# smups/inflatox

Hardware: AMD Instinct MI355X
Metric: grid-points/sec on complete_analysis sweep; achieved HBM GB/s vs peak (higher is better)
Workload: dtype f64

## Files before the change

include/inflx_hip.h:

```cpp
#ifndef INFLX_HIP_H
#define INFLX_HIP_H

#include <stddef.h>
#include <stdint.h>

#ifdef __cplusplus
extern "C" {
#endif

typedef struct inflx_model inflx_model;

typedef enum inflx_status {
  INFLX_OK = 0,
  INFLX_ERR_IO = 1,
  INFLX_ERR_SYMBOL = 2,
  INFLX_ERR_VERSION = 3,
  INFLX_ERR_SHAPE = 4,
  INFLX_ERR_DEVICE = 5,
  INFLX_ERR_ARG = 6,
  INFLX_ERR_BASIS = 7,
  INFLX_ERR_GSL = 8
} inflx_status;

typedef enum inflx_sf_bits {
  INFLX_SF_EDOM = 1,
  INFLX_SF_EDECLINED = 2
} inflx_sf_bits;

typedef enum inflx_sf_policy_t {
  INFLX_SF_QUIET = 0,
  INFLX_SF_FAIL = 1
} inflx_sf_policy_t;

typedef enum inflx_op {
  INFLX_SWEEP_COMPLETE = 0,
  INFLX_SWEEP_CONSISTENCY = 1,
  INFLX_SWEEP_RAPIDTURN = 2,
  INFLX_SWEEP_EPSILON_V = 3,
  INFLX_SWEEP_RAW = 4,
  INFLX_SWEEP_HESSE = 6
} inflx_op;

typedef enum inflx_layout {
  INFLX_AOS = 0,
  INFLX_SOA = 1
} inflx_layout;

const char* inflx_last_error(void);

int inflx_device_count(int* count);

int inflx_open(const char* artefact_path, int device, inflx_model** out);
void inflx_close(inflx_model* model);

int inflx_attach(inflx_model* model, const char* group_object_path);
uint32_t inflx_groups(const inflx_model* model);

uint32_t inflx_n_fields(const inflx_model* model);
uint32_t inflx_n_parameters(const inflx_model* model);
const char* inflx_model_name(const inflx_model* model);
int inflx_device_of(const inflx_model* model);
int inflx_stage_info(const inflx_model* model, uint32_t* n_uniform, uint32_t* n_row, uint32_t* n_col, uint32_t* out_mask);

int inflx_complete_analysis(inflx_model* model, const double* p, size_t n_p, double* out, const double* start_stop,
                            size_t N0, size_t N1, int progress, size_t threads);
int inflx_consistency_only(inflx_model* model, const double* p, size_t n_p, double* out, const double* start_stop,
                           size_t N0, size_t N1, int progress, size_t threads);
int inflx_consistency_rapidturn_only(inflx_model* model, const double* p, size_t n_p, double* out,
                                     const double* start_stop, size_t N0, size_t N1, int progress,
                                     size_t threads);
int inflx_epsilon_v_only(inflx_model* model, const double* p, size_t n_p, double* out, const double* start_stop,
                         size_t N0, size_t N1, int progress, size_t threads);

int inflx_flag_quantum_dif(inflx_model* model, const double* p, size_t n_p, uint8_t* out, const double* start_stop,
                           size_t N0, size_t N1, int progress, double accuracy);

int inflx_sweep_on_trajectory(inflx_model* model, int op, const double* p, size_t n_p, const double* x, size_t n,
                              double* out, int progress, size_t threads);

int inflx_basis_on_points(inflx_model* model, const double* p, size_t n_p, const double* x, size_t n, double* out);
int inflx_validate_basis_at_random(inflx_model* model, uint64_t seed);
int inflx_validate_basis_on_domain(inflx_model* model, const uint32_t* num_points, size_t n_axes, const double* p,
                                   size_t n_p, const double* start_stop, double accuracy);

int inflx_ops_on_values(inflx_model* model, const double* values, size_t n, double* out, int ieee_only);

int inflx_sweep_host(inflx_model* model, int op, const double* p, size_t P, size_t n_p, double* out,
                     const double* start_stop, size_t N0, size_t N1, size_t row_begin, size_t row_count, int layout);

int inflx_sweep_host_planes(inflx_model* model, int op, const double* p, size_t P, size_t n_p, double* out,
                            const double* start_stop, size_t N0, size_t N1, size_t row_begin, size_t row_count,
                            size_t first_plane, size_t n_planes);

int inflx_sweep_device(inflx_model* model, int op, const double* p, size_t P, size_t n_p, void* d_out,
                       size_t d_out_bytes, const double* start_stop, size_t N0, size_t N1, size_t row_begin,
                       size_t row_count, int layout, void* stream);

typedef enum inflx_path {
  INFLX_PATH_TILE = 0,
  INFLX_PATH_ROW_STREAM = 1,
  INFLX_PATH_ROWS = 2,
  INFLX_PATH_COL_STREAM = 3
} inflx_path;
int inflx_sweep_plan(const inflx_model* model, int op, size_t P, size_t N1, size_t row_count, int layout, uint32_t plan[4]);

typedef enum inflx_sweep_flags {
  INFLX_SWEEP_DEFAULT = 0,
  INFLX_SWEEP_FORCE_TILE = 1
} inflx_sweep_flags;
int inflx_sweep_device_ex(inflx_model* model, int op, const double* p, size_t P, size_t n_p, void* d_out,
                          size_t d_out_bytes, const double* start_stop, size_t N0, size_t N1, size_t row_begin,
                          size_t row_count, int layout, void* stream, unsigned flags);
int inflx_sweep_plan_ex(const inflx_model* model, int op, size_t P, size_t N1, size_t row_count, int layout, unsigned flags,
                        uint32_t plan[4]);

int inflx_host_threads(unsigned devices_at_work, unsigned out[3]);

int inflx_sweep_device_timed(inflx_model* model, int op, const double* p, size_t P, size_t n_p, void* d_out,
                             size_t d_out_bytes, const double* start_stop, size_t N0, size_t N1, size_t row_begin,
                             size_t row_count, int layout, void* stream, int repeats, int dominant_only,
                             float* ms_per_launch);
typedef enum inflx_timing {
  INFLX_TIME_BACK_TO_BACK = 0,
  INFLX_TIME_DOMINANT_ONLY = 1,
  INFLX_TIME_IN_PIPELINE = 2,
  INFLX_TIME_SINGLE_CALL = 3
} inflx_timing;
int inflx_sweep_device_timed_ex(inflx_model* model, int op, const double* p, size_t P, size_t n_p, void* d_out,
                                size_t d_out_bytes, const double* start_stop, size_t N0, size_t N1, size_t row_begin,
                                size_t row_count, int layout, void* stream, int repeats, int mode, unsigned flags,
                                float* ms_per_launch);

typedef struct inflx_summary {
  double min[6];
  double max[6];
  uint64_t count[6];
} inflx_summary;

int inflx_sweep_device_stats(inflx_model* model, const double* p, size_t P, size_t n_p, void* d_out, size_t d_out_bytes,
                             const double* start_stop, size_t N0, size_t N1, size_t row_begin, size_t row_count,
                             void* stream, inflx_summary* summary);

int inflx_synchronize(inflx_model* model);

int inflx_sf_status(inflx_model* model, unsigned* bits, int clear);
int inflx_sf_policy(inflx_model* model, int policy);
int inflx_uses_gsl(const inflx_model* model);

typedef struct inflx_multi inflx_multi;
int inflx_shard_plan(size_t P, size_t N0, int world, int rank, size_t plan[5]);
int inflx_open_multi(const char* artefact_path, const int* devices, int n_dev, inflx_multi** out);
void inflx_close_multi(inflx_multi* multi);
int inflx_multi_device_count(const inflx_multi* multi);
inflx_model* inflx_multi_handle(const inflx_multi* multi, int index);
int inflx_sweep_host_multi(inflx_multi* multi, int op, const double* p, size_t P, size_t n_p, double* out,
                           const double* start_stop, size_t N0, size_t N1, int layout, int progress, size_t max_devices);
int inflx_complete_analysis_multi(inflx_multi* multi, const double* p, size_t n_p, double* out, const double* start_stop,
                                  size_t N0, size_t N1, int progress, size_t threads);
int inflx_sweep_stats_multi(inflx_multi* multi, const double* p, size_t P, size_t n_p, const double* start_stop, size_t N0,
                            size_t N1, size_t max_devices, inflx_summary* summary);
int inflx_sweep_device_multi(inflx_multi* multi, int op, const double* p, size_t P, size_t n_p, void* const* d_out,
                             const size_t* d_out_bytes, const double* start_stop, size_t N0, size_t N1, int layout,
                             void* const* streams);
int inflx_sweep_allgather_multi(inflx_multi* multi, int op, const double* p, size_t P, size_t n_p, void* const* d_full,
                                size_t d_full_bytes, const double* start_stop, size_t N0, size_t N1);
typedef enum inflx_gather {
  INFLX_GATHER_PEER_PUSH = 0,
  INFLX_GATHER_RCCL = 1
} inflx_gather;
int inflx_sweep_allgather_multi_ex(inflx_multi* multi, int op, const double* p, size_t P, size_t n_p, void* const* d_full,
                                   size_t d_full_bytes, const double* start_stop, size_t N0, size_t N1, int gather);

typedef enum inflx_eom_method {
  INFLX_EOM_RK4 = 0,
  INFLX_EOM_RKF = 1
} inflx_eom_method;
typedef enum inflx_eom_flags {
  INFLX_EOM_STOP_AT_END = 1,
  INFLX_EOM_FINAL_ONLY = 2,
  INFLX_EOM_SAMPLE_T = 4,
  INFLX_EOM_HOST_SCATTER = 8
} inflx_eom_flags;
typedef enum inflx_eom_status {
  INFLX_EOM_COMPLETE = 0,
  INFLX_EOM_ENDED = 1,
  INFLX_EOM_NONFINITE = 2,
  INFLX_EOM_REJECTED = 3,
  INFLX_EOM_UNDERFLOW = 4,
  INFLX_EOM_TARGET = 5
} inflx_eom_status;
int inflx_solve_eom(inflx_model* model, const double* p, size_t P, size_t n_p, const double* init, size_t B, size_t rows, size_t substeps,
                    int method, double max_err, double dt, unsigned flags, double* states, double* t, double* efolds, int8_t* status,
                    int64_t* last_row);

int inflx_solve_eom_device(inflx_model* model, const double* p, size_t P, size_t n_p, const double* init, size_t B, size_t rows,
                           size_t substeps, int method, double max_err, double dt, unsigned flags, double* d_states, size_t d_states_bytes,
                           double* d_t, size_t d_t_bytes, double* efolds, int8_t* status, int64_t* last_row, void* stream);

int inflx_solve_eom_to_efolds(inflx_model* model, const double* p, size_t P, size_t n_p, const double* init, size_t B, const double* target,
                              size_t max_steps, int method, double max_err, double dt, unsigned flags, double* states, double* t,
                              double* eps_h, double* efolds, int8_t* status);

int inflx_solve_eom_sampled(inflx_model* model, const double* p, size_t P, size_t n_p, const double* init, size_t B, const double* samples,
                            size_t S, size_t max_steps, int method, double max_err, double dt, unsigned flags, double* out, double* efolds,
                            int8_t* status, uint32_t* n_stored);

int inflx_kinematics(inflx_model* model, const double* p, size_t P, size_t n_p, const double* states, size_t n, size_t ld, size_t traj_len,
                     double* out);

int inflx_kinematics_device(inflx_model* model, const double* p, size_t P, size_t n_p, const void* d_states, size_t d_states_bytes, size_t n,
                            size_t ld, size_t traj_len, void* d_out, size_t d_out_bytes, void* stream);

int inflx_masses(inflx_model* model, const double* p, size_t P, size_t n_p, const double* states, size_t n, size_t ld, size_t traj_len, double* out);

int inflx_masses_device(inflx_model* model, const double* p, size_t P, size_t n_p, const void* d_states, size_t d_states_bytes, size_t n, size_t ld,
                        size_t traj_len, void* d_out, size_t d_out_bytes, void* stream);

#ifdef __cplusplus
}
#endif
#endif
```

inflatox_amd/_native.py:

```python

from __future__ import annotations

import ctypes as C
import os
import subprocess

import numpy as np

_PKG = os.path.dirname(os.path.abspath(__file__))
_REPO = os.path.dirname(_PKG)
LIB_PATH = os.path.join(_PKG, "libinflx_hip.so")

OK, ERR_IO, ERR_SYMBOL, ERR_VERSION, ERR_SHAPE, ERR_DEVICE, ERR_ARG, ERR_BASIS, ERR_GSL = range(9)
SF_EDOM, SF_EDECLINED = 1, 2
SF_QUIET, SF_FAIL = 0, 1

OP_COMPLETE, OP_CONSISTENCY, OP_RAPIDTURN, OP_EPSILON_V, OP_RAW = range(5)
OP_HESSE = 6
OP_QDIF = 5
OP_GROUP = {OP_COMPLETE: "core", OP_CONSISTENCY: "consistency", OP_RAPIDTURN: "rapidturn", OP_EPSILON_V: "epsilon_v", OP_RAW: "raw", OP_QDIF: "qdif", OP_HESSE: "hesse"}
OP_WIDTH = {OP_COMPLETE: 6, OP_CONSISTENCY: 1, OP_RAPIDTURN: 1, OP_EPSILON_V: 1, OP_RAW: 5, OP_HESSE: 4}
LAYOUT_AOS, LAYOUT_SOA = 0, 1
SWEEP_DEFAULT, SWEEP_FORCE_TILE = 0, 1
TIME_BACK_TO_BACK, TIME_DOMINANT_ONLY, TIME_IN_PIPELINE, TIME_SINGLE_CALL = range(4)
EOM_RK4, EOM_RKF = 0, 1
EOM_STOP_AT_END, EOM_FINAL_ONLY, EOM_SAMPLE_T, EOM_HOST_SCATTER = 1, 2, 4, 8
GATHER_PEER_PUSH, GATHER_RCCL = 0, 1

_DP = C.POINTER(C.c_double)
_SIZE = C.c_size_t

SIGNATURES = {
    "inflx_last_error": (C.c_char_p, []),
    "inflx_device_count": (C.c_int, [C.POINTER(C.c_int)]),
    "inflx_open": (C.c_int, [C.c_char_p, C.c_int, C.POINTER(C.c_void_p)]),
    "inflx_close": (None, [C.c_void_p]),
    "inflx_attach": (C.c_int, [C.c_void_p, C.c_char_p]),
    "inflx_groups": (C.c_uint32, [C.c_void_p]),
    "inflx_n_fields": (C.c_uint32, [C.c_void_p]),
    "inflx_n_parameters": (C.c_uint32, [C.c_void_p]),
    "inflx_model_name": (C.c_char_p, [C.c_void_p]),
    "inflx_device_of": (C.c_int, [C.c_void_p]),
    "inflx_stage_info": (C.c_int, [C.c_void_p] + [C.POINTER(C.c_uint32)] * 4),
    "inflx_complete_analysis": (C.c_int, [C.c_void_p, _DP, _SIZE, _DP, _DP, _SIZE, _SIZE, C.c_int, _SIZE]),
    "inflx_consistency_only": (C.c_int, [C.c_void_p, _DP, _SIZE, _DP, _DP, _SIZE, _SIZE, C.c_int, _SIZE]),
    "inflx_consistency_rapidturn_only": (C.c_int, [C.c_void_p, _DP, _SIZE, _DP, _DP, _SIZE, _SIZE, C.c_int, _SIZE]),
    "inflx_epsilon_v_only": (C.c_int, [C.c_void_p, _DP, _SIZE, _DP, _DP, _SIZE, _SIZE, C.c_int, _SIZE]),
    "inflx_flag_quantum_dif": (C.c_int, [C.c_void_p, _DP, _SIZE, C.POINTER(C.c_uint8), _DP, _SIZE, _SIZE, C.c_int, C.c_double]),
    "inflx_sweep_on_trajectory": (C.c_int, [C.c_void_p, C.c_int, _DP, _SIZE, _DP, _SIZE, _DP, C.c_int, _SIZE]),
    "inflx_sweep_host": (C.c_int, [C.c_void_p, C.c_int, _DP, _SIZE, _SIZE, _DP, _DP, _SIZE, _SIZE, _SIZE, _SIZE, C.c_int]),
    "inflx_sweep_host_planes": (C.c_int, [C.c_void_p, C.c_int, _DP, _SIZE, _SIZE, _DP, _DP, _SIZE, _SIZE, _SIZE, _SIZE, _SIZE, _SIZE]),
    "inflx_sweep_device": (
        C.c_int,
        [C.c_void_p, C.c_int, _DP, _SIZE, _SIZE, C.c_void_p, _SIZE, _DP, _SIZE, _SIZE, _SIZE, _SIZE, C.c_int, C.c_void_p],
    ),
    "inflx_sweep_device_timed": (
        C.c_int,
        [C.c_void_p, C.c_int, _DP, _SIZE, _SIZE, C.c_void_p, _SIZE, _DP, _SIZE, _SIZE, _SIZE, _SIZE, C.c_int, C.c_void_p, C.c_int, C.c_int, C.POINTER(C.c_float)],
    ),
    "inflx_sweep_device_ex": (
        C.c_int,
        [C.c_void_p, C.c_int, _DP, _SIZE, _SIZE, C.c_void_p, _SIZE, _DP, _SIZE, _SIZE, _SIZE, _SIZE, C.c_int, C.c_void_p, C.c_uint],
    ),
    "inflx_sweep_device_timed_ex": (
        C.c_int,
        [C.c_void_p, C.c_int, _DP, _SIZE, _SIZE, C.c_void_p, _SIZE, _DP, _SIZE, _SIZE, _SIZE, _SIZE, C.c_int, C.c_void_p, C.c_int, C.c_int, C.c_uint, C.POINTER(C.c_float)],
    ),
    "inflx_sweep_plan_ex": (C.c_int, [C.c_void_p, C.c_int, _SIZE, _SIZE, _SIZE, C.c_int, C.c_uint, C.POINTER(C.c_uint32)]),
    "inflx_host_threads": (C.c_int, [C.c_uint, C.POINTER(C.c_uint)]),
    "inflx_sweep_device_stats": (
        C.c_int,
        [C.c_void_p, _DP, _SIZE, _SIZE, C.c_void_p, _SIZE, _DP, _SIZE, _SIZE, _SIZE, _SIZE, C.c_void_p, C.c_void_p],
    ),
    "inflx_synchronize": (C.c_int, [C.c_void_p]),
    "inflx_sf_status": (C.c_int, [C.c_void_p, C.POINTER(C.c_uint), C.c_int]),
    "inflx_sf_policy": (C.c_int, [C.c_void_p, C.c_int]),
    "inflx_uses_gsl": (C.c_int, [C.c_void_p]),
    "inflx_sweep_plan": (C.c_int, [C.c_void_p, C.c_int, _SIZE, _SIZE, _SIZE, C.c_int, C.POINTER(C.c_uint32)]),
    "inflx_basis_on_points": (C.c_int, [C.c_void_p, _DP, _SIZE, _DP, _SIZE, _DP]),
    "inflx_ops_on_values": (C.c_int, [C.c_void_p, _DP, _SIZE, _DP, C.c_int]),
    "inflx_validate_basis_at_random": (C.c_int, [C.c_void_p, C.c_uint64]),
    "inflx_validate_basis_on_domain": (C.c_int, [C.c_void_p, C.POINTER(C.c_uint32), _SIZE, _DP, _SIZE, _DP, C.c_double]),
    "inflx_shard_plan": (C.c_int, [_SIZE, _SIZE, C.c_int, C.c_int, C.POINTER(_SIZE)]),
    "inflx_open_multi": (C.c_int, [C.c_char_p, C.POINTER(C.c_int), C.c_int, C.POINTER(C.c_void_p)]),
    "inflx_close_multi": (None, [C.c_void_p]),
    "inflx_multi_device_count": (C.c_int, [C.c_void_p]),
    "inflx_multi_handle": (C.c_void_p, [C.c_void_p, C.c_int]),
    "inflx_sweep_host_multi": (C.c_int, [C.c_void_p, C.c_int, _DP, _SIZE, _SIZE, _DP, _DP, _SIZE, _SIZE, C.c_int, C.c_int, _SIZE]),
    "inflx_complete_analysis_multi": (C.c_int, [C.c_void_p, _DP, _SIZE, _DP, _DP, _SIZE, _SIZE, C.c_int, _SIZE]),
    "inflx_sweep_stats_multi": (C.c_int, [C.c_void_p, _DP, _SIZE, _SIZE, _DP, _SIZE, _SIZE, _SIZE, C.c_void_p]),
    "inflx_sweep_device_multi": (C.c_int, [C.c_void_p, C.c_int, _DP, _SIZE, _SIZE, C.POINTER(C.c_void_p), C.POINTER(_SIZE), _DP, _SIZE, _SIZE, C.c_int, C.POINTER(C.c_void_p)]),
    "inflx_sweep_allgather_multi": (C.c_int, [C.c_void_p, C.c_int, _DP, _SIZE, _SIZE, C.POINTER(C.c_void_p), _SIZE, _DP, _SIZE, _SIZE]),
    "inflx_sweep_allgather_multi_ex": (C.c_int, [C.c_void_p, C.c_int, _DP, _SIZE, _SIZE, C.POINTER(C.c_void_p), _SIZE, _DP, _SIZE, _SIZE, C.c_int]),
    "inflx_solve_eom": (
        C.c_int,
        [C.c_void_p, _DP, _SIZE, _SIZE, _DP, _SIZE, _SIZE, _SIZE, C.c_int, C.c_double, C.c_double, C.c_uint, _DP, _DP, _DP, C.POINTER(C.c_int8), C.POINTER(C.c_int64)],
    ),
    "inflx_solve_eom_device": (
        C.c_int,
        [C.c_void_p, _DP, _SIZE, _SIZE, _DP, _SIZE, _SIZE, _SIZE, C.c_int, C.c_double, C.c_double, C.c_uint, C.c_void_p, _SIZE, C.c_void_p, _SIZE, _DP, C.POINTER(C.c_int8),
         C.POINTER(C.c_int64), C.c_void_p],
    ),
    "inflx_solve_eom_to_efolds": (
        C.c_int,
        [C.c_void_p, _DP, _SIZE, _SIZE, _DP, _SIZE, _DP, _SIZE, C.c_int, C.c_double, C.c_double, C.c_uint, _DP, _DP, _DP, _DP, C.POINTER(C.c_int8)],
    ),
    "inflx_solve_eom_sampled": (
        C.c_int,
        [C.c_void_p, _DP, _SIZE, _SIZE, _DP, _SIZE, _DP, _SIZE, _SIZE, C.c_int, C.c_double, C.c_double, C.c_uint, _DP, _DP, C.POINTER(C.c_int8), C.POINTER(C.c_uint32)],
    ),
    "inflx_kinematics": (C.c_int, [C.c_void_p, _DP, _SIZE, _SIZE, _DP, _SIZE, _SIZE, _SIZE, _DP]),
    "inflx_kinematics_device": (C.c_int, [C.c_void_p, _DP, _SIZE, _SIZE, C.c_void_p, _SIZE, _SIZE, _SIZE, _SIZE, C.c_void_p, _SIZE, C.c_void_p]),
    "inflx_masses": (C.c_int, [C.c_void_p, _DP, _SIZE, _SIZE, _DP, _SIZE, _SIZE, _SIZE, _DP]),
    "inflx_masses_device": (C.c_int, [C.c_void_p, _DP, _SIZE, _SIZE, C.c_void_p, _SIZE, _SIZE, _SIZE, _SIZE, C.c_void_p, _SIZE, C.c_void_p]),
}


class Summary(C.Structure):

    _fields_ = [("min", C.c_double * 6), ("max", C.c_double * 6), ("count", C.c_uint64 * 6)]

_lib = None


def build_library(force: bool = False) -> str:
    src = os.path.join(_PKG, "csrc", "inflx_hip.cpp")
    deps = [src, os.path.join(_PKG, "csrc", "inflx_kernel_abi.h"), os.path.join(_PKG, "csrc", "inflx_background_abi.h"), os.path.join(_PKG, "csrc", "inflx_background_rows.h"), os.path.join(_PKG, "csrc", "inflx_kinematics_abi.h"), os.path.join(_PKG, "csrc", "inflx_masses_abi.h"), os.path.join(_REPO, "include", "inflx_hip.h")]
    stale = force or not os.path.exists(LIB_PATH) or any(os.path.getmtime(d) > os.path.getmtime(LIB_PATH) for d in deps)
    if stale:
        from .compiler import hipcc_path

        cmd = [
            hipcc_path(),
            "-O2",
            "-fPIC",
            "-shared",
            "-std=c++17",
            "-Wall",
            "-Wextra",
            f"-I{os.path.join(_REPO, 'include')}",
            f"-I{os.path.join(_PKG, 'csrc')}",
            src,
            "-o",
            LIB_PATH + ".tmp",
        ]
        subprocess.run(cmd, check=True)
        os.replace(LIB_PATH + ".tmp", LIB_PATH)
    return LIB_PATH


def _preload_hip_runtime():
    import importlib.util

    try:
        spec = importlib.util.find_spec("torch")
    except (ImportError, ValueError):
        spec = None
    if spec is not None and spec.origin:
        cand = os.path.join(os.path.dirname(spec.origin), "lib", "libamdhip64.so")
        if os.path.exists(cand):
            C.CDLL(cand, mode=C.RTLD_GLOBAL)


def load_library():
    global _lib
    if _lib is None:
        if not os.path.exists(LIB_PATH):
            raise ImportError(
                f"{LIB_PATH} is missing: build it with `python -c 'import __graft_entry__ as g; g.build()'` "
                "(the sweep has no CPU fallback)"
            )
        _preload_hip_runtime()
        lib = C.CDLL(LIB_PATH)
        for name, (res, args) in SIGNATURES.items():
            fn = getattr(lib, name)
            fn.restype = res
            fn.argtypes = args
        _lib = lib
    return _lib


class InflatoxShapeError(Exception):
    """Counterpart of LibInflxRsErr::Shape, which PyO3 raises as a plain Exception (err.rs:71)."""


class InflatoxBasisError(Exception):
    """Counterpart of LibInflxRsErr::BasisNorm / BasisOth (err.rs:36-37), plain Exceptions in PyO3 too."""


class InflatoxSpecialFunctionError(ArithmeticError):
    """A special function of the model was called outside its domain somewhere in the call (``INFLX_ERR_GSL``).  The reference's
    GSL error handler prints the reason and panics at that point (src/err.rs:86-103): the call does not return there either.  Here
    the result was complete when the error was raised -- NaN at the offending points -- and ``sf_errors="nan"`` returns it."""


def _raise(rc: int):
    msg = load_library().inflx_last_error().decode("utf-8", "replace")
    if rc == ERR_GSL:
        raise InflatoxSpecialFunctionError(msg)
    if rc == ERR_IO:
        raise IOError(msg)
    if rc in (ERR_SYMBOL, ERR_VERSION, ERR_DEVICE):
        raise SystemError(msg)
    if rc == ERR_SHAPE:
        raise InflatoxShapeError(msg)
    if rc == ERR_BASIS:
        raise InflatoxBasisError(msg)
    raise ValueError(msg)


def _check(rc: int):
    if rc != OK:
        _raise(rc)


def _sf_policy(mode: str) -> int:
    try:
        return {"raise": SF_FAIL, "nan": SF_QUIET}[mode]
    except (KeyError, TypeError):
        raise ValueError(f'sf_errors must be "raise" or "nan" (got {mode!r})') from None


def _f64(a, name: str) -> np.ndarray:
    try:
        return np.ascontiguousarray(a, dtype=np.float64)
    except (TypeError, ValueError) as exc:
        raise ValueError(f"{name} must be convertible to a float64 array") from exc


def _ptr(a: np.ndarray):
    return a.ctypes.data_as(_DP)


def device_count() -> int:
    n = C.c_int(0)
    rc = load_library().inflx_device_count(C.byref(n))
    return n.value if rc == OK else 0


def _ensure_group(lib, handles, art, group: str) -> None:
    from .compiler import KERNEL_GROUPS

    bit = KERNEL_GROUPS[group]
    pending = [h for h in handles if not (int(lib.inflx_groups(h)) & bit)]
    if not pending or art is None:
        return
    path = art.ensure_group(group)
    if path is None:
        return
    for h in pending:
        _check(lib.inflx_attach(h, os.fsencode(path)))


class InflatoxDevLib:

    def __init__(self, artefact_path: str, device: int = 0):
        lib = load_library()
        handle = C.c_void_p()
        _check(lib.inflx_open(os.fsencode(artefact_path), int(device), C.byref(handle)))
        self._h = handle
        self._lib = lib
        self.path = artefact_path
        from .compiler import artefact_for_path

        self._artefact = artefact_for_path(artefact_path)
        self.device = int(device)
        self.n_fields = int(lib.inflx_n_fields(handle))
        self.n_parameters = int(lib.inflx_n_parameters(handle))
        self.name = lib.inflx_model_name(handle).decode("utf-8", "replace")
        vals = [C.c_uint32(0) for _ in range(4)]
        _check(lib.inflx_stage_info(handle, *[C.byref(v) for v in vals]))
        self.stage_info = dict(zip(("n_uniform", "n_row", "n_col", "out_mask"), (v.value for v in vals)))

    def close(self):
        if getattr(self, "_h", None):
            self._lib.inflx_close(self._h)
            self._h = None

    def __del__(self):
        try:
            self.close()
        except Exception:
            pass

    def _need(self, group: str) -> None:
        _ensure_group(self._lib, [self._h], self._artefact, group)

    @property
    def uses_gsl(self) -> bool:
        return bool(self._lib.inflx_uses_gsl(self._h))

    def sf_status(self, clear: bool = True) -> int:
        bits = C.c_uint(0)
        _check(self._lib.inflx_sf_status(self._h, C.byref(bits), int(bool(clear))))
        return int(bits.value)

    def set_sf_errors(self, mode: str) -> None:
        _check(self._lib.inflx_sf_policy(self._h, _sf_policy(mode)))

    @property
    def groups(self) -> int:
        return int(self._lib.inflx_groups(self._h))

    def _grid(self, fn, p, out, start_stop, progress, threads, last_axis):
        p = _f64(p, "p").reshape(-1)
        ss = _f64(start_stop, "start_stop")
        if ss.shape != (2, 2):
            raise InflatoxShapeError(f"start_stop array should have 2 rows and as many columns as there are fields (got {ss.shape})")
        if out.dtype != np.float64 or not out.flags.c_contiguous or not out.flags.writeable:
            raise ValueError("output array must be a writeable C-contiguous float64 array")
        if last_axis is not None and (out.ndim != 3 or out.shape[2] != last_axis):
            raise InflatoxShapeError(f"Output array should be 3D. Last axis must have lenght {last_axis} (got {out.shape})")
        if last_axis is None and out.ndim != 2:
            raise InflatoxShapeError(f"Output array should be 2D (got {out.shape})")
        _check(fn(self._h, _ptr(p), p.size, _ptr(out), _ptr(ss), out.shape[0], out.shape[1], int(bool(progress)), int(threads)))

    def complete_analysis(self, p, out, start_stop, progress=False, threads=0):
        self._grid(self._lib.inflx_complete_analysis, p, out, start_stop, progress, threads, 6)

    def consistency_only(self, p, out, start_stop, progress=False, threads=0):
        self._need("consistency")
        self._grid(self._lib.inflx_consistency_only, p, out, start_stop, progress, threads, None)

    def consistency_rapidturn_only(self, p, out, start_stop, progress=False, threads=0):
        self._need("rapidturn")
        self._grid(self._lib.inflx_consistency_rapidturn_only, p, out, start_stop, progress, threads, None)

    def epsilon_v_only(self, p, out, start_stop, progress=False, threads=0):
        self._need("epsilon_v")
        self._grid(self._lib.inflx_epsilon_v_only, p, out, start_stop, progress, threads, None)

    def flag_quantum_dif(self, p, out, start_stop, progress=False, accuracy=1e-3):
        p = _f64(p, "p").reshape(-1)
        ss = _f64(start_stop, "start_stop")
        if ss.shape != (2, 2):
            raise InflatoxShapeError(f"start_stop array should have 2 rows and as many columns as there are fields (got {ss.shape})")
        if out.dtype != np.bool_ or out.ndim != 2 or not out.flags.c_contiguous or not out.flags.writeable:
            raise ValueError("output array must be a writeable C-contiguous 2-D bool array")
        self._need("qdif")
        _check(
            self._lib.inflx_flag_quantum_dif(
                self._h, _ptr(p), p.size, out.view(np.uint8).ctypes.data_as(C.POINTER(C.c_uint8)), _ptr(ss), out.shape[0], out.shape[1], int(bool(progress)), float(accuracy)
            )
        )

    def sweep_on_trajectory(self, op, p, x, progress=False, threads=0) -> np.ndarray:
        p = _f64(p, "p").reshape(-1)
        x = _f64(x, "x")
        if x.ndim != 2 or x.shape[1] != 2:
            raise InflatoxShapeError(f"trajectory array should have shape (n,2) (got {x.shape})")
        k = OP_WIDTH[op]
        self._need(OP_GROUP[op])
        from ._result_pool import result_array

        shape = (x.shape[0], k) if k > 1 else (x.shape[0],)
        out = result_array(shape) if x.shape[0] * k * 8 >= (1 << 20) else np.zeros(shape)
        _check(self._lib.inflx_sweep_on_trajectory(self._h, op, _ptr(p), p.size, _ptr(x), x.shape[0], _ptr(out), int(bool(progress)), int(threads)))
        return out

    def basis_on_points(self, p, x) -> np.ndarray:
        p = _f64(p, "p").reshape(-1)
        x = _f64(x, "x")
        if x.ndim != 2 or x.shape[1] != 2:
            raise InflatoxShapeError(f"point array should have shape (n,2) (got {x.shape})")
        out = np.zeros((x.shape[0], 7))
        _check(self._lib.inflx_basis_on_points(self._h, _ptr(p), p.size, _ptr(x), x.shape[0], _ptr(out)))
        return out

    def ops_on_values(self, values, ieee_only: bool = False) -> np.ndarray:
        values = _f64(values, "values")
        if values.ndim != 2 or values.shape[1] != 5:
            raise InflatoxShapeError(f"values array should have shape (n,5) (got {values.shape})")
        out = np.zeros((values.shape[0], 9))
        self._need("values")
        _check(self._lib.inflx_ops_on_values(self._h, _ptr(values), values.shape[0], _ptr(out), int(bool(ieee_only))))
        return out

    def validate_basis_at_random(self, seed: int = 0) -> None:
        _check(self._lib.inflx_validate_basis_at_random(self._h, int(seed)))

    def validate_basis_on_domain(self, num_points, p, start_stop, accuracy) -> None:
        n = np.ascontiguousarray(num_points, dtype=np.uint32).reshape(-1)
        p = _f64(p, "p").reshape(-1)
        ss = _f64(start_stop, "start_stop")
        if ss.ndim != 2 or ss.shape[1] != 2 or ss.shape[0] != n.size:
            raise InflatoxShapeError(f"start_stop array should have 2 rows and as many columns as there are fields (got {ss.shape})")
        _check(
            self._lib.inflx_validate_basis_on_domain(
                self._h, n.ctypes.data_as(C.POINTER(C.c_uint32)), n.size, _ptr(p), p.size, _ptr(ss), float(accuracy)
            )
        )

    def solve_eom(self, p, init, rows: int, substeps: int, method: int, max_err: float, dt: float, flags: int):
        init = _f64(init, "init")
        p = _f64(p, "p")
        B = init.shape[0]
        P = 1 if p.ndim <= 1 else p.shape[0]
        p = p.reshape(-1)
        final_only = bool(flags & EOM_FINAL_ONLY)
        states = np.empty((B, 6) if final_only else (B, rows, 6))
        t = np.empty((B,) if final_only else (B, rows))
        efolds = np.empty(B)
        status = np.empty(B, dtype=np.int8)
        last_row = np.empty(B, dtype=np.int64)
        _check(
            self._lib.inflx_solve_eom(
                self._h, _ptr(p), P, self.n_parameters, _ptr(init), B, int(rows), int(substeps), int(method), float(max_err), float(dt), int(flags),
                _ptr(states), _ptr(t), _ptr(efolds), status.ctypes.data_as(C.POINTER(C.c_int8)), last_row.ctypes.data_as(C.POINTER(C.c_int64)),
            )
        )
        return states, t, efolds, status, last_row

    def solve_eom_device(self, p, init, rows: int, substeps: int, method: int, max_err: float, dt: float, flags: int, d_states_ptr: int, d_states_bytes: int,
                         d_t_ptr: int, d_t_bytes: int, stream: int = 0):
        init = _f64(init, "init")
        p = _f64(p, "p")
        B = init.shape[0]
        P = 1 if p.ndim <= 1 else p.shape[0]
        p = p.reshape(-1)
        efolds = np.empty(B)
        status = np.empty(B, dtype=np.int8)
        last_row = np.empty(B, dtype=np.int64)
        _check(
            self._lib.inflx_solve_eom_device(
                self._h, _ptr(p), P, self.n_parameters, _ptr(init), B, int(rows), int(substeps), int(method), float(max_err), float(dt), int(flags),
                C.c_void_p(d_states_ptr), int(d_states_bytes), C.c_void_p(d_t_ptr), int(d_t_bytes), _ptr(efolds), status.ctypes.data_as(C.POINTER(C.c_int8)),
                last_row.ctypes.data_as(C.POINTER(C.c_int64)), C.c_void_p(stream),
            )
        )
        return efolds, status, last_row

    def solve_eom_to_efolds(self, p, init, target, max_steps: int, method: int, max_err: float, dt: float, flags: int):
        init = _f64(init, "init")
        p = _f64(p, "p")
        target = _f64(target, "target")
        B = init.shape[0]
        if target.shape != (B,):
            raise InflatoxShapeError(f"target must have shape ({B},) (got {target.shape})")
        P = 1 if p.ndim <= 1 else p.shape[0]
        p = p.reshape(-1)
        states = np.empty((B, 6))
        t, eps_h, efolds = np.empty(B), np.empty(B), np.empty(B)
        status = np.empty(B, dtype=np.int8)
        _check(
            self._lib.inflx_solve_eom_to_efolds(
                self._h, _ptr(p), P, self.n_parameters, _ptr(init), B, _ptr(target), int(max_steps), int(method), float(max_err), float(dt), int(flags),
                _ptr(states), _ptr(t), _ptr(eps_h), _ptr(efolds), status.ctypes.data_as(C.POINTER(C.c_int8)),
            )
        )
        return states, t, eps_h, efolds, status

    def solve_eom_sampled(self, p, init, samples, max_steps: int, method: int, max_err: float, dt: float, flags: int):
        init = _f64(init, "init")
        p = _f64(p, "p")
        samples = _f64(samples, "samples")
        if samples.ndim != 1:
            raise InflatoxShapeError(f"samples must be one-dimensional (got shape {samples.shape})")
        B, S = init.shape[0], samples.size
        P = 1 if p.ndim <= 1 else p.shape[0]
        p = p.reshape(-1)
        out = np.empty((S, 8, B))
        efolds = np.empty(B)
        status = np.empty(B, dtype=np.int8)
        n_stored = np.empty(B, dtype=np.uint32)
        _check(
            self._lib.inflx_solve_eom_sampled(
                self._h, _ptr(p), P, self.n_parameters, _ptr(init), B, _ptr(samples), S, int(max_steps), int(method), float(max_err), float(dt), int(flags),
                _ptr(out), _ptr(efolds), status.ctypes.data_as(C.POINTER(C.c_int8)), n_stored.ctypes.data_as(C.POINTER(C.c_uint32)),
            )
        )
        return out, efolds, status, n_stored

    def kinematics(self, p, states: np.ndarray, n: int, ld: int, traj_len: int = 1) -> np.ndarray:
        p = _f64(p, "p")
        P = 1 if p.ndim <= 1 else p.shape[0]
        p = p.reshape(-1)
        out = np.empty((6, n))
        _check(self._lib.inflx_kinematics(self._h, _ptr(p), P, self.n_parameters, _ptr(states), int(n), int(ld), int(traj_len), _ptr(out)))
        return out

    def kinematics_device(self, p, d_states_ptr: int, d_states_bytes: int, n: int, ld: int, traj_len: int, d_out_ptr: int, d_out_bytes: int, stream: int = 0) -> None:
        p = _f64(p, "p")
        P = 1 if p.ndim <= 1 else p.shape[0]
        p = p.reshape(-1)
        _check(
            self._lib.inflx_kinematics_device(
                self._h, _ptr(p), P, self.n_parameters, C.c_void_p(d_states_ptr), int(d_states_bytes), int(n), int(ld), int(traj_len), C.c_void_p(d_out_ptr),
                int(d_out_bytes), C.c_void_p(stream),
            )
        )

    def masses(self, p, states: np.ndarray, n: int, ld: int, traj_len: int = 1) -> np.ndarray:
        p = _f64(p, "p")
        P = 1 if p.ndim <= 1 else p.shape[0]
        p = p.reshape(-1)
        out = np.empty((8, n))
        _check(self._lib.inflx_masses(self._h, _ptr(p), P, self.n_parameters, _ptr(states), int(n), int(ld), int(traj_len), _ptr(out)))
        return out

    def masses_device(self, p, d_states_ptr: int, d_states_bytes: int, n: int, ld: int, traj_len: int, d_out_ptr: int, d_out_bytes: int, stream: int = 0) -> None:
        p = _f64(p, "p")
        P = 1 if p.ndim <= 1 else p.shape[0]
        p = p.reshape(-1)
        _check(
            self._lib.inflx_masses_device(
                self._h, _ptr(p), P, self.n_parameters, C.c_void_p(d_states_ptr), int(d_states_bytes), int(n), int(ld), int(traj_len), C.c_void_p(d_out_ptr),
                int(d_out_bytes), C.c_void_p(stream),
            )
        )

    def sweep_host(self, op, p, start_stop, N0, N1, row_begin=0, row_count=None, layout=LAYOUT_AOS) -> np.ndarray:
        p = _f64(p, "p")
        single = p.ndim == 1
        p2 = p.reshape(1, -1) if single else p
        ss = _f64(start_stop, "start_stop").reshape(-1)
        row_count = N0 - row_begin if row_count is None else row_count
        P, k = p2.shape[0], OP_WIDTH[op]
        if k == 1:
            shape = (P, row_count, N1)
        elif layout == LAYOUT_AOS:
            shape = (P, row_count, N1, k)
        else:
            shape = (P, k, row_count, N1)
        from ._result_pool import result_array

        out = result_array(shape)
        self._need(OP_GROUP[op])
        _check(self._lib.inflx_sweep_host(self._h, op, _ptr(p2), P, p2.shape[1], _ptr(out), _ptr(ss), N0, N1, row_begin, row_count, layout))
        return out[0] if single else out

    def sweep_host_planes(self, op, p, start_stop, N0, N1, first_plane, n_planes, row_begin=0, row_count=None) -> np.ndarray:
        p = _f64(p, "p")
        single = p.ndim == 1
        p2 = p.reshape(1, -1) if single else p
        ss = _f64(start_stop, "start_stop").reshape(-1)
        row_count = N0 - row_begin if row_count is None else row_count
        from ._result_pool import result_array

        out = result_array((p2.shape[0], n_planes, row_count, N1))
        self._need(OP_GROUP[op])
        _check(self._lib.inflx_sweep_host_planes(self._h, op, _ptr(p2), p2.shape[0], p2.shape[1], _ptr(out), _ptr(ss), N0, N1, row_begin, row_count, first_plane, n_planes))
        return out[0] if single else out

    def sweep_device(self, op, p, d_out_ptr: int, d_out_bytes: int, start_stop, N0, N1, row_begin=0, row_count=None, layout=LAYOUT_AOS, stream: int = 0, force_tile: bool = False):
        p2 = _f64(p, "p")
        p2 = p2.reshape(1, -1) if p2.ndim == 1 else p2
        ss = _f64(start_stop, "start_stop").reshape(-1)
        row_count = N0 - row_begin if row_count is None else row_count
        self._need(OP_GROUP[op])
        _check(
            self._lib.inflx_sweep_device_ex(
                self._h, op, _ptr(p2), p2.shape[0], p2.shape[1], C.c_void_p(d_out_ptr), d_out_bytes, _ptr(ss), N0, N1, row_begin, row_count, layout, C.c_void_p(stream),
                SWEEP_FORCE_TILE if force_tile else SWEEP_DEFAULT,
            )
        )

    def sweep_device_timed(self, op, p, d_out_ptr, d_out_bytes, start_stop, N0, N1, row_begin=0, row_count=None, layout=LAYOUT_AOS, stream: int = 0, repeats: int = 10, dominant_only: bool = False, in_pipeline: bool = False, single_call: bool = False, force_tile: bool = False) -> float:
        p2 = _f64(p, "p")
        p2 = p2.reshape(1, -1) if p2.ndim == 1 else p2
        ss = _f64(start_stop, "start_stop").reshape(-1)
        row_count = N0 - row_begin if row_count is None else row_count
        mode = TIME_SINGLE_CALL if single_call else (TIME_IN_PIPELINE if in_pipeline else (TIME_DOMINANT_ONLY if dominant_only else TIME_BACK_TO_BACK))
        ms = C.c_float(0.0)
        self._need(OP_GROUP[op])
        _check(
            self._lib.inflx_sweep_device_timed_ex(
                self._h, op, _ptr(p2), p2.shape[0], p2.shape[1], C.c_void_p(d_out_ptr), d_out_bytes, _ptr(ss), N0, N1, row_begin, row_count, layout, C.c_void_p(stream), repeats, mode,
                SWEEP_FORCE_TILE if force_tile else SWEEP_DEFAULT, C.byref(ms)
            )
        )
        return float(ms.value)

    def sweep_stats(self, p, start_stop, N0, N1, row_begin=0, row_count=None, d_out_ptr: int = 0, d_out_bytes: int = 0, stream: int = 0) -> dict:
        p2 = _f64(p, "p")
        p2 = p2.reshape(1, -1) if p2.ndim == 1 else p2
        ss = _f64(start_stop, "start_stop").reshape(-1)
        row_count = N0 - row_begin if row_count is None else row_count
        out = Summary()
        self._need("stats")
        _check(
            self._lib.inflx_sweep_device_stats(
                self._h, _ptr(p2), p2.shape[0], p2.shape[1], C.c_void_p(d_out_ptr), d_out_bytes, _ptr(ss), N0, N1, row_begin, row_count, C.c_void_p(stream), C.byref(out)
            )
        )
        return {"min": np.array(out.min[:]), "max": np.array(out.max[:]), "count": np.array(out.count[:], dtype=np.uint64)}

    def sweep_plan(self, op, P, N1, row_count, layout=LAYOUT_AOS, force_tile: bool = False) -> dict:
        plan = (C.c_uint32 * 4)()
        _check(self._lib.inflx_sweep_plan_ex(self._h, op, P, N1, row_count, layout, SWEEP_FORCE_TILE if force_tile else SWEEP_DEFAULT, plan))
        path = ("tile", "row_stream", "rows", "col_stream")[plan[0]]
        out = {"path": path, "batch_rows": int(plan[1]), "batches": int(plan[2]), "replicas": int(plan[3])}
        if path == "tile":
            out["tile_rows"] = out.pop("replicas")
        out["host_threads"] = host_threads()
# ... 133 lines not shown
```

inflatox_amd/compiler.py:

```python

from __future__ import annotations

import hashlib
import os
import re
import shutil
import subprocess
import sys
import tempfile
import weakref

import numpy as np
import sympy
from sympy.printing.c import C99CodePrinter

from .staging import HIPInflatoxPrinter, emit_eom_header, emit_kinematics_header, emit_masses_header, emit_stage_header
from .symbolic import InflationModel
from .version import __abi_version__, __version__

_CSRC = os.path.join(os.path.dirname(os.path.abspath(__file__)), "csrc")

KERNEL_GROUPS = {"core": 1, "stats": 2, "values": 4, "consistency": 8, "rapidturn": 16, "epsilon_v": 32, "raw": 64, "qdif": 128, "hesse": 256}
ALL_GROUPS = 511
GROUP_OF_OP = {0: "core", 1: "consistency", 2: "rapidturn", 3: "epsilon_v", 4: "raw", 5: "qdif", 6: "hesse"}

_ARTEFACTS: "weakref.WeakValueDictionary[str, CompilationArtifact]" = weakref.WeakValueDictionary()


def artefact_for_path(path: str):
    return _ARTEFACTS.get(os.path.abspath(path))

_REFERENCE_CONSTANTS = {
    "M_E": "2.71828182846",
    "M_LOG2E": "1.44269504089",
    "M_LOG10E": "0.4342944819",
    "M_LN2": "0.69314718056",
    "M_LN10": "2.30258509299",
    "M_PI": "3.14159265359",
    "M_PI_2": "1.57079632679",
    "M_PI_4": "0.78539816339",
    "M_1_PI": "0.31830988618",
    "M_2_PI": "0.63661977236",
    "M_2_SQRTPI": "1.1283791671",
    "M_SQRT2": "1.41421356237",
    "M_SQRT1_2": "0.70710678118",
}
_EXACT_CONSTANTS = {
    "M_E": "2.7182818284590452354",
    "M_LOG2E": "1.4426950408889634074",
    "M_LOG10E": "0.43429448190325182765",
    "M_LN2": "0.69314718055994530942",
    "M_LN10": "2.30258509299404568402",
    "M_PI": "3.14159265358979323846",
    "M_PI_2": "1.57079632679489661923",
    "M_PI_4": "0.78539816339744830962",
    "M_1_PI": "0.31830988618379067154",
    "M_2_PI": "0.63661977236758134308",
    "M_2_SQRTPI": "1.12837916709551257390",
    "M_SQRT2": "1.41421356237309504880",
    "M_SQRT1_2": "0.70710678118654752440",
}


class CInflatoxPrinter(C99CodePrinter):

    def __init__(self, coordinate_symbols, coordinate_derivative_symbols, settings=None):
        super().__init__(settings)
        plain = super()._print_Symbol
        self.coord_dict = {plain(s): f"x[{i}]" for i, s in enumerate(coordinate_symbols)}
        self.dotcoord_dict = {plain(s): f"xdot[{i}]" for i, s in enumerate(coordinate_derivative_symbols)}
        self.param_dict = {}

    def _print_Symbol(self, expr):
        if expr.is_number:
            return expr.evalf(self._settings["precision"])
        known = self.get_symbol(expr)
        return known if known is not None else self.register_parameter(expr)

    def register_parameter(self, symbol):
        slot = f"args[{len(self.param_dict)}]"
        self.param_dict[super()._print_Symbol(symbol)] = slot
        return slot

    def get_symbol(self, symbol):
        name = super()._print_Symbol(symbol)
        if name.startswith("cse"):
            return name
        for table in (self.coord_dict, self.dotcoord_dict, self.param_dict):
            if name in table:
                return table[name]
        return None


class GSLInflatoxPrinter(CInflatoxPrinter):

    HYPERH = "gsl_sf_hyperg"
    BESSELH = "gsl_sf_bessel"
    _FAMILIES = {
        "besselj": ("J", ("0", "1"), "Jn", "Jnu"),
        "bessely": ("Y", ("0", "1"), "Yn", "Ynu"),
        "besseli": ("I", ("0", "1"), "In", "Inu"),
        "besselk": ("K", ("0", "1"), "Kn", "Knu"),
        "jn": ("j", ("0", "1", "2"), "jl", None),
        "yn": ("y", ("0", "1", "2"), "yl", None),
    }
    _HYPER = {(2, 0): "2F0", (2, 1): "2F1", (1, 1): "1F1", (0, 1): "0F1"}

    def __init__(self, coordinate_symbols, coordinate_derivative_symbols, settings=None):
        super().__init__(coordinate_symbols, coordinate_derivative_symbols, settings)
        self.required_headers = []

    def update_preamble(self, header):
        if header not in self.required_headers:
            self.required_headers.append(header)

    def _bessel(self, expr):
        letter, own, integer_name, real_name = self._FAMILIES[expr.func.__name__]
        self.update_preamble(self.BESSELH)
        arg = expr.args[1]
        nu, x = expr.args[0], (self._print_Symbol(arg) if arg.is_Symbol else self._print(arg))
        if nu.is_integer:
            n = int(float(self._print_Symbol(nu)))
            if str(n) in own:
                return f"gsl_sf_bessel_{letter}{n}({x})"
            return f"gsl_sf_bessel_{integer_name}({n}, {x})"
        if real_name is None:
            raise KeyError("No non-integer impl found.")
        return f"gsl_sf_bessel_{real_name}({self._print_Symbol(nu) if (nu.is_Symbol or nu.is_number) else self._print(nu)}, {x})"

    _print_besselj = _print_bessely = _print_besseli = _print_besselk = _print_jn = _print_yn = _bessel

    def _print_hyper(self, expr):
        self.update_preamble(self.HYPERH)
        ap, bq, x = expr.args[0], expr.args[1], self.doprint(expr.args[2])
        kind = self._HYPER.get((len(ap), len(bq)))
        if kind is None:
            raise Exception("Cannot compute hypergeometric functions other than 2F0, 2F1, 1F1 and 0F1")
        return f"gsl_sf_hyperg_{kind}(" + ", ".join([self.doprint(a) for a in list(ap) + list(bq)] + [x]) + ")"




class CompilationArtifact:

    symbol_printer = C99CodePrinter()

    def __init__(self, symbol_dictionary, shared_object_path, n_fields, n_parameters, auto_cleanup=True, stage_info=None, header_path=None):
        self.symbol_dictionary = symbol_dictionary
        self.shared_object_path = shared_object_path
        self.n_fields = n_fields
        self.n_parameters = n_parameters
        self.auto_cleanup = auto_cleanup
        self.stage_info = stage_info or {}
        self.header_path = header_path
        self._recipe = None
        self.kernel_groups = ALL_GROUPS
        self._build = None
        self._group_paths = {}
        self._eom_recipe = None
        self._companion_paths = {}
        _ARTEFACTS[os.path.abspath(shared_object_path)] = self

    def ensure_group(self, group: str) -> str | None:
        bit = KERNEL_GROUPS[group]
        if self.kernel_groups & bit:
            return None
        path = self._group_paths.get(group)
        if path is None or not os.path.exists(path):
            if self._build is None:
                raise ValueError(f"this artefact does not know how it was compiled: kernel group {group!r} cannot be built (not made by Compiler.compile)")
            header_text, options, tag = self._build
            cached, log, code = _build_code_object(header_text, options, tag, bit)
            if code != 0:
                print(log.decode("utf-8", "replace"))
                raise Exception(f"hipcc compiler error while building kernel group {group!r} (see previous output)")
            path = self.shared_object_path + "." + group
            tmp = path + f".{os.getpid()}.tmp"
            shutil.copyfile(cached, tmp)
            os.replace(tmp, path)
            self._group_paths[group] = path
        return path

    def _trajectory_header_text(self, emitter) -> str:
        if self._eom_recipe is None:
            raise ValueError("this artefact does not know how it was compiled (not made by Compiler.compile)")
        model, params, use_cse, max_cses = self._eom_recipe
        cse = cse_vector = None
        if use_cse:
            def symbols():
                for k in range(max_cses + 1):
                    yield sympy.symbols(f"cse{k}")
                raise Exception("Maximum number of common subexpressions reached!")

            def cse(expr):
                return sympy.cse(expr, symbols=symbols(), order="none", list=False)

            def cse_vector(vector):
                return sympy.cse(list(vector), symbols=symbols(), list=True)

        return emitter(model, params, cse=cse, cse_vector=cse_vector)

    def eom_header_text(self) -> str:
        return self._trajectory_header_text(emit_eom_header)

    def kinematics_header_text(self) -> str:
        return self._trajectory_header_text(emit_kinematics_header)

    def masses_header_text(self) -> str:
        return self._trajectory_header_text(emit_masses_header)

    def _ensure_companion(self, what: str, sources: tuple, object_name: str, headers) -> str:
        path = self._companion_paths.get(what)
        if path is None or not os.path.exists(path):
            if self._build is None or self._eom_recipe is None:
                raise ValueError(f"this artefact does not know how it was compiled: its {what} object cannot be built (not made by Compiler.compile)")
            header_text, options, tag = self._build
            cached, log, code = _build_companion_object(header_text, options, tag, sources, object_name, headers())
            if code != 0:
                print(log.decode("utf-8", "replace"))
                raise Exception(f"hipcc compiler error while building the {what} object (see previous output)")
            path = self.shared_object_path + "." + what
            tmp = path + f".{os.getpid()}.tmp"
            shutil.copyfile(cached, tmp)
            os.replace(tmp, path)
            self._companion_paths[what] = path
        return path

    def ensure_background(self) -> str:
        return self._ensure_companion("background", _BACKGROUND_SOURCES, "bg{key}.hsaco", lambda: [("INFLX_EOM_HEADER", "eom{key}.h", self.eom_header_text())])

    def ensure_kinematics(self) -> str:
        return self._ensure_companion(
            "kinematics", _KINEMATICS_SOURCES, "kin{key}.hsaco",
            lambda: [("INFLX_EOM_HEADER", "kin{key}.eom.h", self.eom_header_text()), ("INFLX_KIN_HEADER", "kin{key}.h", self.kinematics_header_text())],
        )

    def ensure_masses(self) -> str:
        return self._ensure_companion(
            "masses", _MASSES_SOURCES, "mass{key}.hsaco",
            lambda: [("INFLX_EOM_HEADER", "mass{key}.eom.h", self.eom_header_text()), ("INFLX_KIN_HEADER", "mass{key}.kin.h", self.kinematics_header_text()),
                     ("INFLX_MASS_HEADER", "mass{key}.h", self.masses_header_text())],
        )

    def ensure_all_groups(self) -> list[str]:
        return [p for p in (self.ensure_group(g) for g in KERNEL_GROUPS) if p]

    def profile_guided(self, args, extent, silent: bool = True) -> "CompilationArtifact":
        if self._recipe is None:
            raise ValueError("this artefact does not know how it was compiled (not made by Compiler.compile)")
        model, kwargs = self._recipe
        kwargs = dict(kwargs, regroup="auto", sample=(args, extent), silent=silent, tan_shortcut=None)
        return Compiler(model, **kwargs).compile()

    def __del__(self):
        if getattr(self, "auto_cleanup", False):
            for path in [self.shared_object_path, *getattr(self, "_group_paths", {}).values(), *getattr(self, "_companion_paths", {}).values()]:
                if path is None:
                    continue
                try:
                    os.remove(path)
                except OSError:
                    pass

    def lookup_symbol(self, symbol):
        name = self.symbol_printer._print_Symbol(symbol)
        if not isinstance(name, str):
            return None
        return self.symbol_dictionary[name]

    def print_sym_lookup_table(self):
        print("[Symbol Dictionary]")
        for old, new in self.symbol_dictionary.items():
            print(f"{old} -> {new}")


_COMMENT = re.compile(r'"(?:\\.|[^"\\])*"|(?<![0-9A-Za-z_])\'(?:\\.|[^\'\\])*\'|//[^\n]*|/\*.*?\*/', re.S)


def _code_only(source: str) -> str:
    text = _COMMENT.sub(lambda m: m.group(0) if m.group(0)[0] in "\"'" else " ", source)
    return "\n".join(ln.rstrip() for ln in text.splitlines() if ln.strip())


def _tile_kernel_scratch_bytes(code_object: str) -> int:
    tool = os.path.join(os.path.dirname(os.path.realpath(hipcc_path())), "..", "lib", "llvm", "bin", "llvm-readelf")
    if not os.path.exists(tool):
        tool = "/opt/rocm/lib/llvm/bin/llvm-readelf"
    try:
        notes = subprocess.run([tool, "--notes", code_object], capture_output=True, text=True, timeout=60).stdout
    except (OSError, subprocess.SubprocessError):
        return 1 << 30
    for block in notes.split("- .agpr_count:"):
        if re.search(r"\.name:\s+inflx_sweep_tile_complete\s", block):
            m = re.search(r"\.private_segment_fixed_size:\s+(\d+)", block)
            if m:
                return int(m.group(1))
    return 1 << 30


def _cache_dir() -> str:
    d = os.environ.get("INFLATOX_AMD_CACHE") or os.path.join(os.path.dirname(os.path.abspath(__file__)), "_jit_cache")
    os.makedirs(d, exist_ok=True)
    return d


def hipcc_path() -> str:
    cand = os.environ.get("HIPCC") or shutil.which("hipcc") or "/opt/rocm/bin/hipcc"
    if not os.path.exists(cand):
        raise FileNotFoundError("hipcc not found: the HIP back-end needs ROCm's hipcc to build the model code object")
    return cand


def _build_code_object(header_text: str, options: list[str], tag: str, groups: int):
    cache = _cache_dir()
    kernel_src = os.path.join(_CSRC, "inflx_sweep_kernels.hip")
    header_path = os.path.join(cache, f"{tag}.h")
    cached = os.path.join(cache, f"{tag}.hsaco" if groups == KERNEL_GROUPS["core"] else f"{tag}.g{groups}.hsaco")
    log, code = b"", 0
    if not os.path.exists(cached):
        if not os.path.exists(header_path):
            tmp_hdr = header_path + f".{os.getpid()}.tmp"
            with open(tmp_hdr, "w") as fh:
                fh.write(header_text)
            os.replace(tmp_hdr, header_path)
        tmp_out = cached + f".{os.getpid()}.tmp"
        cmd = [hipcc_path(), *options, f"-DINFLX_KERNEL_GROUPS={groups}u", f'-DINFLX_MODEL_TAG="{tag}"', f"-I{_CSRC}", f'-DINFLX_MODEL_HEADER="{header_path}"', kernel_src, "-o", tmp_out]
        proc = subprocess.run(cmd, stdout=subprocess.PIPE, stderr=subprocess.STDOUT)
        log, code = proc.stdout, proc.returncode
        if code == 0:
            os.replace(tmp_out, cached)
    return cached, log, code


_BACKGROUND_SOURCES = ("inflx_background_kernels.hip", "inflx_background.h", "inflx_background_abi.h", "inflx_background_rows.h")
_KINEMATICS_SOURCES = ("inflx_kinematics_kernels.hip", "inflx_kinematics.h", "inflx_kinematics_abi.h")
_MASSES_SOURCES = ("inflx_masses_kernels.hip", "inflx_masses.h", "inflx_masses_abi.h")


def _build_companion_object(header_text: str, options: list[str], tag: str, sources: tuple, object_name: str, headers: list):
    cache = _cache_dir()
    h = hashlib.sha256()
    for _macro, _name, text in headers:
        h.update(text.encode())
    for f in sources:
        with open(os.path.join(_CSRC, f), "r", encoding="utf-8") as fh:
            h.update(_code_only(fh.read()).encode())
    key = h.hexdigest()[:12]
    files = [("INFLX_MODEL_HEADER", os.path.join(cache, f"{tag}.h"), header_text)]
    files += [(macro, os.path.join(cache, f"{tag}." + name.format(key=key)), text) for macro, name, text in headers]
    cached = os.path.join(cache, f"{tag}." + object_name.format(key=key))
    log, code = b"", 0
    if not os.path.exists(cached):
        for _macro, path, text in files:
            if not os.path.exists(path):
                tmp = path + f".{os.getpid()}.tmp"
                with open(tmp, "w") as fh:
                    fh.write(text)
                os.replace(tmp, path)
        tmp_out = cached + f".{os.getpid()}.tmp"
        cmd = [hipcc_path(), *options, f'-DINFLX_MODEL_TAG="{tag}"', f"-I{_CSRC}", *[f'-D{macro}="{path}"' for macro, path, _text in files],
               os.path.join(_CSRC, sources[0]), "-o", tmp_out]
        proc = subprocess.run(cmd, stdout=subprocess.PIPE, stderr=subprocess.STDOUT)
        log, code = proc.stdout, proc.returncode
        if code == 0:
            os.replace(tmp_out, cached)
    return cached, log, code


class Compiler:

    HOIST_MIN_GAIN = 100
    INLINE_MIN_QUOTIENTS = 6
    DEFAULT_TAN_SHORTCUT = 0
    TUNED_TAN_SHORTCUT = 16

    @staticmethod
    def quick_point_gain(info) -> int:
        hoisted, pure = info.get("hoisted_quotients", 0), info.get("pure_quotients", 0)
        shared, groups = info.get("shared_quotients", 0), info.get("shared_reciprocals", 0)
        return 8 * pure + 7 * (hoisted - pure) + 7 * shared - 6 * groups

    MAX_SCRATCH_FOR_THREE_WAVES = 128
    c_prefix = "inflx_auto_"
    lib_prefix = "libinflx_auto_"

    default_hipcc_flags = [
        "--offload-arch=gfx950",
        "--genco",
        "--no-gpu-bundle-output",
        "-O3",
        "-std=c++17",
        "-fno-fast-math",
        "-ffp-contract=on",
        "-fno-gpu-rdc",
        "-Wall",
        "-Werror",
        "-Wno-unused-but-set-variable",
        "-Wno-unused-variable",
        "-Wno-error=pass-failed",
    ]

    def __init__(
        self,
        model: InflationModel,
        output_path: str | None = None,
        cleanup: bool = True,
        silent: bool = False,
        link_gsl: bool = False,
        cse: bool = False,
        max_cses: int = 1000,
        compiler_flags: list[str] | None = None,
        staged: bool = True,
        exact_constants: bool = False,
        regroup: bool | None = None,
        hoist_reciprocals: bool | None = None,
        tan_shortcut: float | None = None,
        share_reciprocals: bool = False,
        sample=None,
        quick_sqrt: bool | None = None,
        kernel_groups="core",
        contraction: str = "expression",
    ):
        self._init_kwargs = dict(output_path=None, cleanup=cleanup, silent=silent, link_gsl=link_gsl, cse=cse, max_cses=max_cses, compiler_flags=compiler_flags,
                                 staged=staged, exact_constants=exact_constants, hoist_reciprocals=hoist_reciprocals, share_reciprocals=share_reciprocals, quick_sqrt=quick_sqrt,
                                 kernel_groups=kernel_groups, contraction=contraction)
        self.gsl = bool(link_gsl)
        if contraction not in ("statement", "expression"):
            raise ValueError('contraction must be "statement" or "expression"')
        self.contraction = contraction
        if isinstance(kernel_groups, str):
            if kernel_groups not in ("core", "all"):
                raise ValueError('kernel_groups must be "core", "all" or an iterable of group names')
            self.kernel_groups = ALL_GROUPS if kernel_groups == "all" else KERNEL_GROUPS["core"]
        else:
            unknown = [g for g in kernel_groups if g not in KERNEL_GROUPS]
            if unknown:
                raise ValueError(f"kernel_groups: unknown group(s) {unknown}; choose from {sorted(KERNEL_GROUPS)}")
            self.kernel_groups = KERNEL_GROUPS["core"]
            for g in kernel_groups:
                self.kernel_groups |= KERNEL_GROUPS[g]
        if model.dim != 2:
            raise Exception("the HIP sweep back-end supports two-field models only")
        self.symbolic_out = model
        self.output_path = output_path
        self.cleanup = cleanup
        self.silent = silent
        self.cse = cse
        self.max_cses = max_cses
        self.staged = staged
        if regroup is None:
            regroup = False
        self.sample = None
        if isinstance(regroup, str) and regroup == "auto":
            if sample is None:
                raise ValueError('regroup="auto" needs sample=(args, (x0_start, x0_stop, x1_start, x1_stop)): the parameter values and the field range the decision is measured on')
            args_, extent_ = sample
            self.sample = (np.ascontiguousarray(args_, dtype=np.float64).reshape(-1), tuple(float(v) for v in extent_))
            if len(self.sample[1]) != 4:
                raise ValueError("sample extent must be (x0_start, x0_stop, x1_start, x1_stop)")
            self.regroup = "auto"
        elif isinstance(regroup, (bool, int)):
            self.regroup = bool(regroup)
        else:
            names = {"V": 0, "v00": 1, "v10": 2, "v11": 3, "g": 4, "v": 5}
            unknown = [n for n in regroup if n not in names]
            if unknown:
                raise ValueError(f"regroup: unknown model value(s) {unknown}; choose from {sorted(names)}")
            self.regroup = frozenset(names[n] for n in regroup)
        self.hoist_reciprocals = hoist_reciprocals
        self.share_reciprocals = bool(share_reciprocals)
        self.quick_sqrt = quick_sqrt
        if tan_shortcut is None:
            tan_shortcut = self.TUNED_TAN_SHORTCUT if self.regroup == "auto" else self.DEFAULT_TAN_SHORTCUT
        if tan_shortcut < 0 or tan_shortcut != int(tan_shortcut) or tan_shortcut >= 2**17:
            raise ValueError("tan_shortcut must be a whole number in [0, 2^17): the largest |v10/v00| for which tan(atan(t)) is taken as t")
        self.tan_shortcut = int(tan_shortcut)
        self.constants = dict(_EXACT_CONSTANTS if exact_constants else _REFERENCE_CONSTANTS)
        self.hipcc_opts = list(compiler_flags) if compiler_flags is not None else list(self.default_hipcc_flags)
        self.symbol_dict = None
        self.stage_info = None

    def _cse_symbols(self):
        k = 0
        while k <= self.max_cses:
            yield sympy.symbols(f"cse{k}")
            k += 1
        raise Exception("Maximum number of common subexpressions reached!")

    def _register(self, printer, expr_or_list):
        is_list = isinstance(expr_or_list, (list, tuple))
        if self.cse:
            if is_list:
                repl, red = sympy.cse(list(expr_or_list), symbols=self._cse_symbols(), list=True)
            else:
                repl, red = sympy.cse(expr_or_list, symbols=self._cse_symbols(), order="none", list=False)
                red = [red]
            for s, d in repl:
                printer.doprint(s)
                printer.doprint(d)
            for r in red:
                printer.doprint(r)
        else:
            for e in expr_or_list if is_list else [expr_or_list]:
                printer.doprint(e)

    def _number_parameters(self):
        m = self.symbolic_out
        pr = (GSLInflatoxPrinter if self.gsl else CInflatoxPrinter)(m.coordinates, m.coordinate_tangents)
        plain = C99CodePrinter()._print_Symbol
        coords = set(m.coordinates) | set(m.coordinate_tangents)

        def pending(exprs):
            want = set()
            for e in exprs:
                want |= {s for s in sympy.sympify(e).free_symbols if s not in coords}
            return {s for s in want if plain(s) not in pr.param_dict}

        dim = m.dim
        flat_metric = [sympy.sympify(m.metric[i][j]) for i in range(dim) for j in range(dim)]
        hesse = [m.hesse_cmp[a][b] for a in range(dim) for b in range(dim)]
        later = hesse + [c for vec in m.basis for c in vec] + [m.gradient_square] + list(m.eom_fields or []) + [m.eom_h, m.eom_hdot]
        later = [e for e in later if e is not None]
        self._register(pr, sympy.sympify(m.potential))
        self._register(pr, flat_metric)
        if pending(later):
            for a in range(dim):
                for b in range(dim):
                    self._register(pr, sympy.sympify(m.hesse_cmp[a][b]))
            for vec in m.basis:
                self._register(pr, [sympy.sympify(c) for c in vec])
            self._register(pr, sympy.sympify(m.gradient_square))
            for e in list(m.eom_fields or []) + [m.eom_h, m.eom_hdot]:
                if e is not None:
                    self._register(pr, sympy.sympify(e))
        symbol_dict = dict(pr.coord_dict)
        symbol_dict.update(pr.param_dict)
        return symbol_dict, dict(pr.param_dict)

    def _generate_hip_header(self) -> str:
        self.symbol_dict, params = self._number_parameters()
        self._param_slots = params
        if not self.silent and self.cse:
            print("Converting sympy to HIP using common subexpression elimination...")
        cse = cse_vector = None
        if self.cse:
            def cse(expr):
                return sympy.cse(expr, symbols=self._cse_symbols(), order="none", list=False)

            def cse_vector(vector):
                return sympy.cse(list(vector), symbols=self._cse_symbols(), list=True)

        if isinstance(self.regroup, str):
            from . import _instrument

            def header_for(regroup):
                saved, saved_info = self.regroup, self.stage_info
                self.regroup = regroup
                try:
                    return self._generate_hip_header()
                finally:
                    self.regroup, self.stage_info = saved, saved_info

            log = None if self.silent else (lambda msg: print("[regroup=auto] " + msg))
            key = hashlib.sha256()
            key.update(header_for(False).encode())
            key.update(header_for(frozenset(range(5))).encode())
            key.update(self.sample[0].tobytes() + np.asarray(self.sample[1], dtype=np.float64).tobytes())
            key.update(repr((_instrument.RTOL, _instrument.C_ERR, _instrument.COPIES)).encode())
            with open(_instrument.__file__, "rb") as fh:
                key.update(fh.read())
            decision_path = os.path.join(_cache_dir(), f"{key.hexdigest()[:20]}.regroup")
            if os.path.exists(decision_path):
                chosen = [int(t) for t in open(decision_path).read().split()]
                if log:
                    log("cached decision: " + ", ".join(_instrument.NAMES[k] for k in chosen))
            else:
                chosen = sorted(_instrument.choose_regroup(header_for, self.sample[0], self.sample[1], log=log))
                if _instrument.host_compiler() is not None:
                    tmp = decision_path + f".{os.getpid()}.tmp"
                    with open(tmp, "w") as fh:
                        fh.write(" ".join(str(k) for k in chosen) + "\n")
                    os.replace(tmp, decision_path)
            self.regroup = frozenset(chosen)
            self.regrouped_values = tuple(_instrument.NAMES[k] for k in sorted(chosen))
            self.symbol_dict, params = self._number_parameters()

        def emit(hoist):
            return emit_stage_header(
                self.symbolic_out,
                params,
                self.constants,
                self.symbolic_out.model_name,
                __version__,
                __abi_version__,
                staged=self.staged,
                cse=cse,
                cse_vector=cse_vector,
                regroup=self.regroup,
                hoist_reciprocals=hoist,
                share_point_reciprocals=self.share_reciprocals,
                quick_sqrt=(hoist is True or hoist == 1) if self.quick_sqrt is None else bool(self.quick_sqrt),
                contract_products=self.contraction == "expression",
            )

        if self.hoist_reciprocals is None:
            text, info = emit(self.staged)
            self._inline_fallback = None
            if self.quick_point_gain(info) < self.HOIST_MIN_GAIN:
                text, info = emit(False)
                if self.staged:
                    itext, iinfo = emit("inline")
                    if iinfo.get("inline_quotients", 0) >= self.INLINE_MIN_QUOTIENTS and self._inline_verdict(itext) != "no":
                        self._inline_fallback = (text, info)
                        text, info = itext, iinfo
        else:
            text, info = emit(self.hoist_reciprocals)
        value_names = ("V", "v00", "v10", "v11", "g")
        info["regrouped"] = (list(value_names) if self.regroup else []) if isinstance(self.regroup, bool) else [value_names[k] for k in sorted(self.regroup) if k < 5]
        self.stage_info = info
        return text

    def _inline_verdict_path(self, inline_header: str) -> str:
        return os.path.join(_cache_dir(), hashlib.sha256(("inline-verdict:" + " ".join(self.hipcc_opts) + inline_header).encode()).hexdigest()[:20] + ".inline")

    def _inline_verdict(self, inline_header: str):
        path = self._inline_verdict_path(inline_header)
        return open(path).read().strip() if os.path.exists(path) else None

    def _hipcc_compile(self, header_text: str):
        kernel_src = os.path.join(_CSRC, "inflx_sweep_kernels.hip")
        deps = [kernel_src] + [os.path.join(_CSRC, f) for f in ("inflx_ops.h", "inflx_device_math.h", "inflx_kernel_abi.h")]
        if "inflx_sf_" in header_text:
            deps += [os.path.join(_CSRC, f) for f in ("inflx_sf.h", "inflx_sf_tables.h")]
        h = hashlib.sha256()
        h.update(header_text.encode())
        for d in deps:
            with open(d, "r", encoding="utf-8") as fh:
                h.update(_code_only(fh.read()).encode())
        opts = list(self.hipcc_opts)
        if self.gsl:
            opts.append("-DINFLX_USE_GSL=1")
        info = self.stage_info or {}
        n_row = (max(1, info.get("nr", 1)) + 1) & ~1
        n_uniform = max(1, info.get("nu", 1))
        fixed_lds = 4 * 64 * 6 * 8 + 34 * 8 + (n_uniform * 8 if n_uniform > 8 else 0)
        if not any(o.startswith("-DINFLX_TILE_ROWS") for o in opts):
            rows = 32
            while rows > 1 and rows * n_row * 8 + fixed_lds > 64 * 1024:
                rows //= 2
            if rows != 32:
                opts.append(f"-DINFLX_TILE_ROWS={rows}")
        if self.tan_shortcut and not any(o.startswith("-DINFLX_TAN_SHORTCUT_MAX") for o in opts):
            opts.append(f"-DINFLX_TAN_SHORTCUT_MAX={self.tan_shortcut}")
        cache = _cache_dir()

        def build(options):
            hh = h.copy()
            hh.update(" ".join(options).encode())
            tag = hh.hexdigest()[:20]
            cached, log, code = _build_code_object(header_text, options, tag, self.kernel_groups)
            return cached, os.path.join(cache, f"{tag}.h"), log, code, list(options), tag

        if any(o.startswith("-DINFLX_MIN_WAVES") for o in opts):
            return build(opts)
        three = opts + ["-DINFLX_MIN_WAVES=3"]
        hh = h.copy()
        hh.update(" ".join(three).encode())
        verdict_path = os.path.join(cache, f"{hh.hexdigest()[:20]}.waves")
        verdict = open(verdict_path).read().strip() if os.path.exists(verdict_path) else None
        if verdict != "2":
            result = build(three)
            if result[3] == 0 and verdict is None:
                verdict = "3" if _tile_kernel_scratch_bytes(result[0]) <= self.MAX_SCRATCH_FOR_THREE_WAVES else "2"
                tmp = verdict_path + f".{os.getpid()}.tmp"
                with open(tmp, "w") as fh:
                    fh.write(verdict + "\n")
                os.replace(tmp, verdict_path)
            if verdict == "3" or result[3] != 0:
                return result
        return build(opts + ["-DINFLX_MIN_WAVES=2"])

    def compile(self) -> CompilationArtifact:
        if not self.silent:
            print("Compiling model...")
        header = self._generate_hip_header()
        cached, header_path, log, code, options, tag = self._hipcc_compile(header)
        fallback = getattr(self, "_inline_fallback", None)
        if code == 0 and fallback is not None and self._inline_verdict(header) is None:
            fits = "-DINFLX_MIN_WAVES=3" in options
            tmp = self._inline_verdict_path(header) + f".{os.getpid()}.tmp"
            with open(tmp, "w") as fh:
                fh.write(("yes" if fits else "no") + "\n")
            os.replace(tmp, self._inline_verdict_path(header))
            if not fits:
                header, self.stage_info = fallback
                self._inline_fallback = None
                cached, header_path, log, code, options, tag = self._hipcc_compile(header)
        if code != 0:
            print(log.decode("utf-8", "replace"))
            print(f'Problematic source file located at: "{header_path}"')
            raise Exception("hipcc compiler error (see previous output)")
        if not self.silent and log:
            print(log.decode("utf-8", "replace"), end="")
        if self.output_path is not None and not self.cleanup:
            with open(self.output_path, "w") as fh:
                fh.write(header)
        fd, out_path = tempfile.mkstemp(prefix=self.lib_prefix, suffix=".hsaco")
        os.close(fd)
        shutil.copyfile(cached, out_path)
        art = CompilationArtifact(
            self.symbol_dict,
            out_path,
            self.symbolic_out.dim,
            len(self.symbol_dict) - self.symbolic_out.dim,
            auto_cleanup=self.cleanup,
            stage_info=self.stage_info,
            header_path=header_path,
        )
        art._recipe = (self.symbolic_out, dict(self._init_kwargs))
        art.kernel_groups = self.kernel_groups
        art._build = (header, options, tag)
        art._eom_recipe = (self.symbolic_out, dict(self._param_slots), self.cse, self.max_cses)
        return art
```

inflatox_amd/csrc/inflx_hip.cpp:

```cpp
#include "inflx_hip.h"

#include <dlfcn.h>
#include <hip/hip_runtime.h>

#include <algorithm>
#include <atomic>
#include <cerrno>
#include <chrono>
#include <cmath>
#include <cstdarg>
#include <cstdio>
#include <cstdlib>
#include <condition_variable>
#include <cstring>
#include <mutex>
#include <future>
#include <random>
#include <string>
#include <thread>
#include <vector>

#include <sched.h>
#include <sys/mman.h>
#if defined(__x86_64__)
#include <emmintrin.h>
#endif
#include <unistd.h>

#include "inflx_background_abi.h"
#include "inflx_background_rows.h"
#include "inflx_kernel_abi.h"
#include "inflx_kinematics_abi.h"
#include "inflx_masses_abi.h"

namespace {

thread_local std::string g_last_error;

int fail(int code, const char* fmt, ...) {
  char buf[1024];
  va_list ap;
  va_start(ap, fmt);
  vsnprintf(buf, sizeof buf, fmt, ap);
  va_end(ap);
  g_last_error = buf;
  return code;
}

#define HIP_TRY(expr)                                                                              \
  do {                                                                                             \
    hipError_t e_ = (expr);                                                                        \
    if (e_ != hipSuccess) return fail(INFLX_ERR_DEVICE, "%s failed: %s", #expr, hipGetErrorString(e_)); \
  } while (0)

constexpr uint16_t kAbiMajor = 5, kAbiMinor = 0;
const char* const kOpNames[INFLX_OP_COUNT] = {"complete", "consistency", "rapidturn", "epsilon_v", "raw", "qdif", "hesse"};
constexpr int kOpWidth[INFLX_OP_COUNT] = {6, 1, 1, 1, 5, 1, 4};
constexpr size_t kOpBytes[INFLX_OP_COUNT] = {48, 8, 8, 8, 40, 1, 32};

size_t chunk_bytes_limit() {
  static const size_t v = [] {
    const char* e = getenv("INFLX_CHUNK_MB");
    const long mb = e ? atol(e) : 0;
    return (size_t)(mb > 0 ? mb : 32) << 20;
  }();
  return v;
}
size_t whole_result_limit() {
  static const size_t v = [] {
    const char* e = getenv("INFLX_WHOLE_RESULT_MB");
    const long mb = e ? atol(e) : -1;
    return (size_t)(mb >= 0 ? mb : 65536) << 20;
  }();
  return v;
}
unsigned quota_from(const std::string& quota_file, const std::string& period_file) {
  FILE* fh = fopen(quota_file.c_str(), "r");
  if (!fh) return 0;
  char a[64] = {0}, b[64] = {0};
  const int got = fscanf(fh, "%63s %63s", a, b);
  fclose(fh);
  if (got < 1 || strcmp(a, "max") == 0) return 0;
  double quota = atof(a), period = got >= 2 ? atof(b) : 0.0;
  if (!period_file.empty()) {
    FILE* ph = fopen(period_file.c_str(), "r");
    if (!ph) return 0;
    if (fscanf(ph, "%63s", b) == 1) period = atof(b);
    fclose(ph);
  }
  if (quota <= 0.0 || period <= 0.0) return 0;
  return (unsigned)std::max(1.0, std::floor(quota / period + 0.5));
}

std::string own_cgroup(const char* want) {
  FILE* fh = fopen("/proc/self/cgroup", "r");
  if (!fh) return "";
  char line[1024];
  std::string found;
  while (fgets(line, sizeof line, fh)) {
    char* c1 = strchr(line, ':');
    char* c2 = c1 ? strchr(c1 + 1, ':') : nullptr;
    if (!c2) continue;
    std::string ctrl(c1 + 1, c2), path(c2 + 1);
    while (!path.empty() && (path.back() == '\n' || path.back() == '\r')) path.pop_back();
    const bool match = *want ? (("," + ctrl + ",").find(std::string(",") + want + ",") != std::string::npos) : ctrl.empty();
    if (match) { found = path; break; }
  }
  fclose(fh);
  return found;
}

unsigned min_quota_upwards(const std::string& mount, std::string leaf, bool v2) {
  unsigned best = 0;
  for (;;) {
    const std::string dir = mount + (leaf == "/" ? "" : leaf);
    const unsigned q = v2 ? quota_from(dir + "/cpu.max", "") : quota_from(dir + "/cpu.cfs_quota_us", dir + "/cpu.cfs_period_us");
    if (q && (!best || q < best)) best = q;
    if (leaf.empty() || leaf == "/") break;
    const size_t cut = leaf.find_last_of('/');
    leaf = cut == 0 || cut == std::string::npos ? "/" : leaf.substr(0, cut);
  }
  return best;
}

unsigned detect_cpu_budget() {
  unsigned n = std::max(1u, std::thread::hardware_concurrency());
  cpu_set_t set;
  CPU_ZERO(&set);
  if (sched_getaffinity(0, sizeof set, &set) == 0) n = std::max(1, CPU_COUNT(&set));
  unsigned quota = min_quota_upwards("/sys/fs/cgroup", own_cgroup(""), true);
  if (!quota) quota = min_quota_upwards("/sys/fs/cgroup", "/", true);
  for (const char* mount : {"/sys/fs/cgroup/cpu", "/sys/fs/cgroup/cpu,cpuacct"}) {
    unsigned q = min_quota_upwards(mount, own_cgroup("cpu"), false);
    if (!q) q = min_quota_upwards(mount, "/", false);
    if (q && (!quota || q < quota)) quota = q;
  }
  return quota ? std::min(n, quota) : n;
}

unsigned host_cpu_budget() {
  static const unsigned v = [] {
    const char* e = getenv("INFLX_HOST_THREADS");
    const long n = e ? atol(e) : 0;
    return n > 0 ? (unsigned)n : detect_cpu_budget();
  }();
  return v;
}

thread_local unsigned tl_sharers = 1;

struct HelperPlan {
  unsigned prefault, fill;
};
HelperPlan helper_plan(unsigned cpus, unsigned sharers) {
  cpus = std::max(1u, cpus);
  sharers = std::max(1u, sharers);
  const unsigned share = std::max(1u, cpus / sharers);
  HelperPlan h;
  h.prefault = std::max(1u, std::min(8u, (share + 1) / 2));
  h.fill = std::min(64u, sharers == 1 ? 2 * share : share);
  return h;
}

unsigned prefault_threads() {
  static const long forced = [] {
    const char* e = getenv("INFLX_PREFAULT_THREADS");
    return e ? atol(e) : 0L;
  }();
  return forced > 0 ? (unsigned)forced : helper_plan(host_cpu_budget(), tl_sharers).prefault;
}

unsigned host_fill_threads() {
  static const long forced = [] {
    const char* e = getenv("INFLX_HOST_FILL_THREADS");
    return e ? atol(e) : 0L;
  }();
  return forced > 0 ? (unsigned)forced : helper_plan(host_cpu_budget(), tl_sharers).fill;
}

#if defined(__x86_64__)
constexpr bool kTouchIsAtomic = true;
#else
constexpr bool kTouchIsAtomic = false;
#endif
void touch_range(char* begin, size_t bytes) {
  const size_t page = (size_t)sysconf(_SC_PAGESIZE);
  char* lo = reinterpret_cast<char*>((reinterpret_cast<uintptr_t>(begin) + page - 1) / page * page);
  char* hi = reinterpret_cast<char*>(reinterpret_cast<uintptr_t>(begin + bytes) / page * page);
#if defined(__x86_64__)
  for (char* q = lo; q < hi; q += page) asm volatile("lock orb $0, %0" : "+m"(*q) : : "cc");
#else
  if (hi > lo && madvise(lo, (size_t)(hi - lo), MADV_POPULATE_WRITE) != 0)
    for (volatile char* q = lo; q < hi; q += page) *q = *q;
#endif
}

void advise_huge_pages(char* begin, size_t bytes) {
#ifdef MADV_HUGEPAGE
  const size_t page = (size_t)sysconf(_SC_PAGESIZE);
  char* lo = reinterpret_cast<char*>((reinterpret_cast<uintptr_t>(begin) + page - 1) / page * page);
  char* hi = reinterpret_cast<char*>(reinterpret_cast<uintptr_t>(begin + bytes) / page * page);
  if (hi > lo) (void)madvise(lo, (size_t)(hi - lo), MADV_HUGEPAGE);
#else
  (void)begin, (void)bytes;
#endif
}

void prefault_range(char* begin, size_t bytes) {
  const size_t page = (size_t)sysconf(_SC_PAGESIZE);
  char* lo = reinterpret_cast<char*>((reinterpret_cast<uintptr_t>(begin) + page - 1) / page * page);
  char* hi = reinterpret_cast<char*>(reinterpret_cast<uintptr_t>(begin + bytes) / page * page);
  if (hi <= lo) return;
#ifdef MADV_HUGEPAGE
  (void)madvise(lo, (size_t)(hi - lo), MADV_HUGEPAGE);
#endif
  const unsigned nthreads = (unsigned)std::min<size_t>(prefault_threads(), (size_t)(hi - lo) / (size_t(8) << 20) + 1);
  static const bool use_populate = [] {
    const char* e = getenv("INFLX_PREFAULT_MODE");
    return e && strcmp(e, "populate") == 0;
  }();
  auto work = [](char* a, char* b) {
#ifdef MADV_POPULATE_WRITE
    if (use_populate && madvise(a, (size_t)(b - a), MADV_POPULATE_WRITE) == 0) return;
#endif
    touch_range(a, (size_t)(b - a));
  };
  std::vector<std::thread> pool;
  const size_t pages = (size_t)(hi - lo) / page;
  for (unsigned t = 0; t < nthreads; ++t) {
    char* a = lo + pages * t / nthreads * page;
    char* b = lo + pages * (t + 1) / nthreads * page;
    bool spawned = false;
    if (t + 1 < nthreads) {
      try {
        pool.emplace_back(work, a, b);
        spawned = true;
      } catch (...) {
      }
    }
    if (!spawned) work(a, b);
  }
  for (auto& th : pool) th.join();
}

struct TableRing {
  double* buf[2] = {nullptr, nullptr};
  size_t cap[2] = {0, 0};
  hipEvent_t ready[2] = {nullptr, nullptr};
  hipEvent_t free[2] = {nullptr, nullptr};
  bool used[2] = {false, false};
  unsigned turn = 0;

  bool create() {
    for (int b = 0; b < 2; ++b)
      if (hipEventCreateWithFlags(&ready[b], hipEventDisableTiming | hipEventDisableSystemFence) != hipSuccess ||
          hipEventCreateWithFlags(&free[b], hipEventDisableTiming | hipEventDisableSystemFence) != hipSuccess)
        return false;
    return true;
  }
  void destroy() {
    for (int b = 0; b < 2; ++b) {
      if (ready[b]) (void)hipEventDestroy(ready[b]);
      if (free[b]) (void)hipEventDestroy(free[b]);
      if (buf[b]) (void)hipFree(buf[b]);
    }
  }
  bool idle() const {
    for (int b = 0; b < 2; ++b)
      if (used[b] && hipEventQuery(free[b]) != hipSuccess) return false;
    return true;
  }
  int grow(int b, size_t doubles) {
    if (buf[b]) HIP_TRY(hipFree(buf[b]));
    buf[b] = nullptr;
    cap[b] = 0;
    HIP_TRY(hipMalloc(reinterpret_cast<void**>(&buf[b]), doubles * sizeof(double)));
    cap[b] = doubles;
    return INFLX_OK;
  }
};
}

#define INFLX_SERIALISE(m) \
  std::unique_lock<std::recursive_mutex> inflx_call_lock_; \
  if (m) inflx_call_lock_ = std::unique_lock<std::recursive_mutex>((m)->mu)

struct inflx_model {
  std::recursive_mutex mu;
  int device = 0;
  hipModule_t module = nullptr;
  hipStream_t stream = nullptr;
  hipStream_t copy_stream = nullptr;
  hipFunction_t tile[INFLX_OP_COUNT] = {};
  hipFunction_t rows[INFLX_OP_COUNT] = {};
  hipFunction_t traj[INFLX_OP_COUNT] = {};
  hipFunction_t basis_points = nullptr;
  hipFunction_t ops_on_values = nullptr;
  hipFunction_t rowvals[INFLX_OP_COUNT] = {};
  hipFunction_t rowstream6 = nullptr;
  hipFunction_t rowstream_planes = nullptr;
  hipFunction_t colvals[INFLX_OP_COUNT] = {};
  hipFunction_t colstream = nullptr;
  hipFunction_t colvals_stats = nullptr;
  hipFunction_t stage_tables = nullptr;
  TableRing stage_ring;
  hipFunction_t tile_stats = nullptr, tile_stats_nostore = nullptr, rowvals_stats = nullptr;
  double* d_stats = nullptr;
  TableRing row_ring;
  hipStream_t side = nullptr;
  std::vector<std::pair<hipEvent_t, hipEvent_t>>* probe = nullptr;
  size_t probe_used = 0;
  bool probe_overflow = false;
  InflxKernelInfo info = {};
  uint32_t groups = 0;
  std::vector<hipModule_t> attached;
  std::string tag;
  std::vector<hipDeviceptr_t> sf_words;
  int sf_policy = INFLX_SF_QUIET;
  hipEvent_t sf_done = nullptr;
  bool sf_pending = false;
  char use_gsl = 0;
  uint16_t version[3] = {};
  uint32_t dim = 0, n_par = 0;
  std::string name, path;
  struct ParamSlot {
    double* host = nullptr;
    double* dev = nullptr;
    size_t cap = 0, count = 0;
    hipStream_t stream = nullptr;
    hipEvent_t last_use = nullptr;
    hipStream_t last_reader = nullptr;
    bool in_flight = false;
  };
  static constexpr int kParamSlots = 4;
  ParamSlot pslot[kParamSlots];
  int pcur = 0;
  void* d_chunk[2] = {nullptr, nullptr};
  size_t d_chunk_cap[2] = {0, 0};
  void* d_whole = nullptr;
  size_t d_whole_cap = 0;
  hipEvent_t chunk_done[2] = {nullptr, nullptr};
  hipEvent_t copy_done[2] = {nullptr, nullptr};
  hipEvent_t t0 = nullptr, t1 = nullptr;
  hipModule_t bg_module = nullptr;
  hipFunction_t bg_init = nullptr;
  hipFunction_t bg_advance[2][2] = {};
  hipFunction_t bg_target[2] = {};
  hipFunction_t bg_sampled[2] = {};
  hipFunction_t bg_rows_transpose = nullptr;
  hipModule_t kin_module = nullptr;
  hipFunction_t kin_states = nullptr;
  hipModule_t mass_module = nullptr;
  hipFunction_t mass_states = nullptr;
};

namespace {

template <typename T>
int read_global(inflx_model* m, const char* sym, T* dst, size_t bytes, bool exact) {
  hipDeviceptr_t dptr = nullptr;
  size_t size = 0;
  if (hipModuleGetGlobal(&dptr, &size, m->module, sym) != hipSuccess)
    return fail(INFLX_ERR_SYMBOL, "artefact %s lacks symbol %s", m->path.c_str(), sym);
  if (exact ? size != bytes : size > bytes)
    return fail(INFLX_ERR_SYMBOL, "symbol %s in %s has %zu bytes, expected %s%zu", sym, m->path.c_str(), size,
                exact ? "" : "<= ", bytes);
  HIP_TRY(hipMemcpy(dst, dptr, size, hipMemcpyDeviceToHost));
  return INFLX_OK;
}

int acquire_params(inflx_model* m, const double* p, size_t count, hipStream_t s, const double** d_params) {
  inflx_model::ParamSlot& cur = m->pslot[m->pcur];
  if (cur.dev && cur.count == count && cur.stream == s && memcmp(cur.host, p, count * sizeof(double)) == 0) {
    *d_params = cur.dev;
    return INFLX_OK;
  }
  const int next = (m->pcur + 1) % inflx_model::kParamSlots;
  inflx_model::ParamSlot& slot = m->pslot[next];
  if (slot.in_flight) {
    HIP_TRY(hipEventSynchronize(slot.last_use));
    slot.in_flight = false;
  }
  if (!slot.last_use) HIP_TRY(hipEventCreateWithFlags(&slot.last_use, hipEventDisableTiming));
  if (count > slot.cap) {
    if (slot.dev) HIP_TRY(hipFree(slot.dev));
    if (slot.host) HIP_TRY(hipHostFree(slot.host));
    slot.dev = slot.host = nullptr;
    slot.cap = slot.count = 0;
    const size_t cap = std::max<size_t>(count, 64);
    HIP_TRY(hipHostMalloc(reinterpret_cast<void**>(&slot.host), cap * sizeof(double), hipHostMallocDefault));
    HIP_TRY(hipMalloc(reinterpret_cast<void**>(&slot.dev), cap * sizeof(double)));
    slot.cap = cap;
  }
  memcpy(slot.host, p, count * sizeof(double));
  HIP_TRY(hipMemcpyAsync(slot.dev, slot.host, count * sizeof(double), hipMemcpyHostToDevice, s));
  slot.count = count;
  slot.stream = s;
  m->pcur = next;
  *d_params = slot.dev;
  return INFLX_OK;
}

int release_params(inflx_model* m, hipStream_t reader) {
  inflx_model::ParamSlot& cur = m->pslot[m->pcur];
  if (!cur.last_use) return INFLX_OK;
  if (cur.in_flight && cur.last_reader != reader) HIP_TRY(hipStreamWaitEvent(reader, cur.last_use, 0));
  HIP_TRY(hipEventRecord(cur.last_use, reader));
  cur.last_reader = reader;
  cur.in_flight = true;
  return INFLX_OK;
}

int release_params_after(inflx_model* m, hipStream_t reader, int rc) {
  if (rc == INFLX_OK) return release_params(m, reader);
  const std::string first = g_last_error;
  (void)release_params(m, reader);
  g_last_error = first;
  return rc;
}

void note_sf_word(inflx_model* m, hipModule_t module) {
  if (!m->use_gsl) return;
  hipDeviceptr_t dptr = nullptr;
  size_t size = 0;
  if (hipModuleGetGlobal(&dptr, &size, module, "INFLX_SF_STATUS") == hipSuccess && size == sizeof(unsigned))
    m->sf_words.push_back(dptr);
  else
    (void)hipGetLastError();
}

int sf_collect(inflx_model* m, bool clear, unsigned* bits) {
  *bits = 0;
  if (m->sf_words.empty()) return INFLX_OK;
  HIP_TRY(hipSetDevice(m->device));
  HIP_TRY(hipStreamSynchronize(m->side));
  HIP_TRY(hipStreamSynchronize(m->stream));
  if (m->sf_pending) {
    HIP_TRY(hipEventSynchronize(m->sf_done));
    m->sf_pending = false;
  }
  for (hipDeviceptr_t w : m->sf_words) {
    unsigned v = 0;
    HIP_TRY(hipMemcpy(&v, w, sizeof v, hipMemcpyDeviceToHost));
    *bits |= v;
    if (v && clear) {
      const unsigned zero = 0;
      HIP_TRY(hipMemcpy(w, &zero, sizeof zero, hipMemcpyHostToDevice));
    }
  }
  return INFLX_OK;
}

int sf_error(const inflx_model* m, unsigned bits) {
  const bool dom = (bits & INFLX_SF_EDOM) != 0;
  return fail(INFLX_ERR_GSL, "a GSL exception ocurred (ERRCODE %s): model \"%s\" called a special function %s at one or more points of this call. "
              "Those points hold NaN and the result is complete otherwise; the reference's GSL error handler panics here instead of returning. "
              "inflx_sf_policy(handle, INFLX_SF_QUIET) / GeneralisedAL(..., sf_errors=\"nan\") returns the result with its NaNs.",
              dom ? "0X1" : "0X11", m->name.c_str(),
              dom ? "outside its domain (input domain error)" : "where this implementation could not deliver 1e-13 and declined (loss of accuracy)");
}

int sf_verdict(inflx_model* m) {
  if (m->sf_words.empty() || m->sf_policy != INFLX_SF_FAIL) return INFLX_OK;
  unsigned bits = 0;
  const int rc = sf_collect(m, true, &bits);
  if (rc) return rc;
  return bits ? sf_error(m, bits) : INFLX_OK;
}

const char* const kGroupNames[9] = {"core", "stats", "values", "consistency", "rapidturn", "epsilon_v", "raw", "qdif", "hesse"};
uint32_t group_of_op(int op) { return INFLX_GROUP_OF_OP(op); }

int resolve_group_kernels(inflx_model* m, hipModule_t module, uint32_t mask, const char* path) {
  auto get = [&](hipFunction_t* slot, const std::string& name) -> int {
    if (hipModuleGetFunction(slot, module, name.c_str()) != hipSuccess) {
      *slot = nullptr;
      return fail(INFLX_ERR_SYMBOL, "artefact %s lacks kernel %s", path, name.c_str());
    }
    return INFLX_OK;
  };
  int rc;
  for (int op = 0; op < INFLX_OP_COUNT; ++op) {
    if (!(mask & group_of_op(op))) continue;
    const std::string nm = kOpNames[op];
    if ((rc = get(&m->tile[op], "inflx_sweep_tile_" + nm)) || (rc = get(&m->rows[op], "inflx_sweep_rows_" + nm)) || (rc = get(&m->traj[op], "inflx_sweep_traj_" + nm)) ||
        (rc = get(&m->rowvals[op], "inflx_sweep_rowvals_" + nm)) || (rc = get(&m->colvals[op], "inflx_sweep_colvals_" + nm)))
      return rc;
  }
  if (mask & INFLX_GROUP_CORE) {
    if ((rc = get(&m->rowstream6, "inflx_sweep_rowstream6")) || (rc = get(&m->rowstream_planes, "inflx_sweep_rowstream_planes")) || (rc = get(&m->colstream, "inflx_sweep_colstream")) ||
        (rc = get(&m->stage_tables, "inflx_stage_tables")) || (rc = get(&m->basis_points, "inflx_basis_points")))
      return rc;
  }
  if (mask & INFLX_GROUP_STATS) {
    if ((rc = get(&m->tile_stats, "inflx_sweep_tile_complete_stats")) || (rc = get(&m->tile_stats_nostore, "inflx_sweep_tile_complete_stats_nostore")) ||
        (rc = get(&m->rowvals_stats, "inflx_sweep_rowvals_complete_stats")) || (rc = get(&m->colvals_stats, "inflx_sweep_colvals_complete_stats")))
      return rc;
  }
  if (mask & INFLX_GROUP_VALUES) {
    if ((rc = get(&m->ops_on_values, "inflx_ops_on_values"))) return rc;
  }
  return INFLX_OK;
}

template <typename T>
int read_global_of(hipModule_t module, const char* path, const char* sym, T* dst, size_t bytes, bool exact) {
  hipDeviceptr_t dptr = nullptr;
  size_t size = 0;
  if (hipModuleGetGlobal(&dptr, &size, module, sym) != hipSuccess) return fail(INFLX_ERR_SYMBOL, "artefact %s lacks symbol %s", path, sym);
  if (exact ? size != bytes : size > bytes) return fail(INFLX_ERR_SYMBOL, "symbol %s in %s has %zu bytes, expected %s%zu", sym, path, size, exact ? "" : "<= ", bytes);
  HIP_TRY(hipMemcpy(dst, dptr, size, hipMemcpyDeviceToHost));
  return INFLX_OK;
}

int attach_object(inflx_model* m, const char* path) {
  hipModule_t module = nullptr;
  hipError_t e = hipModuleLoad(&module, path);
  if (e != hipSuccess) return fail(INFLX_ERR_IO, "could not load %s as a gfx950 code object: %s", path, hipGetErrorString(e));
  auto bail = [&](int code) {
    const std::string first = g_last_error;
    (void)hipModuleUnload(module);
    g_last_error = first;
    return code;
  };
  uint16_t version[3] = {};
  InflxKernelInfo info = {};
  uint32_t groups = 0;
  char tag[128] = {0};
  int rc;
  if ((rc = read_global_of(module, path, "VERSION", version, sizeof version, true)) || (rc = read_global_of(module, path, "INFLX_KERNEL_INFO", &info, sizeof info, true)) ||
      (rc = read_global_of(module, path, "INFLX_GROUPS", &groups, sizeof groups, true)) || (rc = read_global_of(module, path, "MODEL_TAG", tag, sizeof tag - 1, false)))
    return bail(rc);
  if (version[0] != m->version[0] || version[1] != m->version[1] || memcmp(&info, &m->info, sizeof info) != 0 || m->tag != tag)
    return bail(fail(INFLX_ERR_VERSION, "%s does not belong to artefact %s: built from another model, with other options or for another kernel ABI (tag \"%s\", expected \"%s\")",
                     path, m->path.c_str(), tag, m->tag.c_str()));
  const uint32_t fresh = groups & ~m->groups;
  if ((rc = resolve_group_kernels(m, module, fresh, path))) return bail(rc);
  m->attached.push_back(module);
  m->groups |= fresh;
  note_sf_word(m, module);
  return INFLX_OK;
}

int need_groups(inflx_model* m, uint32_t mask) {
  uint32_t missing = mask & ~m->groups & INFLX_GROUP_ALL;
  for (int b = 0; missing && b < 9; ++b) {
    const uint32_t bit = 1u << b;
    if (!(missing & bit)) continue;
    const std::string side = m->path + "." + kGroupNames[b];
    FILE* fh = fopen(side.c_str(), "rb");
    if (!fh)
      return fail(INFLX_ERR_SYMBOL, "the kernels of group \"%s\" are not part of %s and no %s exists: build that group (inflatox_amd does on first use; "
                  "Compiler(kernel_groups=\"all\") builds a complete artefact) and pass it to inflx_attach", kGroupNames[b], m->path.c_str(), side.c_str());
    fclose(fh);
    HIP_TRY(hipSetDevice(m->device));
    const int rc = attach_object(m, side.c_str());
    if (rc) return rc;
    missing = mask & ~m->groups & INFLX_GROUP_ALL;
  }
  return INFLX_OK;
}

int validate(inflx_model* m, int op, const double* p, size_t P, size_t n_p, bool kernels = true) {
  if (!m) return fail(INFLX_ERR_ARG, "model handle is NULL");
  if (op < 0 || op >= INFLX_OP_COUNT) return fail(INFLX_ERR_ARG, "unknown sweep operation %d", op);
  if (m->dim != 2)
    return fail(INFLX_ERR_SHAPE, "the Anguelova & Lazaroiu consistency condition requires a 2-field model (model has %u fields)",
                m->dim);
  if (n_p != m->n_par)
    return fail(INFLX_ERR_SHAPE, "model \"%s\" has %u paramters (got %zu)", m->name.c_str(), m->n_par, n_p);
  if (!p && n_p) return fail(INFLX_ERR_ARG, "parameter array is NULL");
  if (P == 0) return fail(INFLX_ERR_SHAPE, "parameter array has no rows");
  if (kernels && (m->groups & group_of_op(op)) == 0) {
    INFLX_SERIALISE(m);
    return need_groups(m, group_of_op(op));
  }
  return INFLX_OK;
}

struct SweepPlan {
  int path = INFLX_PATH_TILE;
  size_t batch = 0;
  size_t cpr = 0;
  size_t replicas = 0;
  size_t rows_per_launch = 0;
  bool one_stream = false;

  hipStream_t upload_stream(const inflx_model* m, hipStream_t s) const {
    return path == INFLX_PATH_ROWS || one_stream ? s : m->side;
  }
  hipStream_t reader_stream(const inflx_model* m, hipStream_t s) const {
    return path == INFLX_PATH_ROW_STREAM || path == INFLX_PATH_COL_STREAM ? upload_stream(m, s) : s;
  }
};

SweepPlan plan_sweep(const InflxKernelInfo& info, int op, int layout, size_t P, size_t N1, size_t row_count, unsigned flags, bool alone) {
  SweepPlan pl;
  const size_t K = kOpWidth[op];
  const bool aos6 = K == 6 && layout == INFLX_AOS;
  const bool planes = layout == INFLX_SOA || K == 1;
  const bool may_broadcast = op != INFLX_OP_QDIF && !(flags & INFLX_SWEEP_FORCE_TILE);
  const bool row_only = may_broadcast && (info.out_mask & 2u) == 0, col_only = may_broadcast && (info.out_mask & 3u) == 2u;
  if (row_only && (aos6 || (planes && N1 % 2 == 0))) {
    pl.path = INFLX_PATH_ROW_STREAM;
    const size_t units_row = aos6 ? 3 * N1 : N1 / 2;
    pl.cpr = (units_row + info.row_chunk_units - 1) / info.row_chunk_units;
    pl.replicas = 32;
    while (pl.replicas > 1 && pl.replicas > pl.cpr) pl.replicas /= 2;
    const size_t line_bytes = row_count * pl.replicas * 64;
    pl.batch = std::max<size_t>(1, std::min<size_t>(P, (size_t(64) << 20) / std::max<size_t>(line_bytes, 1)));
    pl.batch = std::min<size_t>(pl.batch, 65535 / (aos6 ? 1 : K));
    pl.one_stream = alone && P <= pl.batch;
  } else if (col_only && (planes ? N1 : K * N1) % 2 == 0) {
    pl.path = INFLX_PATH_COL_STREAM;
    pl.batch = std::max<size_t>(1, std::min<size_t>(P, (size_t(64) << 20) / std::max<size_t>(K * N1 * 8, 1)));
    pl.batch = std::min<size_t>(pl.batch, 65535 / (planes ? K : 1));
    pl.one_stream = alone && P <= pl.batch;
  } else if (row_only) {
    pl.path = INFLX_PATH_ROWS;
  } else {
    pl.path = INFLX_PATH_TILE;
    const size_t nu = std::max<size_t>(info.n_uniform, 1), nc = std::max<size_t>(info.n_col, 1);
    const size_t nr = (std::max<size_t>(info.n_row, 1) + 1) & ~size_t(1);
    pl.rows_per_launch = size_t(65535) * info.tile_rows;
    const size_t per_p = nu + std::min(pl.rows_per_launch, row_count) * nr + nc * N1;
    pl.batch = std::max<size_t>(1, std::min<size_t>(P, (size_t(1) << 27) / std::max<size_t>(per_p, 1)));
    pl.one_stream = alone && P <= pl.batch && row_count <= pl.rows_per_launch;
  }
  return pl;
}

bool handle_idle(inflx_model* m) {
  const bool idle = m->row_ring.idle() && m->stage_ring.idle();
  (void)hipGetLastError();
  return idle;
}

hipError_t probe_begin(inflx_model* m, hipStream_t s) {
  if (!m->probe) return hipSuccess;
  if (m->probe_used >= m->probe->size()) {
    m->probe_overflow = true;
    return hipSuccess;
  }
  return hipEventRecord((*m->probe)[m->probe_used].first, s);
}
hipError_t probe_end(inflx_model* m, hipStream_t s) {
  if (!m->probe || m->probe_used >= m->probe->size()) return hipSuccess;
  return hipEventRecord((*m->probe)[m->probe_used++].second, s);
}


struct BroadcastPath {
  hipFunction_t eval;
  unsigned eval_gx, eval_block;
  hipFunction_t store;
  size_t cpr;
  size_t z_per_p;
  size_t table_doubles;
};

int launch_broadcast(inflx_model* m, const SweepPlan& plan, const BroadcastPath& path, int op, InflxSweepArgs a, const double* d_params, size_t P,
                     double* d_out, hipStream_t s, bool stores_only) {
  void* params[] = {&a};
  TableRing& ring = m->row_ring;
  const hipStream_t ev = plan.upload_stream(m, s);
  const size_t batch = plan.batch, row_count = a.row_count;
  if (path.cpr > 0x7fffffffULL) return fail(INFLX_ERR_SHAPE, "grid rows too long for one launch");
  if (stores_only && batch < P)
    return fail(INFLX_ERR_ARG, "dominant_only timing needs the parameter rows to fit one table batch (%zu rows here, got %zu)", batch, P);
  const bool store = d_out != nullptr;
  for (size_t p0 = 0; p0 < P; p0 += batch) {
    const size_t pb = std::min(batch, P - p0);
    const int b = (int)((ring.turn + (stores_only ? 1 : 0)) & 1);
    if (store && pb * path.table_doubles > ring.cap[b]) {
      HIP_TRY(hipDeviceSynchronize());
      const int rc = ring.grow(b, pb * path.table_doubles);
      if (rc) return rc;
    }
    a.params = d_params + p0 * m->n_par;
    a.out = store ? d_out + p0 * row_count * a.N1 * kOpWidth[op] : nullptr;
    a.P = (uint32_t)pb;
    a.row_table = store ? ring.buf[b] : nullptr;
    if (!stores_only) {
      if (ring.used[b]) HIP_TRY(hipStreamWaitEvent(ev, ring.free[b], 0));
      HIP_TRY(hipModuleLaunchKernel(path.eval, path.eval_gx, (unsigned)pb, 1, path.eval_block, 1, 1, 0, ev, params, nullptr));
      if (ev != s) HIP_TRY(hipEventRecord(ring.ready[b], ev));
      ring.turn++;
    }
    if (store) {
      if (ev != s) HIP_TRY(hipStreamWaitEvent(s, ring.ready[b], 0));
      for (size_t r0 = 0; r0 < row_count; r0 += 65535) {
        a.stream_row0 = (uint32_t)r0;
        const size_t nr = std::min<size_t>(65535, row_count - r0);
        HIP_TRY(probe_begin(m, s));
        HIP_TRY(hipModuleLaunchKernel(path.store, (unsigned)path.cpr, (unsigned)nr, (unsigned)(pb * path.z_per_p), m->info.tile_cols, 1, 1, 0, s, params, nullptr));
        HIP_TRY(probe_end(m, s));
      }
      HIP_TRY(hipEventRecord(ring.free[b], s));
      ring.used[b] = true;
    }
  }
  return INFLX_OK;
}

int launch_rows_fallback(inflx_model* m, int op, InflxSweepArgs a, size_t P, size_t N1, size_t row_count, hipStream_t s) {
  void* params[] = {&a};
  const size_t rpb = m->info.rows_per_block;
  const size_t groups = (row_count + rpb - 1) / rpb;
  size_t chunks = 1;
  const size_t want = 4096;
  if (groups * P < want) {
    const size_t units = N1 / 64;
    chunks = std::min<size_t>(std::max<size_t>(units, 1), (want + groups * P - 1) / (groups * P));
  }
  if (groups * chunks > 0x7fffffffULL) return fail(INFLX_ERR_SHAPE, "grid too large for one launch");
  a.col_chunks = (uint32_t)chunks;
  HIP_TRY(hipModuleLaunchKernel(m->rows[op], (unsigned)(groups * chunks), (unsigned)P, 1, m->info.tile_cols, 1, 1, 0, s, params,
                                nullptr));
  return INFLX_OK;
}

constexpr size_t kLaunchWorkgroups = 1024;

size_t tile_height(size_t full, size_t segments) {
  return std::min(full, std::max<size_t>({size_t(1), std::min(full / 2, segments / kLaunchWorkgroups), segments / (4 * kLaunchWorkgroups)}));
}

int launch_tiles(inflx_model* m, const SweepPlan& plan, int op, InflxSweepArgs a, const double* d_params, size_t P, double* d_out, size_t N1,
                 size_t row_count, hipStream_t s, double* d_stats) {
  void* params[] = {&a};
  TableRing& ring = m->stage_ring;
  const size_t gx = (N1 + m->info.tile_cols - 1) / m->info.tile_cols;
  if (gx > 0x7fffffffULL) return fail(INFLX_ERR_SHAPE, "grid rows too long for one launch (%zu column tiles)", gx);
  if (row_count > 0xffffffffULL) return fail(INFLX_ERR_SHAPE, "at most 2^32 grid rows per call (got %zu)", row_count);
  hipFunction_t f = d_stats ? (d_out ? m->tile_stats : m->tile_stats_nostore) : m->tile[op];
  const size_t nu = std::max<size_t>(m->info.n_uniform, 1), nc = std::max<size_t>(m->info.n_col, 1);
  const size_t nr = (std::max<size_t>(m->info.n_row, 1) + 1) & ~size_t(1);
  const size_t rows_per_launch = plan.rows_per_launch, pbatch = plan.batch;
  const hipStream_t tables = plan.upload_stream(m, s);
  for (size_t p0 = 0; p0 < P; p0 += pbatch) {
    const size_t pb = std::min(pbatch, P - p0);
    a.params = d_params + p0 * m->n_par;
    a.out = d_out ? reinterpret_cast<double*>(reinterpret_cast<char*>(d_out) + p0 * row_count * N1 * kOpBytes[op]) : nullptr;
    a.P = (uint32_t)pb;
    for (size_t r0 = 0; r0 < row_count; r0 += rows_per_launch) {
      const size_t slab = std::min(rows_per_launch, row_count - r0);
      const size_t need = pb * (nu + slab * nr + nc * N1);
      const int b = (int)(ring.turn & 1);
      if (need > ring.cap[b]) {
        if (ring.used[b]) HIP_TRY(hipEventSynchronize(ring.free[b]));
        const int rc = ring.grow(b, need);
        if (rc) return rc;
      }
      a.row_table = ring.buf[b];
      a.stream_row0 = (uint32_t)r0;
      a.stream_units = slab;
      if (ring.used[b]) HIP_TRY(hipStreamWaitEvent(tables, ring.free[b], 0));
      const size_t tx = (slab + m->info.tile_cols - 1) / m->info.tile_cols + (N1 + m->info.tile_cols - 1) / m->info.tile_cols;
      HIP_TRY(hipModuleLaunchKernel(m->stage_tables, (unsigned)tx, (unsigned)pb, 1, m->info.tile_cols, 1, 1, 0, tables, params, nullptr));
      ring.turn++;
      if (tables != s) {
        HIP_TRY(hipEventRecord(ring.ready[b], tables));
        HIP_TRY(hipStreamWaitEvent(s, ring.ready[b], 0));
      }
      const size_t th = tile_height(m->info.tile_rows, gx * slab * pb);
      a.tile_rows = (uint32_t)th;
      const size_t gy = (slab + th - 1) / th;
      HIP_TRY(probe_begin(m, s));
      HIP_TRY(hipModuleLaunchKernel(f, (unsigned)gx, (unsigned)gy, (unsigned)pb, m->info.tile_cols, 1, 1, 0, s, params, nullptr));
      HIP_TRY(probe_end(m, s));
      HIP_TRY(hipEventRecord(ring.free[b], s));
      ring.used[b] = true;
    }
  }
  return INFLX_OK;
}

int launch_grid(inflx_model* m, const SweepPlan& plan, int op, const double* d_params, size_t P, double* d_out, const double* ss, size_t N0,
                size_t N1, size_t row_begin, size_t row_count, int layout, hipStream_t s, bool stores_only = false, double accuracy = 0.0,
                double* d_stats = nullptr) {
  if (row_count == 0 || N1 == 0) return INFLX_OK;
  if (P > 65535) {
    for (size_t p0 = 0; p0 < P; p0 += 65535) {
      const size_t pb = std::min<size_t>(65535, P - p0);
      double* sub = d_out ? reinterpret_cast<double*>(reinterpret_cast<char*>(d_out) + p0 * row_count * N1 * kOpBytes[op]) : nullptr;
      const int rc = launch_grid(m, plan, op, d_params + p0 * m->n_par, pb, sub, ss, N0, N1, row_begin, row_count, layout, s, stores_only, accuracy, d_stats);
      if (rc) return rc;
    }
    return INFLX_OK;
  }
  InflxSweepArgs a;
  memset(&a, 0, sizeof a);
  a.out = d_out;
  a.params = d_params;
  a.x0a = ss[0];
  a.dx0 = (ss[1] - ss[0]) / (double)N0;
  a.x1a = ss[2];
  a.dx1 = (ss[3] - ss[2]) / (double)N1;
  a.N1 = N1;
  a.row_begin = row_begin;
  a.row_count = row_count;
  a.P = (uint32_t)P;
  a.layout = (uint32_t)layout;
  a.col_chunks = 1;
  a.accuracy = accuracy;
  a.stats = d_stats;
  const size_t K = kOpWidth[op];
  switch (plan.path) {
    case INFLX_PATH_ROW_STREAM: {
      const bool aos6 = K == 6 && layout == INFLX_AOS;
      a.table_replicas = (uint32_t)plan.replicas;
      a.stream_planes = (uint32_t)K;
      const BroadcastPath path = {d_stats ? m->rowvals_stats : m->rowvals[op], (unsigned)((row_count + 63) / 64), 64,
                                  aos6 ? m->rowstream6 : m->rowstream_planes, plan.cpr, aos6 ? 1 : K, row_count * plan.replicas * 8};
      return launch_broadcast(m, plan, path, op, a, d_params, P, d_out, s, stores_only);
    }
    case INFLX_PATH_COL_STREAM: {
      const bool planes = layout == INFLX_SOA || K == 1;
      a.stream_units = (planes ? N1 : K * N1) / 2;
      const size_t tc = m->info.tile_cols;
      const BroadcastPath path = {d_stats ? m->colvals_stats : m->colvals[op], (unsigned)((N1 + tc - 1) / tc), (unsigned)tc,
                                  m->colstream, (a.stream_units + tc - 1) / tc, planes ? K : 1, K * N1};
      return launch_broadcast(m, plan, path, op, a, d_params, P, d_out, s, stores_only);
    }
    case INFLX_PATH_ROWS:
      return launch_rows_fallback(m, op, a, P, N1, row_count, s);
    default:
      return launch_tiles(m, plan, op, a, d_params, P, d_out, N1, row_count, s, d_stats);
  }
}

int ensure_chunk(inflx_model* m, int which, size_t bytes) {
  if (bytes <= m->d_chunk_cap[which]) return INFLX_OK;
  if (m->d_chunk[which]) HIP_TRY(hipFree(m->d_chunk[which]));
  m->d_chunk[which] = nullptr;
  m->d_chunk_cap[which] = 0;
  HIP_TRY(hipMalloc(&m->d_chunk[which], bytes));
  m->d_chunk_cap[which] = bytes;
  return INFLX_OK;
}

void say(const char* fmt, ...) {
  va_list ap;
  va_start(ap, fmt);
  fputs("[Inflatox Info] ", stderr);
  vfprintf(stderr, fmt, ap);
  fputc('\n', stderr);
  fflush(stderr);
  va_end(ap);
}

void warn(const char* fmt, ...) {
  va_list ap;
  va_start(ap, fmt);
  fputs("[Inflatox Warning] ", stderr);
  vfprintf(stderr, fmt, ap);
  fputc('\n', stderr);
  fflush(stderr);
  va_end(ap);
}

std::string num_text(double v, int digits = -1) {
  if (std::isnan(v)) return "NaN";
  if (std::isinf(v)) return v > 0 ? "inf" : "-inf";
  char buf[64];
  if (digits >= 0) snprintf(buf, sizeof buf, "%.*f", digits, v); else snprintf(buf, sizeof buf, "%.17g", v);
  return buf;
}

std::string list_text(const double* v, size_t n) {
  std::string s = "[";
  for (size_t k = 0; k < n; ++k) s += (k ? ", " : "") + num_text(v[k], 3);
  return s + "]";
}

double unit_random(uint64_t& state) {
  uint64_t z = (state += 0x9E3779B97F4A7C15ull);
  z = (z ^ (z >> 30)) * 0xBF58476D1CE4E5B9ull;
  z = (z ^ (z >> 27)) * 0x94D049BB133111EBull;
  z ^= z >> 31;
  return (double)(z >> 11) * 0x1.0p-53;
}

int check_basis(const double* basis, const double* x, size_t n, double accuracy, size_t* failed) {
  for (size_t k = 0; k < n; ++k) {
    const double* b = basis + 7 * k;
    const std::string point = list_text(x + 2 * k, 2);
    bool encountered_nan = false;
    const int pair[3][2] = {{0, 0}, {0, 1}, {1, 1}};
    for (int q = 0; q < 3; ++q) {
      const int i = pair[q][0], j = pair[q][1];
      const double ip = b[q];
      const std::string vi = list_text(b + 3 + 2 * i, 2), vj = list_text(b + 3 + 2 * j, 2);
      if (i == j) {
        if (!std::isnormal(ip)) {
          warn("Norm of basisvector %d is %s at field-space point %s. v%d=%s\nAre we outside the model's domain?", i,
               num_text(ip).c_str(), point.c_str(), i, vi.c_str());
          encountered_nan = true;
        } else if (std::fabs(ip - 1.) >= accuracy) {
          return fail(INFLX_ERR_BASIS, "Expected basis vector %d to be normalised everywhere in the models domain. Instead, "
                      "found norm %s at %s.", i, num_text(ip).c_str(), point.c_str());
        }
      } else {
        if (!std::isnormal(ip) && ip != 0.0) {
          warn("w%d•w%d = %s at field-space point %s.\nv%d=%s\nv%d=%s\nAre we outside the model's domain?", i, j,
               num_text(ip).c_str(), point.c_str(), i, vi.c_str(), j, vj.c_str());
          encountered_nan = true;
        } else if (std::fabs(ip) >= accuracy) {
          return fail(INFLX_ERR_BASIS, "Expected basis vectors w%d and w%d to be orthogonal everywhere in the model's domain. "
                      "Instead, found inner product %s at %s.", i, j, num_text(ip).c_str(), point.c_str());
        }
      }
    }
    if (encountered_nan) ++*failed;
  }
  return INFLX_OK;
}

}

extern "C" {

const char* inflx_last_error(void) { return g_last_error.c_str(); }

int inflx_device_count(int* count) {
  if (!count) return fail(INFLX_ERR_ARG, "count is NULL");
  *count = 0;
  hipError_t e = hipGetDeviceCount(count);
  if (e != hipSuccess) {
    *count = 0;
    return fail(INFLX_ERR_DEVICE, "hipGetDeviceCount failed: %s", hipGetErrorString(e));
  }
  return INFLX_OK;
}

int inflx_open(const char* artefact_path, int device, inflx_model** out) {
  if (!artefact_path || !out) return fail(INFLX_ERR_ARG, "artefact path / output handle is NULL");
  *out = nullptr;
  FILE* fh = fopen(artefact_path, "rb");
  if (!fh) return fail(INFLX_ERR_IO, "could not open model artefact %s: %s", artefact_path, strerror(errno));
  fclose(fh);
  int ndev = 0;
  if (hipGetDeviceCount(&ndev) != hipSuccess || ndev <= 0)
    return fail(INFLX_ERR_DEVICE, "no HIP device available: the sweep has no CPU fallback");
  if (device < 0 || device >= ndev) return fail(INFLX_ERR_ARG, "device %d out of range (have %d)", device, ndev);
  HIP_TRY(hipSetDevice(device));

  inflx_model* m = new inflx_model();
  m->device = device;
  m->path = artefact_path;
  auto bail = [&](int code) {
    inflx_close(m);
    return code;
  };
  hipError_t e = hipModuleLoad(&m->module, artefact_path);
  if (e != hipSuccess) {
    m->module = nullptr;
    fail(INFLX_ERR_IO, "could not load %s as a gfx950 code object: %s", artefact_path, hipGetErrorString(e));
    return bail(INFLX_ERR_IO);
  }
  int rc;
  if ((rc = read_global(m, "VERSION", m->version, sizeof m->version, true))) return bail(rc);
  if (m->version[0] != kAbiMajor || m->version[1] != kAbiMinor) {
    fail(INFLX_ERR_VERSION, "artefact %s was built for inflatox ABI v%u.%u.%u, this library implements v%u.%u", artefact_path,
         m->version[0], m->version[1], m->version[2], kAbiMajor, kAbiMinor);
    return bail(INFLX_ERR_VERSION);
  }
  if ((rc = read_global(m, "DIM", &m->dim, sizeof m->dim, true))) return bail(rc);
  if ((rc = read_global(m, "N_PARAMETERS", &m->n_par, sizeof m->n_par, true))) return bail(rc);
  char name[512] = {0};
  if ((rc = read_global(m, "MODEL_NAME", name, sizeof name - 1, false))) return bail(rc);
  m->name = name;
  if ((rc = read_global(m, "INFLX_KERNEL_INFO", &m->info, sizeof m->info, true))) return bail(rc);
  if (m->info.kernel_abi != INFLX_KERNEL_ABI) {
    fail(INFLX_ERR_VERSION, "artefact %s uses kernel ABI %u, this library expects %u", artefact_path, m->info.kernel_abi,
         INFLX_KERNEL_ABI);
    return bail(INFLX_ERR_VERSION);
  }
  if ((rc = read_global(m, "USE_GSL", &m->use_gsl, sizeof m->use_gsl, true))) return bail(rc);
  note_sf_word(m, m->module);
  m->sf_policy = m->use_gsl ? INFLX_SF_FAIL : INFLX_SF_QUIET;
  char tag[128] = {0};
  if ((rc = read_global(m, "INFLX_GROUPS", &m->groups, sizeof m->groups, true))) return bail(rc);
  if ((rc = read_global(m, "MODEL_TAG", tag, sizeof tag - 1, false))) return bail(rc);
  m->tag = tag;
  m->groups &= INFLX_GROUP_ALL;
  if (!(m->groups & INFLX_GROUP_CORE)) {
    fail(INFLX_ERR_SYMBOL, "artefact %s is not a model's core object (it carries kernel groups 0x%x only): open the core object and attach this one (inflx_attach)", artefact_path, m->groups);
    m->groups = 0;
    return bail(INFLX_ERR_SYMBOL);
  }
  {
    const uint32_t present = m->groups;
    m->groups = 0;
    if ((rc = resolve_group_kernels(m, m->module, present, artefact_path))) return bail(rc);
    m->groups = present;
  }
  if (hipStreamCreateWithFlags(&m->stream, hipStreamNonBlocking) != hipSuccess ||
      hipStreamCreateWithFlags(&m->side, hipStreamNonBlocking) != hipSuccess ||
      hipStreamCreateWithFlags(&m->copy_stream, hipStreamNonBlocking) != hipSuccess) {
    fail(INFLX_ERR_DEVICE, "could not create HIP streams");
    return bail(INFLX_ERR_DEVICE);
  }
  for (int k = 0; k < 2; ++k) {
    if (hipEventCreateWithFlags(&m->chunk_done[k], hipEventDisableTiming) != hipSuccess ||
        hipEventCreateWithFlags(&m->copy_done[k], hipEventDisableTiming) != hipSuccess) {
      fail(INFLX_ERR_DEVICE, "could not create HIP events");
      return bail(INFLX_ERR_DEVICE);
    }
  }
  for (TableRing* ring : {&m->row_ring, &m->stage_ring}) {
    if (!ring->create()) {
      fail(INFLX_ERR_DEVICE, "could not create HIP events");
      return bail(INFLX_ERR_DEVICE);
    }
  }
  if (hipEventCreate(&m->t0) != hipSuccess || hipEventCreate(&m->t1) != hipSuccess) {
    fail(INFLX_ERR_DEVICE, "could not create HIP timing events");
    return bail(INFLX_ERR_DEVICE);
  }
  *out = m;
  return INFLX_OK;
}

void inflx_close(inflx_model* m) {
  if (!m) return;
  { std::lock_guard<std::recursive_mutex> last_call_has_returned(m->mu); }
  (void)hipSetDevice(m->device);
  if (m->stream) (void)hipStreamSynchronize(m->stream);
  if (m->side) (void)hipStreamSynchronize(m->side);
  if (m->copy_stream) (void)hipStreamSynchronize(m->copy_stream);
  for (int k = 0; k < 2; ++k) {
    if (m->d_chunk[k]) (void)hipFree(m->d_chunk[k]);
    if (m->chunk_done[k]) (void)hipEventDestroy(m->chunk_done[k]);
    if (m->copy_done[k]) (void)hipEventDestroy(m->copy_done[k]);
  }
  for (TableRing* ring : {&m->row_ring, &m->stage_ring}) ring->destroy();
  if (m->t0) (void)hipEventDestroy(m->t0);
  if (m->t1) (void)hipEventDestroy(m->t1);
  if (m->sf_done) (void)hipEventDestroy(m->sf_done);
  for (auto& slot : m->pslot) {
    if (slot.dev) (void)hipFree(slot.dev);
    if (slot.host) (void)hipHostFree(slot.host);
    if (slot.last_use) (void)hipEventDestroy(slot.last_use);
  }
  if (m->d_stats) (void)hipFree(m->d_stats);
  if (m->d_whole) (void)hipFree(m->d_whole);
  if (m->stream) (void)hipStreamDestroy(m->stream);
  if (m->side) (void)hipStreamDestroy(m->side);
  if (m->copy_stream) (void)hipStreamDestroy(m->copy_stream);
  for (hipModule_t extra : m->attached) (void)hipModuleUnload(extra);
  if (m->bg_module) (void)hipModuleUnload(m->bg_module);
  if (m->kin_module) (void)hipModuleUnload(m->kin_module);
  if (m->mass_module) (void)hipModuleUnload(m->mass_module);
  if (m->module) (void)hipModuleUnload(m->module);
  delete m;
}

int inflx_attach(inflx_model* m, const char* path) {
  if (!m || !path) return fail(INFLX_ERR_ARG, "model handle / path is NULL");
  INFLX_SERIALISE(m);
  FILE* fh = fopen(path, "rb");
  if (!fh) return fail(INFLX_ERR_IO, "could not open code object %s: %s", path, strerror(errno));
  fclose(fh);
  HIP_TRY(hipSetDevice(m->device));
  return attach_object(m, path);
}

uint32_t inflx_groups(const inflx_model* m) { return m ? m->groups : 0; }

uint32_t inflx_n_fields(const inflx_model* m) { return m ? m->dim : 0; }
uint32_t inflx_n_parameters(const inflx_model* m) { return m ? m->n_par : 0; }
const char* inflx_model_name(const inflx_model* m) { return m ? m->name.c_str() : ""; }
int inflx_device_of(const inflx_model* m) { return m ? m->device : -1; }

int inflx_host_threads(unsigned devices_at_work, unsigned out[3]) {
  if (!out) return fail(INFLX_ERR_ARG, "output array is NULL");
  const unsigned saved = tl_sharers;
  tl_sharers = std::max(1u, devices_at_work);
  out[0] = host_cpu_budget();
  out[1] = prefault_threads();
  out[2] = host_fill_threads();
  tl_sharers = saved;
  return INFLX_OK;
}

int inflx_stage_info(const inflx_model* m, uint32_t* nu, uint32_t* nr, uint32_t* nc, uint32_t* out_mask) {
  if (!m) return fail(INFLX_ERR_ARG, "model handle is NULL");
  if (nu) *nu = m->info.n_uniform;
  if (nr) *nr = m->info.n_row;
  if (nc) *nc = m->info.n_col;
  if (out_mask) *out_mask = m->info.out_mask;
  return INFLX_OK;
}

int inflx_sweep_plan(const inflx_model* m, int op, size_t P, size_t N1, size_t row_count, int layout, uint32_t plan[4]) {
  return inflx_sweep_plan_ex(m, op, P, N1, row_count, layout, INFLX_SWEEP_DEFAULT, plan);
}

int inflx_sweep_plan_ex(const inflx_model* m, int op, size_t P, size_t N1, size_t row_count, int layout, unsigned flags, uint32_t plan[4]) {
  if (!m || !plan) return fail(INFLX_ERR_ARG, "model handle / plan array is NULL");
  if (op < 0 || op >= INFLX_OP_COUNT) return fail(INFLX_ERR_ARG, "unknown sweep operation %d", op);
  if (flags & ~(unsigned)INFLX_SWEEP_FORCE_TILE) return fail(INFLX_ERR_ARG, "unknown sweep flags 0x%x", flags);
  const SweepPlan pl = plan_sweep(m->info, op, layout, P, N1, row_count, flags, false);
  plan[0] = (uint32_t)pl.path;
  plan[1] = plan[2] = plan[3] = 0;
  if (pl.path == INFLX_PATH_ROWS) return INFLX_OK;
  plan[1] = (uint32_t)pl.batch;
  plan[2] = (uint32_t)((P + pl.batch - 1) / pl.batch);
  if (pl.path == INFLX_PATH_ROW_STREAM) plan[3] = (uint32_t)pl.replicas;
  if (pl.path == INFLX_PATH_TILE) {
    const size_t gx = (N1 + m->info.tile_cols - 1) / m->info.tile_cols, slab = std::min(pl.rows_per_launch, row_count);
    plan[2] = (uint32_t)(((P + pl.batch - 1) / pl.batch) * ((row_count + pl.rows_per_launch - 1) / pl.rows_per_launch));
    plan[3] = (uint32_t)tile_height(m->info.tile_rows, gx * slab * pl.batch);
  }
  return INFLX_OK;
}

int inflx_sweep_device_stats(inflx_model* m, const double* p, size_t P, size_t n_p, void* d_out, size_t d_out_bytes, const double* ss,
                             size_t N0, size_t N1, size_t row_begin, size_t row_count, void* stream, inflx_summary* summary) {
  INFLX_SERIALISE(m);
  const int op = INFLX_OP_COMPLETE;
  int rc = validate(m, op, p, P, n_p);
  if (rc) return rc;
  if ((rc = need_groups(m, INFLX_GROUP_STATS))) return rc;
  if (!ss || !summary) return fail(INFLX_ERR_ARG, "start_stop / summary pointer is NULL");
  if (row_begin + row_count > N0) return fail(INFLX_ERR_SHAPE, "rows [%zu,%zu) exceed the grid (N0 = %zu)", row_begin, row_begin + row_count, N0);
  if (d_out && d_out_bytes < P * row_count * N1 * kOpBytes[op])
    return fail(INFLX_ERR_SHAPE, "output buffer has %zu bytes, the sweep writes %zu", d_out_bytes, P * row_count * N1 * kOpBytes[op]);
  HIP_TRY(hipSetDevice(m->device));
  hipStream_t s = stream ? static_cast<hipStream_t>(stream) : m->stream;
  const SweepPlan plan = plan_sweep(m->info, op, INFLX_AOS, P, N1, row_count, INFLX_SWEEP_DEFAULT, false);
  hipStream_t up = plan.upload_stream(m, s), eval = plan.reader_stream(m, s);
  if (!m->d_stats) HIP_TRY(hipMalloc(reinterpret_cast<void**>(&m->d_stats), 18 * sizeof(double)));
  inflx_summary init;
  for (int k = 0; k < 6; ++k) {
    init.min[k] = HUGE_VAL;
    init.max[k] = -HUGE_VAL;
    init.count[k] = 0;
  }
  static_assert(sizeof(inflx_summary) == 18 * 8, "inflx_summary must match the device layout");
  HIP_TRY(hipMemcpyAsync(m->d_stats, &init, sizeof init, hipMemcpyHostToDevice, up));
  const double* d_params = nullptr;
  if ((rc = acquire_params(m, p, P * n_p, up, &d_params))) return rc;
  if (row_count && N1) {
    rc = launch_grid(m, plan, op, d_params, P, static_cast<double*>(d_out), ss, N0, N1, row_begin, row_count, INFLX_AOS, s, false, 0.0, m->d_stats);
  }
  if ((rc = release_params_after(m, eval, rc))) return rc;
  HIP_TRY(hipMemcpyAsync(summary, m->d_stats, sizeof *summary, hipMemcpyDeviceToHost, eval));
  HIP_TRY(hipStreamSynchronize(eval));
  if (eval != s) HIP_TRY(hipStreamSynchronize(s));
  return sf_verdict(m);
}

int inflx_synchronize(inflx_model* m) {
  INFLX_SERIALISE(m);
  if (!m) return fail(INFLX_ERR_ARG, "model handle is NULL");
  HIP_TRY(hipSetDevice(m->device));
  HIP_TRY(hipStreamSynchronize(m->side));
  HIP_TRY(hipStreamSynchronize(m->stream));
  return sf_verdict(m);
}

int inflx_sf_status(inflx_model* m, unsigned* bits, int clear) {
  if (!m || !bits) return fail(INFLX_ERR_ARG, "model handle / status pointer is NULL");
  INFLX_SERIALISE(m);
  return sf_collect(m, clear != 0, bits);
}

int inflx_sf_policy(inflx_model* m, int policy) {
  if (!m) return fail(INFLX_ERR_ARG, "model handle is NULL");
  if (policy != INFLX_SF_QUIET && policy != INFLX_SF_FAIL) return fail(INFLX_ERR_ARG, "unknown special-function policy %d", policy);
  INFLX_SERIALISE(m);
  m->sf_policy = policy;
  return INFLX_OK;
}

int inflx_uses_gsl(const inflx_model* m) { return m ? (int)m->use_gsl : 0; }

int inflx_sweep_device(inflx_model* m, int op, const double* p, size_t P, size_t n_p, void* d_out, size_t d_out_bytes,
                       const double* ss, size_t N0, size_t N1, size_t row_begin, size_t row_count, int layout, void* stream) {
  return inflx_sweep_device_ex(m, op, p, P, n_p, d_out, d_out_bytes, ss, N0, N1, row_begin, row_count, layout, stream, INFLX_SWEEP_DEFAULT);
}

int inflx_sweep_device_ex(inflx_model* m, int op, const double* p, size_t P, size_t n_p, void* d_out, size_t d_out_bytes,
                          const double* ss, size_t N0, size_t N1, size_t row_begin, size_t row_count, int layout, void* stream, unsigned flags) {
  INFLX_SERIALISE(m);
  int rc = validate(m, op, p, P, n_p);
  if (rc) return rc;
  if (!d_out || !ss) return fail(INFLX_ERR_ARG, "output / start_stop pointer is NULL");
  if (layout != INFLX_AOS && layout != INFLX_SOA) return fail(INFLX_ERR_ARG, "unknown layout %d", layout);
  if (flags & ~(unsigned)INFLX_SWEEP_FORCE_TILE) return fail(INFLX_ERR_ARG, "unknown sweep flags 0x%x", flags);
  if (row_begin + row_count > N0) return fail(INFLX_ERR_SHAPE, "rows [%zu,%zu) exceed the grid (N0 = %zu)", row_begin, row_begin + row_count, N0);
  if (op == INFLX_OP_QDIF) return fail(INFLX_ERR_ARG, "the flag sweep has a byte result: use inflx_flag_quantum_dif");
  const size_t need = P * row_count * N1 * kOpBytes[op];
  if (d_out_bytes < need) return fail(INFLX_ERR_SHAPE, "output buffer has %zu bytes, the sweep writes %zu", d_out_bytes, need);
  HIP_TRY(hipSetDevice(m->device));
  hipStream_t s = stream ? static_cast<hipStream_t>(stream) : m->stream;
  const SweepPlan plan = plan_sweep(m->info, op, layout, P, N1, row_count, flags, handle_idle(m));
  const double* d_params = nullptr;
  if ((rc = acquire_params(m, p, P * n_p, plan.upload_stream(m, s), &d_params))) return rc;
  rc = launch_grid(m, plan, op, d_params, P, static_cast<double*>(d_out), ss, N0, N1, row_begin, row_count, layout, s);
  rc = release_params_after(m, plan.reader_stream(m, s), rc);
  if (rc == INFLX_OK && !m->sf_words.empty() && s != m->stream) {
    if (!m->sf_done) HIP_TRY(hipEventCreateWithFlags(&m->sf_done, hipEventDisableTiming));
    HIP_TRY(hipEventRecord(m->sf_done, s));
    m->sf_pending = true;
  }
  return rc;
}

int inflx_sweep_device_timed(inflx_model* m, int op, const double* p, size_t P, size_t n_p, void* d_out, size_t d_out_bytes,
                             const double* ss, size_t N0, size_t N1, size_t row_begin, size_t row_count, int layout, void* stream,
                             int repeats, int dominant_only, float* ms_per_launch) {
  return inflx_sweep_device_timed_ex(m, op, p, P, n_p, d_out, d_out_bytes, ss, N0, N1, row_begin, row_count, layout, stream, repeats, dominant_only,
                                     INFLX_SWEEP_DEFAULT, ms_per_launch);
}

int inflx_sweep_device_timed_ex(inflx_model* m, int op, const double* p, size_t P, size_t n_p, void* d_out, size_t d_out_bytes,
                                const double* ss, size_t N0, size_t N1, size_t row_begin, size_t row_count, int layout, void* stream,
                                int repeats, int mode, unsigned flags, float* ms_per_launch) {
  INFLX_SERIALISE(m);
  if (repeats <= 0 || !ms_per_launch) return fail(INFLX_ERR_ARG, "repeats must be positive and ms_per_launch non-NULL");
  if (mode < INFLX_TIME_BACK_TO_BACK || mode > INFLX_TIME_SINGLE_CALL) return fail(INFLX_ERR_ARG, "unknown timing mode %d", mode);
  int rc = inflx_sweep_device_ex(m, op, p, P, n_p, d_out, d_out_bytes, ss, N0, N1, row_begin, row_count, layout, stream, flags);
  if (rc) return rc;
  hipStream_t s = stream ? static_cast<hipStream_t>(stream) : m->stream;
  if (mode == INFLX_TIME_SINGLE_CALL) {
    float total = 0.f;
    for (int k = 0; k < repeats; ++k) {
      HIP_TRY(hipStreamSynchronize(m->side));
      HIP_TRY(hipStreamSynchronize(s));
      HIP_TRY(hipEventRecord(m->t0, s));
      rc = inflx_sweep_device_ex(m, op, p, P, n_p, d_out, d_out_bytes, ss, N0, N1, row_begin, row_count, layout, stream, flags);
      if (rc) return rc;
      HIP_TRY(hipEventRecord(m->t1, s));
      HIP_TRY(hipEventSynchronize(m->t1));
      float one = 0.f;
      HIP_TRY(hipEventElapsedTime(&one, m->t0, m->t1));
      total += one;
    }
    HIP_TRY(hipStreamSynchronize(m->side));
    *ms_per_launch = total / (float)repeats;
    return INFLX_OK;
  }
  const int dominant_only = mode;
  const double* d_params = m->pslot[m->pcur].dev;
  HIP_TRY(hipStreamSynchronize(s));
  HIP_TRY(hipStreamSynchronize(m->side));
  const SweepPlan plan = plan_sweep(m->info, op, layout, P, N1, row_count, flags, false);
  const hipStream_t reader = plan.reader_stream(m, s);
  std::vector<std::pair<hipEvent_t, hipEvent_t>> pairs;
  struct Disarm {
    inflx_model* m;
    std::vector<std::pair<hipEvent_t, hipEvent_t>>& pairs;
    ~Disarm() {
      m->probe = nullptr;
      for (auto& pr : pairs) {
        if (pr.first) (void)hipEventDestroy(pr.first);
        if (pr.second) (void)hipEventDestroy(pr.second);
      }
    }
  } disarm{m, pairs};
  if (dominant_only == 2) {
    pairs.assign((size_t)repeats * 64, {nullptr, nullptr});
    for (auto& pr : pairs) {
      HIP_TRY(hipEventCreate(&pr.first));
      HIP_TRY(hipEventCreate(&pr.second));
    }
    m->probe = &pairs;
    m->probe_used = 0;
    m->probe_overflow = false;
  }
  HIP_TRY(hipEventRecord(m->t0, s));
  for (int k = 0; k < repeats; ++k) {
    rc = launch_grid(m, plan, op, d_params, P, static_cast<double*>(d_out), ss, N0, N1, row_begin, row_count, layout, s,
                     dominant_only == 1);
    if (rc) return release_params_after(m, reader, rc);
  }
  HIP_TRY(hipEventRecord(m->t1, s));
  if ((rc = release_params(m, reader))) return rc;
  HIP_TRY(hipEventSynchronize(m->t1));
  float ms = 0.f;
  if (dominant_only == 2) {
    if (m->probe_used == 0) return fail(INFLX_ERR_ARG, "in-pipeline timing: this sweep shape has no probed kernel");
    if (m->probe_overflow) return fail(INFLX_ERR_ARG, "in-pipeline timing: more than 64 launches of the dominant kernel per sweep (use fewer parameter rows per call)");
    for (size_t k = 0; k < m->probe_used; ++k) {
      float one = 0.f;
      HIP_TRY(hipEventElapsedTime(&one, pairs[k].first, pairs[k].second));
      ms += one;
    }
  } else {
    HIP_TRY(hipEventElapsedTime(&ms, m->t0, m->t1));
  }
  *ms_per_launch = ms / (float)repeats;
  return INFLX_OK;
}

int inflx_basis_on_points(inflx_model* m, const double* p, size_t n_p, const double* x, size_t n, double* out) {
  INFLX_SERIALISE(m);
  int rc = validate(m, INFLX_OP_RAW, p, 1, n_p, false);
  if (rc) return rc;
  if (n == 0) return INFLX_OK;
  if (!x || !out) return fail(INFLX_ERR_ARG, "point / output pointer is NULL");
  HIP_TRY(hipSetDevice(m->device));
  const size_t in_bytes = n * 2 * sizeof(double), out_bytes = n * 7 * sizeof(double);
  if ((rc = ensure_chunk(m, 0, out_bytes))) return rc;
  if ((rc = ensure_chunk(m, 1, in_bytes))) return rc;
  const double* d_params = nullptr;
  if ((rc = acquire_params(m, p, n_p, m->stream, &d_params))) return rc;
  HIP_TRY(hipMemcpyAsync(m->d_chunk[1], x, in_bytes, hipMemcpyHostToDevice, m->stream));
  InflxTrajectoryArgs a;
  memset(&a, 0, sizeof a);
  a.out = static_cast<double*>(m->d_chunk[0]);
  a.params = d_params;
  a.points = static_cast<const double*>(m->d_chunk[1]);
  a.n = n;
  a.P = 1;
  void* params[] = {&a};
  const size_t gx = (n + m->info.tile_cols - 1) / m->info.tile_cols;
  HIP_TRY(hipModuleLaunchKernel(m->basis_points, (unsigned)gx, 1, 1, m->info.tile_cols, 1, 1, 0, m->stream, params, nullptr));
  HIP_TRY(hipMemcpyAsync(out, m->d_chunk[0], out_bytes, hipMemcpyDeviceToHost, m->stream));
  HIP_TRY(hipStreamSynchronize(m->stream));
  unsigned dropped = 0;
  return sf_collect(m, true, &dropped);
}

int inflx_ops_on_values(inflx_model* m, const double* values, size_t n, double* out, int ieee_only) {
  INFLX_SERIALISE(m);
  if (!m) return fail(INFLX_ERR_ARG, "model handle is NULL");
  if (n == 0) return INFLX_OK;
  if (!values || !out) return fail(INFLX_ERR_ARG, "values / output pointer is NULL");
  HIP_TRY(hipSetDevice(m->device));
  {
    const int rcg = need_groups(m, INFLX_GROUP_VALUES);
    if (rcg) return rcg;
  }
  const size_t in_bytes = n * 5 * sizeof(double), out_bytes = n * 9 * sizeof(double);
  int rc;
  if ((rc = ensure_chunk(m, 0, out_bytes))) return rc;
  if ((rc = ensure_chunk(m, 1, in_bytes))) return rc;
  HIP_TRY(hipMemcpyAsync(m->d_chunk[1], values, in_bytes, hipMemcpyHostToDevice, m->stream));
  InflxTrajectoryArgs a;
  memset(&a, 0, sizeof a);
  a.out = static_cast<double*>(m->d_chunk[0]);
  a.points = static_cast<const double*>(m->d_chunk[1]);
  a.n = n;
  a.P = 1;
  a.reserved = ieee_only ? 1u : 0u;
  void* params[] = {&a};
  const size_t gx = (n + m->info.tile_cols - 1) / m->info.tile_cols;
  if (gx > 0x7fffffffULL) return fail(INFLX_ERR_SHAPE, "too many records for one launch");
  HIP_TRY(hipModuleLaunchKernel(m->ops_on_values, (unsigned)gx, 1, 1, m->info.tile_cols, 1, 1, 0, m->stream, params, nullptr));
  HIP_TRY(hipMemcpyAsync(out, m->d_chunk[0], out_bytes, hipMemcpyDeviceToHost, m->stream));
  HIP_TRY(hipStreamSynchronize(m->stream));
  return INFLX_OK;
}

int inflx_validate_basis_at_random(inflx_model* m, uint64_t seed) {
  INFLX_SERIALISE(m);
  if (!m) return fail(INFLX_ERR_ARG, "model handle is NULL");
  const size_t num_points = 100;
  uint64_t state = seed ? seed : (((uint64_t)std::random_device{}() << 32) ^ std::random_device{}());
  std::vector<double> p(m->n_par), x(2 * num_points);
  for (double& v : p) v = 10. * (-1. + 2. * unit_random(state));
  for (double& v : x) v = -1. + 2. * unit_random(state);
  std::vector<double> basis(7 * num_points);
  int rc = inflx_basis_on_points(m, p.data(), p.size(), x.data(), num_points, basis.data());
  if (rc) return rc;
  size_t failed = 0;
  if ((rc = check_basis(basis.data(), x.data(), num_points, 1e-3, &failed))) return rc;
  if (failed)
    warn("Inflatox was unable to verify basis orthonormality at %zu out of %zu tested points.\nThis could be indicative of a "
         "defective model.\nUsed parameter values: p=%s", failed, num_points, list_text(p.data(), p.size()).c_str());
  return INFLX_OK;
}

int inflx_validate_basis_on_domain(inflx_model* m, const uint32_t* num_points, size_t n_axes, const double* p, size_t n_p,
                                   const double* ss, double accuracy) {
  INFLX_SERIALISE(m);
  if (!m) return fail(INFLX_ERR_ARG, "model handle is NULL");
  if (!num_points || !ss) return fail(INFLX_ERR_ARG, "num_points / start_stop array is NULL");
  say("Validating basis orthonormality on specified domain. This may take a while...");
  if (n_axes != m->dim)
    return fail(INFLX_ERR_SHAPE, "expected an array with with the same number of axes as there are field-space coordinates "
                "(model has %u fields, got %zu)", m->dim, n_axes);
  int rc = validate(m, INFLX_OP_RAW, p, 1, n_p, false);
  if (rc) return rc;
  size_t failed = 0;
  double tested = 1.;
  for (size_t k = 0; k < n_axes; ++k) tested *= (double)num_points[k];
  for (size_t axis = 0; axis < n_axes; ++axis) {
    const size_t n = num_points[axis];
    const double start = ss[2 * axis], stop = ss[2 * axis + 1];
    const double spacing = (stop - start) / (double)n;
    std::vector<double> x(2 * n), basis(7 * n);
    for (size_t idx = 0; idx < n; ++idx) {
      x[2 * idx] = ss[0];
      x[2 * idx + 1] = ss[2];
      x[2 * idx + axis] = stop + spacing * (double)idx;
    }
    if ((rc = inflx_basis_on_points(m, p, n_p, x.data(), n, basis.data()))) return rc;
    if ((rc = check_basis(basis.data(), x.data(), n, accuracy, &failed))) return rc;
    if (failed)
      warn("Inflatox was unable to verify basis orthonormality at %zu out of %g tested points.\nThis could be indicative of a "
           "defective model.\nUsed parameter values: p=%s", failed, tested, list_text(p, n_p).c_str());
  }
  return INFLX_OK;
}

}

namespace {

struct HostDest {
  size_t dst_rows = 0;
  size_t dst_row0 = 0;
  size_t plane0 = 0;
  size_t planes = 0;
};

struct Progress {
  std::atomic<uint64_t> done{0};
  uint64_t total = 0;
};

struct Span {
  size_t src, dst, bytes;
};

std::vector<Span> transfer_spans(int op, size_t P, size_t N1, size_t row_count, int layout, const HostDest& d) {
  const size_t K = kOpWidth[op];
  const bool planes = layout == INFLX_SOA && K > 1;
  const size_t blocks = planes ? P * K : P;
  const size_t row_bytes = planes ? N1 * sizeof(double) : N1 * kOpBytes[op];
  std::vector<Span> spans;
  const bool subset = planes && d.planes != 0;
  for (size_t b = 0; b < blocks; ++b) {
    size_t dst_block = b;
    if (subset) {
      const size_t pr = b / K, k = b % K;
      if (k < d.plane0 || k >= d.plane0 + d.planes) continue;
      dst_block = pr * d.planes + (k - d.plane0);
    }
    const Span sp{b * row_count * row_bytes, (dst_block * d.dst_rows + d.dst_row0) * row_bytes, row_count * row_bytes};
    if (!spans.empty() && spans.back().src + spans.back().bytes == sp.src && spans.back().dst + spans.back().bytes == sp.dst)
      spans.back().bytes += sp.bytes;
    else
      spans.push_back(sp);
  }
  return spans;
}

bool host_fill_enabled() {
  static const bool v = [] {
    const char* e = getenv("INFLX_HOST_FILL");
    return !(e && atoi(e) == 0);
  }();
  return v;
}
size_t host_fill_min_bytes() {
  static const size_t v = [] {
    const char* e = getenv("INFLX_HOST_FILL_MIN_MB");
    const long mb = e ? atol(e) : -1;
    return (size_t)(mb >= 0 ? mb : 8) << 20;
  }();
  return v;
}

void repeat_record(char* dst, const char* rec, size_t rec_bytes, size_t n) {
  const size_t bytes = n * rec_bytes;
#if defined(__x86_64__)
  alignas(64) char pat[16 * 64 + 128];
  const size_t period = 16 * rec_bytes;
  for (size_t off = 0; off < period + 64; off += rec_bytes) memcpy(pat + off, rec, rec_bytes);
  size_t done = 0;
  const size_t head = std::min(bytes, (size_t)((16 - (reinterpret_cast<uintptr_t>(dst) & 15)) & 15));
  if (head) {
    memcpy(dst, pat, head);
    done = head;
  }
  size_t phase = done % period;
  for (; done + 64 <= bytes; done += 64) {
    const char* src = pat + phase;
    __m128d a, b, c, d;
    memcpy(&a, src, 16), memcpy(&b, src + 16, 16), memcpy(&c, src + 32, 16), memcpy(&d, src + 48, 16);
    _mm_stream_pd(reinterpret_cast<double*>(dst + done), a);
    _mm_stream_pd(reinterpret_cast<double*>(dst + done + 16), b);
    _mm_stream_pd(reinterpret_cast<double*>(dst + done + 32), c);
    _mm_stream_pd(reinterpret_cast<double*>(dst + done + 48), d);
    phase += 64;
    if (phase >= period) phase -= period;
  }
  for (; done < bytes; ++done) {
    dst[done] = pat[phase];
    if (++phase == period) phase = 0;
  }
#else
  for (size_t k = 0; k < n; ++k) memcpy(dst + k * rec_bytes, rec, rec_bytes);
#endif
}

void stream_copy(char* dst, const char* src, size_t bytes) {
#if defined(__x86_64__)
  size_t done = std::min(bytes, (size_t)((16 - (reinterpret_cast<uintptr_t>(dst) & 15)) & 15));
  if (done) memcpy(dst, src, done);
  for (; done + 16 <= bytes; done += 16) {
    __m128d a;
    memcpy(&a, src + done, 16);
    _mm_stream_pd(reinterpret_cast<double*>(dst + done), a);
  }
  if (done < bytes) memcpy(dst + done, src + done, bytes - done);
#else
  memcpy(dst, src, bytes);
#endif
}

template <typename F>
void parallel_blocks(size_t n, size_t bytes_per_item, F fill) {
  if (n == 0) return;
  size_t nthreads = std::min<size_t>(host_fill_threads(), n);
  const size_t bytes = n * bytes_per_item;
  nthreads = std::min<size_t>(nthreads, std::max<size_t>({size_t(1), bytes / (size_t(16) << 20), std::min<size_t>(8, bytes / (size_t(4) << 20))}));
  std::vector<std::thread> pool;
  auto block = [&](size_t t) {
    const size_t a = n * t / nthreads, b = n * (t + 1) / nthreads;
    if (b > a) fill(a, b);
#if defined(__x86_64__)
    _mm_sfence();
#endif
  };
  std::vector<size_t> here{0};
  for (size_t t = 1; t < nthreads; ++t) {
    try {
      pool.emplace_back(block, t);
    } catch (...) {
      here.push_back(t);
    }
  }
  for (size_t t : here) block(t);
  for (auto& th : pool) th.join();
}

int sweep_host_body(inflx_model* m, int op, const double* p, size_t P, size_t n_p, void* out_v, const double* ss, size_t N0,
                    size_t N1, size_t row_begin, size_t row_count, int layout, double accuracy, HostDest dest, Progress* progress);

int sweep_host_broadcast(inflx_model* m, int op, int axis, const double* p, size_t P, size_t n_p, char* out, const double* ss, size_t N0,
                         size_t N1, size_t row_begin, size_t row_count, int layout, const HostDest& dest, Progress* progress) {
  const size_t K = kOpWidth[op];
  const bool planes = layout == INFLX_SOA && K > 1;
  const size_t rec = planes ? sizeof(double) : K * sizeof(double);
  const size_t blocks = planes ? P * K : P;
  const size_t dst_row_bytes = N1 * rec;
  for (size_t b = 0; b < blocks; ++b) advise_huge_pages(out + ((b * dest.dst_rows + dest.dst_row0) * N1) * rec, row_count * dst_row_bytes);
  int rc;
  if (axis == 1) {
    std::vector<double> line(P * row_count * K);
    if ((rc = sweep_host_body(m, op, p, P, n_p, line.data(), ss, N0, 1, row_begin, row_count, layout, 0.0, HostDest(), nullptr))) return rc;
    const char* src = reinterpret_cast<const char*>(line.data());
    parallel_blocks(blocks * row_count, dst_row_bytes, [&](size_t first, size_t last) {
      for (size_t q = first; q < last; ++q) {
        const size_t b = q / row_count, r = q % row_count;
        char* dst = out + ((b * dest.dst_rows + dest.dst_row0 + r) * N1) * rec;
        repeat_record(dst, src + q * rec, rec, N1);
        if (progress) progress->done += dst_row_bytes;
      }
    });
    return INFLX_OK;
  }
  std::vector<double> image(P * N1 * K);
  if ((rc = sweep_host_body(m, op, p, P, n_p, image.data(), ss, N0, N1, row_begin, 1, layout, 0.0, HostDest(), nullptr))) return rc;
  const char* src = reinterpret_cast<const char*>(image.data());
  parallel_blocks(blocks * row_count, dst_row_bytes, [&](size_t first, size_t last) {
    for (size_t q = first; q < last; ++q) {
      const size_t b = q / row_count, r = q % row_count;
      char* dst = out + ((b * dest.dst_rows + dest.dst_row0 + r) * N1) * rec;
      stream_copy(dst, src + b * dst_row_bytes, dst_row_bytes);
      if (progress) progress->done += dst_row_bytes;
    }
  });
  return INFLX_OK;
}

int sweep_host_body(inflx_model* m, int op, const double* p, size_t P, size_t n_p, void* out_v, const double* ss, size_t N0,
                    size_t N1, size_t row_begin, size_t row_count, int layout, double accuracy, HostDest dest, Progress* progress) {
  INFLX_SERIALISE(m);
  char* const out = static_cast<char*>(out_v);
  int rc = validate(m, op, p, P, n_p);
  if (rc) return rc;
  if (!out || !ss) return fail(INFLX_ERR_ARG, "output / start_stop pointer is NULL");
  if (layout != INFLX_AOS && layout != INFLX_SOA) return fail(INFLX_ERR_ARG, "unknown layout %d", layout);
  if (row_begin + row_count > N0) return fail(INFLX_ERR_SHAPE, "rows [%zu,%zu) exceed the grid (N0 = %zu)", row_begin, row_begin + row_count, N0);
  if (row_count == 0 || N1 == 0) return INFLX_OK;
  if (dest.dst_rows == 0) dest.dst_rows = row_count;
  if (dest.dst_row0 + row_count > dest.dst_rows) return fail(INFLX_ERR_SHAPE, "slab rows [%zu,%zu) exceed the destination's %zu rows", dest.dst_row0, dest.dst_row0 + row_count, dest.dst_rows);
  HIP_TRY(hipSetDevice(m->device));

  const size_t K = kOpWidth[op];
  const size_t row_bytes = N1 * kOpBytes[op];
  const size_t total = P * row_count * row_bytes;
  const bool subset = dest.planes != 0;
  if (subset && (layout != INFLX_SOA || K == 1 || dest.plane0 + dest.planes > K))
    return fail(INFLX_ERR_ARG, "a plane subset [%zu, %zu) needs the planes layout of an operation with at least that many values (this one has %zu)", dest.plane0, dest.plane0 + dest.planes, K);
  if (!subset && op != INFLX_OP_QDIF && host_fill_enabled() && total >= host_fill_min_bytes()) {
    if ((m->info.out_mask & 2u) == 0 && N1 > 1) return sweep_host_broadcast(m, op, 1, p, P, n_p, out, ss, N0, N1, row_begin, row_count, layout, dest, progress);
    if ((m->info.out_mask & 3u) == 2u && row_count > 1) return sweep_host_broadcast(m, op, 0, p, P, n_p, out, ss, N0, N1, row_begin, row_count, layout, dest, progress);
  }
  bool whole = whole_result_limit() != 0 && (total <= whole_result_limit() || subset);
  if (whole && total > m->d_whole_cap) {
    if (m->d_whole) HIP_TRY(hipFree(m->d_whole));
    m->d_whole = nullptr;
    m->d_whole_cap = 0;
    if (hipMalloc(&m->d_whole, total) == hipSuccess) {
      m->d_whole_cap = total;
    } else {
      (void)hipGetLastError();
      m->d_whole = nullptr;
      whole = false;
    }
  }
  const SweepPlan plan = plan_sweep(m->info, op, layout, whole ? P : 1, N1, row_count, INFLX_SWEEP_DEFAULT, whole);
  const double* d_params = nullptr;
  if ((rc = acquire_params(m, p, P * n_p, plan.upload_stream(m, m->stream), &d_params))) return rc;
  if (whole) {
    rc = launch_grid(m, plan, op, d_params, P, static_cast<double*>(m->d_whole), ss, N0, N1, row_begin, row_count, layout, m->stream, false, accuracy);
    if (rc) {
      (void)hipStreamSynchronize(m->side);
      (void)hipStreamSynchronize(m->stream);
      return rc;
    }
    const std::vector<Span> spans = transfer_spans(op, P, N1, row_count, layout, dest);
    struct Stripe { char* at; size_t bytes; };
    std::vector<Stripe> stripes;
    const size_t stripe = size_t(16) << 20;
    for (const Span& sp : spans) {
      advise_huge_pages(out + sp.dst, sp.bytes);
      for (size_t off = 0; off < sp.bytes; off += stripe) stripes.push_back({out + sp.dst + off, std::min(stripe, sp.bytes - off)});
    }
    size_t head_stripes = 0;
    {
      char* run_at = nullptr;
      size_t run_bytes = 0;
      for (size_t bytes = 0; head_stripes < stripes.size() && (!kTouchIsAtomic || bytes < (size_t(64) << 20)); ++head_stripes) {
        const Stripe& st = stripes[head_stripes];
        if (run_bytes && run_at + run_bytes != st.at) {
          prefault_range(run_at, run_bytes);
          run_bytes = 0;
        }
        if (!run_bytes) run_at = st.at;
        run_bytes += st.bytes;
        bytes += st.bytes;
      }
      if (run_bytes) prefault_range(run_at, run_bytes);
    }
    std::vector<std::thread> pool;
    if (head_stripes < stripes.size()) {
      const size_t rest = stripes.size() - head_stripes;
      const unsigned nthreads = (unsigned)std::min<size_t>(prefault_threads(), rest);
      try {
        for (unsigned t = 0; t < nthreads; ++t)
          pool.emplace_back([&stripes, head_stripes, t, nthreads] {
            for (size_t k = head_stripes + t; k < stripes.size(); k += nthreads) touch_range(stripes[k].at, stripes[k].bytes);
          });
      } catch (...) {
      }
    }
    const size_t slice = size_t(256) << 20;
    hipError_t e = hipSuccess;
    std::vector<std::pair<hipEvent_t, size_t>> marks;
    for (const Span& sp : spans) {
      for (size_t off = 0; off < sp.bytes && e == hipSuccess; off += slice) {
        const size_t n = std::min(slice, sp.bytes - off);
        e = hipMemcpyAsync(out + sp.dst + off, static_cast<char*>(m->d_whole) + sp.src + off, n, hipMemcpyDeviceToHost, m->stream);
        if (progress && e == hipSuccess) {
          hipEvent_t ev = nullptr;
          if (hipEventCreateWithFlags(&ev, hipEventDisableTiming) == hipSuccess && hipEventRecord(ev, m->stream) == hipSuccess) {
            marks.push_back({ev, n});
          } else {
            if (ev) (void)hipEventDestroy(ev);
            marks.push_back({nullptr, n});
          }
        }
      }
    }
    size_t unmarked = 0;
    for (auto& mk : marks) {
      if (mk.first) {
        if (e == hipSuccess) e = hipEventSynchronize(mk.first);
        (void)hipEventDestroy(mk.first);
        if (e == hipSuccess) progress->done += mk.second;
      } else {
        unmarked += mk.second;
      }
    }
    {
      const hipError_t se = hipStreamSynchronize(m->stream);
      if (e == hipSuccess) e = se;
    }
    if (progress && e == hipSuccess) progress->done += unmarked;
    for (auto& th : pool) th.join();
    if (m->d_whole_cap > (size_t(4) << 30) || (subset && m->d_whole_cap > (size_t(1) << 30))) {
      (void)hipFree(m->d_whole);
      m->d_whole = nullptr;
      m->d_whole_cap = 0;
    }
    if (e != hipSuccess) return fail(INFLX_ERR_DEVICE, "device-to-host copy failed: %s", hipGetErrorString(e));
    return INFLX_OK;
  }
  size_t rows_per_chunk = std::max<size_t>(1, chunk_bytes_limit() / row_bytes);
  rows_per_chunk = std::min(rows_per_chunk, row_count);
  const size_t chunk_bytes = rows_per_chunk * row_bytes;
  for (int k = 0; k < 2; ++k)
    if ((rc = ensure_chunk(m, k, chunk_bytes))) return rc;

  struct Piece { size_t pr, r, nrows; };
  std::vector<Piece> pieces;
  for (size_t pr = 0; pr < P; ++pr)
    for (size_t r = 0; r < row_count; r += rows_per_chunk) pieces.push_back({pr, r, std::min(rows_per_chunk, row_count - r)});
  const bool planes = layout == INFLX_SOA && K > 1;
  const size_t k_lo = subset ? dest.plane0 : 0, k_hi = subset ? dest.plane0 + dest.planes : K;
  const size_t piece_row_bytes = planes ? (k_hi - k_lo) * N1 * sizeof(double) : row_bytes;
  auto dst_of = [&](const Piece& pc, size_t k) {
    return planes ? out + (((pc.pr * (k_hi - k_lo) + (k - k_lo)) * dest.dst_rows) + dest.dst_row0 + pc.r) * N1 * sizeof(double)
                  : out + ((pc.pr * dest.dst_rows) + dest.dst_row0 + pc.r) * row_bytes;
  };
  auto touch = [&](const Piece& pc) {
    if (!planes) {
      prefault_range(dst_of(pc, 0), pc.nrows * row_bytes);
    } else {
      for (size_t k = k_lo; k < k_hi; ++k) prefault_range(dst_of(pc, k), pc.nrows * N1 * sizeof(double));
    }
  };
  auto start_touch = [&](const Piece& pc) {
    try {
      return std::async(std::launch::async, touch, pc);
    } catch (...) {
      touch(pc);
      return std::future<void>();
    }
  };
  std::future<void> ready = start_touch(pieces[0]);
  bool used[2] = {false, false};
  auto drain = [&] {
    if (ready.valid()) ready.wait();
    (void)hipStreamSynchronize(m->side);
    (void)hipStreamSynchronize(m->stream);
    (void)hipStreamSynchronize(m->copy_stream);
  };
  size_t counted = 0;
  for (size_t c = 0; c < pieces.size(); ++c) {
    const Piece& pc = pieces[c];
    const int b = (int)(c & 1);
    if (used[b]) {
      hipError_t we = progress ? hipEventSynchronize(m->copy_done[b]) : hipStreamWaitEvent(m->stream, m->copy_done[b], 0);
      if (we != hipSuccess) { drain(); return fail(INFLX_ERR_DEVICE, "waiting for a chunk copy failed: %s", hipGetErrorString(we)); }
      if (progress)
        for (; counted + 2 <= c; ++counted) progress->done += pieces[counted].nrows * piece_row_bytes;
    }
    rc = launch_grid(m, plan, op, d_params + pc.pr * n_p, 1, static_cast<double*>(m->d_chunk[b]), ss, N0, N1, row_begin + pc.r, pc.nrows, layout,
                     m->stream, false, accuracy);
    if (rc) { drain(); return rc; }
    if (ready.valid()) ready.wait();
    if (c + 1 < pieces.size()) ready = start_touch(pieces[c + 1]);
    hipError_t e = hipEventRecord(m->chunk_done[b], m->stream);
    if (e == hipSuccess) e = hipStreamWaitEvent(m->copy_stream, m->chunk_done[b], 0);
    if (e == hipSuccess) {
      if (!planes) {
        e = hipMemcpyAsync(dst_of(pc, 0), m->d_chunk[b], pc.nrows * row_bytes, hipMemcpyDeviceToHost, m->copy_stream);
      } else {
        for (size_t k = k_lo; k < k_hi && e == hipSuccess; ++k) {
          const double* src = static_cast<const double*>(m->d_chunk[b]) + k * pc.nrows * N1;
          e = hipMemcpyAsync(dst_of(pc, k), src, pc.nrows * N1 * sizeof(double), hipMemcpyDeviceToHost, m->copy_stream);
        }
      }
    }
    if (e == hipSuccess) e = hipEventRecord(m->copy_done[b], m->copy_stream);
    if (e != hipSuccess) { drain(); return fail(INFLX_ERR_DEVICE, "device-to-host copy failed: %s", hipGetErrorString(e)); }
    used[b] = true;
  }
  if (ready.valid()) ready.wait();
  HIP_TRY(hipStreamSynchronize(m->copy_stream));
  HIP_TRY(hipStreamSynchronize(m->stream));
  if (progress)
    for (; counted < pieces.size(); ++counted) progress->done += pieces[counted].nrows * piece_row_bytes;
  return INFLX_OK;
}

int sweep_host_impl(inflx_model* m, int op, const double* p, size_t P, size_t n_p, void* out_v, const double* ss, size_t N0,
                    size_t N1, size_t row_begin, size_t row_count, int layout, double accuracy, HostDest dest, Progress* progress) {
  INFLX_SERIALISE(m);
  const int rc = sweep_host_body(m, op, p, P, n_p, out_v, ss, N0, N1, row_begin, row_count, layout, accuracy, dest, progress);
  return rc ? rc : sf_verdict(m);
}

size_t progress_min_bytes() {
  static const size_t v = [] {
    const char* e = getenv("INFLX_PROGRESS_MIN_MB");
    const long mb = e ? atol(e) : -1;
    return (size_t)(mb >= 0 ? mb : 1024) << 20;
  }();
  return v;
}
long progress_interval_ms() {
  static const long v = [] {
    const char* e = getenv("INFLX_PROGRESS_INTERVAL_MS");
    const long ms = e ? atol(e) : 0;
    return ms > 0 ? ms : 500L;
  }();
  return v;
}

class Reporter {
 public:
  Reporter(Progress* pr, double points, bool wanted) : pr_(pr), points_(points) {
    if (!wanted || !pr || pr->total < progress_min_bytes()) return;
    t0_ = std::chrono::steady_clock::now();
    try {
      th_ = std::thread([this] { run(); });
    } catch (...) {
    }
  }
  ~Reporter() {
    if (!th_.joinable()) return;
    {
      std::lock_guard<std::mutex> g(mu_);
      stop_ = true;
    }
    cv_.notify_all();
    th_.join();
  }
  Reporter(const Reporter&) = delete;
  Reporter& operator=(const Reporter&) = delete;
  bool active() const { return th_.joinable(); }

 private:
  void run() {
    std::unique_lock<std::mutex> g(mu_);
    const auto step = std::chrono::milliseconds(progress_interval_ms());
    while (!cv_.wait_for(g, step, [this] { return stop_; })) {
      const double sec = std::chrono::duration<double>(std::chrono::steady_clock::now() - t0_).count();
      const double frac = std::min(1.0, (double)pr_->done.load() / (double)std::max<uint64_t>(pr_->total, 1));
      const double rate = frac * points_ / std::max(sec, 1e-9);
      char eta[32];
      if (frac > 0.0) snprintf(eta, sizeof eta, "%.1f s", sec * (1.0 - frac) / frac); else snprintf(eta, sizeof eta, "?");
      say("Time to completion: %s | grid points/s: %.3g | %3.0f%%", eta, rate, 100.0 * frac);
    }
  }
  Progress* pr_;
  double points_;
  std::chrono::steady_clock::time_point t0_;
  std::thread th_;
  std::mutex mu_;
  std::condition_variable cv_;
  bool stop_ = false;
};

int grid_entry(inflx_model* m, int op, const double* p, size_t n_p, double* out, const double* ss, size_t N0, size_t N1,
               int progress, const char* what) {
  if (!out) return fail(INFLX_ERR_ARG, "output array is NULL");
  if (!ss) return fail(INFLX_ERR_ARG, "start_stop array is NULL");
  int rc = validate(m, op, p, 1, n_p);
  if (rc) return rc;
  const auto t0 = std::chrono::steady_clock::now();
  if (progress) say("Calculating %s on HIP device %d (%s).", what, m->device, m->name.c_str());
  Progress pr;
  pr.total = (uint64_t)N0 * N1 * kOpBytes[op];
  {
    Reporter reporter(&pr, (double)N0 * (double)N1, progress != 0);
    rc = sweep_host_impl(m, op, p, 1, n_p, out, ss, N0, N1, 0, N0, INFLX_AOS, 0.0, HostDest(), reporter.active() ? &pr : nullptr);
  }
  if (rc) return rc;
  if (progress) {
    const double sec = std::chrono::duration<double>(std::chrono::steady_clock::now() - t0).count();
    say("Calculation finished. Took %.3f s (%.3g grid points/s including the copy to host memory).", sec,
        (double)N0 * (double)N1 / std::max(sec, 1e-9));
  }
  return INFLX_OK;
}

void block_bounds(size_t n_items, size_t world, size_t rank, size_t* begin, size_t* count) {
  const size_t base = n_items / world, extra = n_items % world;
  *begin = rank * base + std::min(rank, extra);
  *count = base + (rank < extra ? 1 : 0);
}

struct ShardPlan {
  int axis;
  size_t p_begin, p_count, row_begin, row_count;
};
ShardPlan shard_plan(size_t P, size_t N0, size_t world, size_t rank) {
  ShardPlan s;
  if (P >= world) {
    s.axis = 0;
    block_bounds(P, world, rank, &s.p_begin, &s.p_count);
    s.row_begin = 0;
    s.row_count = N0;
  } else {
    s.axis = 1;
    s.p_begin = 0;
    s.p_count = P;
    block_bounds(N0, world, rank, &s.row_begin, &s.row_count);
  }
  return s;
}
}

struct inflx_multi {
  std::vector<inflx_model*> dev;
  std::string path;
  std::vector<std::vector<hipStream_t>> push;
  std::vector<hipEvent_t> swept;
  std::vector<void*> comms;
  std::mutex mu;
};

namespace {
struct RcclApi {
  int (*CommInitAll)(void** comms, int ndev, const int* devlist) = nullptr;
  int (*CommDestroy)(void* comm) = nullptr;
  int (*AllGather)(const void* send, void* recv, size_t count, int dtype, void* comm, hipStream_t stream) = nullptr;
  int (*GroupStart)() = nullptr;
  int (*GroupEnd)() = nullptr;
  const char* (*GetErrorString)(int) = nullptr;
  std::string origin;
};
constexpr int kNcclFloat64 = 8;

const RcclApi* rccl_api(std::string* why = nullptr) {
  static std::string failure;
  static const RcclApi api = [] {
    RcclApi a;
    void* h = nullptr;
    const char* names[] = {"librccl.so.1", "librccl.so", "/opt/rocm/lib/librccl.so.1", "/opt/rocm/lib/librccl.so"};
    for (const char* nm : names)
      if ((h = dlopen(nm, RTLD_NOW | RTLD_NOLOAD))) { a.origin = std::string(nm) + " (already mapped)"; break; }
    if (!h)
      for (const char* nm : names) {
        if ((h = dlopen(nm, RTLD_NOW | RTLD_GLOBAL))) { a.origin = nm; break; }
        const char* e = dlerror();
        failure += std::string(failure.empty() ? "" : "; ") + nm + ": " + (e ? e : "not found");
      }
    if (!h) return a;
    failure.clear();
    auto bind = [&](const char* sym) -> void* {
      void* fn = dlsym(h, sym);
      if (!fn) failure += std::string(failure.empty() ? "" : ", ") + sym;
      return fn;
    };
    a.CommInitAll = reinterpret_cast<decltype(a.CommInitAll)>(bind("ncclCommInitAll"));
    a.CommDestroy = reinterpret_cast<decltype(a.CommDestroy)>(bind("ncclCommDestroy"));
    a.AllGather = reinterpret_cast<decltype(a.AllGather)>(bind("ncclAllGather"));
    a.GroupStart = reinterpret_cast<decltype(a.GroupStart)>(bind("ncclGroupStart"));
    a.GroupEnd = reinterpret_cast<decltype(a.GroupEnd)>(bind("ncclGroupEnd"));
    a.GetErrorString = reinterpret_cast<decltype(a.GetErrorString)>(bind("ncclGetErrorString"));
    if (!failure.empty()) failure = a.origin + " lacks " + failure;
    return a;
  }();
  const bool ok = api.CommInitAll && api.CommDestroy && api.AllGather && api.GroupStart && api.GroupEnd && api.GetErrorString;
  if (!ok && why) *why = failure.empty() ? "library or symbols missing" : failure;
  return ok ? &api : nullptr;
}

struct GatherCall {
  size_t image, rank, send_off, recv_off, count;
};
std::vector<GatherCall> rccl_gather_calls(size_t P, size_t N0, size_t row_bytes, size_t world) {
  std::vector<GatherCall> calls;
  const ShardPlan s0 = shard_plan(P, N0, world, 0);
  const size_t images = s0.axis == 0 ? 1 : P;
  const size_t block_bytes = s0.axis == 0 ? s0.p_count * N0 * row_bytes : s0.row_count * row_bytes;
  const size_t image_bytes = s0.axis == 0 ? P * N0 * row_bytes : N0 * row_bytes;
  for (size_t q = 0; q < images; ++q)
    for (size_t k = 0; k < world; ++k) calls.push_back({q, k, q * image_bytes + k * block_bytes, q * image_bytes, block_bytes / sizeof(double)});
  return calls;
}

#define RCCL_TRY(api, expr)                                                                                       \
  do {                                                                                                            \
    const int r_ = (expr);                                                                                        \
    if (r_ != 0) return fail(INFLX_ERR_DEVICE, "%s failed: %s", #expr, (api)->GetErrorString(r_));               \
  } while (0)

int ensure_comms(inflx_multi* mm, const RcclApi* api) {
  std::lock_guard<std::mutex> g(mm->mu);
  const size_t n = mm->dev.size();
  if (mm->comms.size() == n) return INFLX_OK;
  std::vector<int> devs(n);
  for (size_t k = 0; k < n; ++k) devs[k] = mm->dev[k]->device;
  for (size_t k = 0; k < n; ++k)
    for (size_t j = k + 1; j < n; ++j)
      if (devs[k] == devs[j])
        return fail(INFLX_ERR_ARG, "the RCCL all-gather needs one device per handle (device %d appears twice): a communicator has one rank per GPU; "
                    "the peer-push gather (INFLX_GATHER_PEER_PUSH) has no such restriction", devs[k]);
  std::vector<void*> comms(n, nullptr);
  RCCL_TRY(api, api->CommInitAll(comms.data(), (int)n, devs.data()));
  mm->comms = std::move(comms);
  return INFLX_OK;
}

template <typename F>
int run_parts(size_t n, F part) {
  std::vector<int> rcs(n, INFLX_OK);
  std::vector<std::string> msgs(n);
  auto body = [&](size_t k) {
    const unsigned before = tl_sharers;
    tl_sharers = (unsigned)n;
    rcs[k] = part(k);
    tl_sharers = before;
    if (rcs[k] != INFLX_OK) msgs[k] = g_last_error;
  };
  std::vector<std::thread> pool;
  std::vector<size_t> inline_parts{0};
  for (size_t k = 1; k < n; ++k) {
    try {
      pool.emplace_back(body, k);
    } catch (...) {
      inline_parts.push_back(k);
    }
  }
  for (size_t k : inline_parts)
    if (k < n) body(k);
  for (auto& th : pool) th.join();
  for (size_t k = 0; k < n; ++k)
    if (rcs[k] != INFLX_OK) {
      g_last_error = msgs[k];
      return rcs[k];
    }
  return INFLX_OK;
}

size_t devices_used(const inflx_multi* mm, size_t max_devices) {
  const size_t n = mm->dev.size();
  return max_devices ? std::min(n, max_devices) : n;
}
}

extern "C" {

int inflx_sweep_host(inflx_model* m, int op, const double* p, size_t P, size_t n_p, double* out, const double* ss, size_t N0,
                     size_t N1, size_t row_begin, size_t row_count, int layout) {
  if (op == INFLX_OP_QDIF) return fail(INFLX_ERR_ARG, "the flag sweep has a byte result: use inflx_flag_quantum_dif");
  return sweep_host_impl(m, op, p, P, n_p, out, ss, N0, N1, row_begin, row_count, layout, 0.0, HostDest(), nullptr);
}

int inflx_sweep_host_planes(inflx_model* m, int op, const double* p, size_t P, size_t n_p, double* out, const double* ss, size_t N0,
                            size_t N1, size_t row_begin, size_t row_count, size_t first_plane, size_t n_planes) {
  if (op == INFLX_OP_QDIF) return fail(INFLX_ERR_ARG, "the flag sweep has a byte result: use inflx_flag_quantum_dif");
  if (n_planes == 0) return fail(INFLX_ERR_ARG, "no planes requested");
  HostDest dest;
  dest.plane0 = first_plane;
  dest.planes = n_planes;
  return sweep_host_impl(m, op, p, P, n_p, out, ss, N0, N1, row_begin, row_count, INFLX_SOA, 0.0, dest, nullptr);
}

int inflx_flag_quantum_dif(inflx_model* m, const double* p, size_t n_p, uint8_t* out, const double* ss, size_t N0, size_t N1,
                           int progress, double accuracy) {
  if (!out || !ss) return fail(INFLX_ERR_ARG, "output / start_stop pointer is NULL");
  if (!m) return fail(INFLX_ERR_ARG, "model handle is NULL");
  if (progress) say("Calculating zeros of the potential gradient on HIP device %d.", m->device);
  return sweep_host_impl(m, INFLX_OP_QDIF, p, 1, n_p, out, ss, N0, N1, 0, N0, INFLX_AOS, accuracy, HostDest(), nullptr);
}

// ... 957 lines not shown
```

Measured before the change: 150.8 billion.

## Add row-pass evaluator kernel with inline kernel-argument parameters on one stream

Adds a separately compiled row-pass kernel module for models whose outputs do not depend on the second coordinate. It evaluates each row once and writes the replicated row table with a wider block split across slices. When the sweep runs on one stream and the parameters fit, they are passed inline in the kernel arguments instead of being uploaded. Cross-stream event hops are replaced by ordering on the solo stream, which trims per-call upload and synchronisation overhead. The cost is a larger kernel-argument struct and more complex ring ordering logic.

```diff
diff --git a/include/inflx_hip.h b/include/inflx_hip.h
--- a/include/inflx_hip.h
+++ b/include/inflx_hip.h
@@ -146,6 +146,7 @@
 int inflx_sf_status(inflx_model* model, unsigned* bits, int clear);
 int inflx_sf_policy(inflx_model* model, int policy);
 int inflx_uses_gsl(const inflx_model* model);
+int inflx_has_row_pass(const inflx_model* model);
 
 typedef struct inflx_multi inflx_multi;
 int inflx_shard_plan(size_t P, size_t N0, int world, int rank, size_t plan[5]);
diff --git a/inflatox_amd/_native.py b/inflatox_amd/_native.py
--- a/inflatox_amd/_native.py
+++ b/inflatox_amd/_native.py
@@ -76,6 +76,7 @@
     "inflx_sf_status": (C.c_int, [C.c_void_p, C.POINTER(C.c_uint), C.c_int]),
     "inflx_sf_policy": (C.c_int, [C.c_void_p, C.c_int]),
     "inflx_uses_gsl": (C.c_int, [C.c_void_p]),
+    "inflx_has_row_pass": (C.c_int, [C.c_void_p]),
     "inflx_sweep_plan": (C.c_int, [C.c_void_p, C.c_int, _SIZE, _SIZE, _SIZE, C.c_int, C.POINTER(C.c_uint32)]),
     "inflx_basis_on_points": (C.c_int, [C.c_void_p, _DP, _SIZE, _DP, _SIZE, _DP]),
     "inflx_ops_on_values": (C.c_int, [C.c_void_p, _DP, _SIZE, _DP, C.c_int]),
@@ -290,6 +291,10 @@
     def uses_gsl(self) -> bool:
         return bool(self._lib.inflx_uses_gsl(self._h))
 
+    @property
+    def has_row_pass(self) -> bool:
+        return bool(self._lib.inflx_has_row_pass(self._h))
+
     def sf_status(self, clear: bool = True) -> int:
         bits = C.c_uint(0)
         _check(self._lib.inflx_sf_status(self._h, C.byref(bits), int(bool(clear))))
diff --git a/inflatox_amd/compiler.py b/inflatox_amd/compiler.py
--- a/inflatox_amd/compiler.py
+++ b/inflatox_amd/compiler.py
@@ -242,6 +242,11 @@
                      ("INFLX_MASS_HEADER", "mass{key}.h", self.masses_header_text())],
         )
 
+    def ensure_rowpass(self) -> str | None:
+        if (self.stage_info or {}).get("out_mask", 3) & 2:
+            return None
+        return self._ensure_companion("rowpass", _ROWPASS_SOURCES, "rp{key}.hsaco", lambda: [])
+
     def ensure_all_groups(self) -> list[str]:
         return [p for p in (self.ensure_group(g) for g in KERNEL_GROUPS) if p]
 
@@ -335,6 +340,7 @@
 _BACKGROUND_SOURCES = ("inflx_background_kernels.hip", "inflx_background.h", "inflx_background_abi.h", "inflx_background_rows.h")
 _KINEMATICS_SOURCES = ("inflx_kinematics_kernels.hip", "inflx_kinematics.h", "inflx_kinematics_abi.h")
 _MASSES_SOURCES = ("inflx_masses_kernels.hip", "inflx_masses.h", "inflx_masses_abi.h")
+_ROWPASS_SOURCES = ("inflx_rowpass_kernels.hip", "inflx_rowpass_abi.h")
 
 
 def _build_companion_object(header_text: str, options: list[str], tag: str, sources: tuple, object_name: str, headers: list):
@@ -721,4 +727,5 @@
         art.kernel_groups = self.kernel_groups
         art._build = (header, options, tag)
         art._eom_recipe = (self.symbolic_out, dict(self._param_slots), self.cse, self.max_cses)
+        art.ensure_rowpass()
         return art
diff --git a/inflatox_amd/csrc/inflx_hip.cpp b/inflatox_amd/csrc/inflx_hip.cpp
--- a/inflatox_amd/csrc/inflx_hip.cpp
+++ b/inflatox_amd/csrc/inflx_hip.cpp
@@ -30,6 +30,7 @@
 #include "inflx_background_abi.h"
 #include "inflx_background_rows.h"
 #include "inflx_kernel_abi.h"
+#include "inflx_rowpass_abi.h"
 #include "inflx_kinematics_abi.h"
 #include "inflx_masses_abi.h"
 
@@ -250,13 +251,15 @@
   hipEvent_t free[2] = {nullptr, nullptr};
   bool used[2] = {false, false};
   unsigned turn = 0;
+  hipStream_t solo[2] = {nullptr, nullptr};
+  hipEvent_t solo_done = nullptr;
 
   bool create() {
     for (int b = 0; b < 2; ++b)
       if (hipEventCreateWithFlags(&ready[b], hipEventDisableTiming | hipEventDisableSystemFence) != hipSuccess ||
           hipEventCreateWithFlags(&free[b], hipEventDisableTiming | hipEventDisableSystemFence) != hipSuccess)
         return false;
-    return true;
+    return hipEventCreateWithFlags(&solo_done, hipEventDisableTiming | hipEventDisableSystemFence) == hipSuccess;
   }
   void destroy() {
     for (int b = 0; b < 2; ++b) {
@@ -264,6 +267,19 @@
       if (free[b]) (void)hipEventDestroy(free[b]);
       if (buf[b]) (void)hipFree(buf[b]);
     }
+    if (solo_done) (void)hipEventDestroy(solo_done);
+  }
+  int order_behind_solo(int b, hipStream_t next) {
+    const hipStream_t last = solo[b];
+    solo[b] = nullptr;
+    if (!last || last == next) return INFLX_OK;
+    if (hipEventRecord(solo_done, last) == hipSuccess) {
+      HIP_TRY(hipStreamWaitEvent(next, solo_done, 0));
+    } else {
+      (void)hipGetLastError();
+      HIP_TRY(hipDeviceSynchronize());
+    }
+    return INFLX_OK;
   }
   bool idle() const {
     for (int b = 0; b < 2; ++b)
@@ -299,6 +315,9 @@
   hipFunction_t rowvals[INFLX_OP_COUNT] = {};
   hipFunction_t rowstream6 = nullptr;
   hipFunction_t rowstream_planes = nullptr;
+  hipModule_t rowpass_module = nullptr;
+  hipFunction_t rowpass[INFLX_OP_COUNT] = {};
+  hipFunction_t rowpass_stats = nullptr;
   hipFunction_t colvals[INFLX_OP_COUNT] = {};
   hipFunction_t colstream = nullptr;
   hipFunction_t colvals_stats = nullptr;
@@ -371,7 +390,8 @@
 
 int acquire_params(inflx_model* m, const double* p, size_t count, hipStream_t s, const double** d_params) {
   inflx_model::ParamSlot& cur = m->pslot[m->pcur];
-  if (cur.dev && cur.count == count && cur.stream == s && memcmp(cur.host, p, count * sizeof(double)) == 0) {
+  if (cur.dev && cur.count == count && memcmp(cur.host, p, count * sizeof(double)) == 0) {
+    if (cur.stream != s && cur.in_flight) HIP_TRY(hipStreamWaitEvent(s, cur.last_use, 0));
     *d_params = cur.dev;
     return INFLX_OK;
   }
@@ -419,6 +439,16 @@
   return rc;
 }
 
+template <typename Plan>
+int acquire_params_for(inflx_model* m, const Plan& plan, const double* p, size_t count, hipStream_t s, const double** d_params) {
+  *d_params = nullptr;
+  return plan.inline_params ? INFLX_OK : acquire_params(m, p, count, plan.upload_stream(m, s), d_params);
+}
+template <typename Plan>
+int release_params_for(inflx_model* m, const Plan& plan, hipStream_t s, int rc) {
+  return plan.inline_params ? rc : release_params_after(m, plan.reader_stream(m, s), rc);
+}
+
 void note_sf_word(inflx_model* m, hipModule_t module) {
   if (!m->use_gsl) return;
   hipDeviceptr_t dptr = nullptr;
@@ -510,6 +540,44 @@
   if (hipModuleGetGlobal(&dptr, &size, module, sym) != hipSuccess) return fail(INFLX_ERR_SYMBOL, "artefact %s lacks symbol %s", path, sym);
   if (exact ? size != bytes : size > bytes) return fail(INFLX_ERR_SYMBOL, "symbol %s in %s has %zu bytes, expected %s%zu", sym, path, size, exact ? "" : "<= ", bytes);
   HIP_TRY(hipMemcpy(dst, dptr, size, hipMemcpyDeviceToHost));
+  return INFLX_OK;
+}
+
+int load_rowpass(inflx_model* m) {
+  const std::string path = m->path + ".rowpass";
+  FILE* fh = fopen(path.c_str(), "rb");
+  if (!fh) return INFLX_OK;
+  fclose(fh);
+  hipModule_t module = nullptr;
+  hipError_t e = hipModuleLoad(&module, path.c_str());
+  if (e != hipSuccess) return fail(INFLX_ERR_IO, "could not load %s as a gfx950 code object: %s", path.c_str(), hipGetErrorString(e));
+  auto bail = [&](int code) {
+    const std::string first = g_last_error;
+    (void)hipModuleUnload(module);
+    g_last_error = first;
+    return code;
+  };
+  uint32_t abi = 0;
+  char tag[128] = {0};
+  int rc;
+  if ((rc = read_global_of(module, path.c_str(), "INFLX_ROWPASS_ABI", &abi, sizeof abi, true)) ||
+      (rc = read_global_of(module, path.c_str(), "MODEL_TAG", tag, sizeof tag - 1, false)))
+    return bail(rc);
+  if (abi != INFLX_ROWPASS_ABI_VERSION || m->tag != tag)
+    return bail(fail(INFLX_ERR_VERSION, "%s does not belong to artefact %s: built from another model, with other options or for another ABI (tag \"%s\", expected \"%s\")",
+                     path.c_str(), m->path.c_str(), tag, m->tag.c_str()));
+  hipFunction_t fn[INFLX_OP_COUNT] = {}, stats = nullptr;
+  for (int op = 0; op < INFLX_OP_COUNT; ++op) {
+    if (op == INFLX_OP_QDIF) continue;
+    const std::string name = std::string("inflx_rowpass_") + kOpNames[op];
+    if (hipModuleGetFunction(&fn[op], module, name.c_str()) != hipSuccess) return bail(fail(INFLX_ERR_SYMBOL, "%s lacks kernel %s", path.c_str(), name.c_str()));
+  }
+  if (hipModuleGetFunction(&stats, module, "inflx_rowpass_complete_stats") != hipSuccess)
+    return bail(fail(INFLX_ERR_SYMBOL, "%s lacks kernel inflx_rowpass_complete_stats", path.c_str()));
+  m->rowpass_module = module;
+  for (int op = 0; op < INFLX_OP_COUNT; ++op) m->rowpass[op] = fn[op];
+  m->rowpass_stats = stats;
+  note_sf_word(m, module);
   return INFLX_OK;
 }
 
@@ -585,6 +653,7 @@
   size_t replicas = 0;
   size_t rows_per_launch = 0;
   bool one_stream = false;
+  bool inline_params = false;
 
   hipStream_t upload_stream(const inflx_model* m, hipStream_t s) const {
     return path == INFLX_PATH_ROWS || one_stream ? s : m->side;
@@ -630,6 +699,13 @@
   return pl;
 }
 
+SweepPlan plan_call(const inflx_model* m, int op, int layout, size_t P, size_t N1, size_t row_count, unsigned flags, bool tile_alone) {
+  SweepPlan pl = plan_sweep(m->info, op, layout, P, N1, row_count, flags, true);
+  if (pl.path == INFLX_PATH_TILE && !tile_alone) pl.one_stream = false;
+  pl.inline_params = pl.path == INFLX_PATH_ROW_STREAM && pl.one_stream && m->rowpass_module && P * m->n_par <= INFLX_INLINE_PARAMS;
+  return pl;
+}
+
 bool handle_idle(inflx_model* m) {
   const bool idle = m->row_ring.idle() && m->stage_ring.idle();
   (void)hipGetLastError();
@@ -653,22 +729,31 @@
 struct BroadcastPath {
   hipFunction_t eval;
   unsigned eval_gx, eval_block;
+  bool rowpass;
   hipFunction_t store;
   size_t cpr;
   size_t z_per_p;
   size_t table_doubles;
 };
 
-int launch_broadcast(inflx_model* m, const SweepPlan& plan, const BroadcastPath& path, int op, InflxSweepArgs a, const double* d_params, size_t P,
-                     double* d_out, hipStream_t s, bool stores_only) {
+int launch_broadcast(inflx_model* m, const SweepPlan& plan, const BroadcastPath& path, int op, InflxSweepArgs a, const double* p_host,
+                     const double* d_params, size_t P, double* d_out, hipStream_t s, bool stores_only) {
   void* params[] = {&a};
+  InflxRowPassArgs ra;
+  memset(&ra, 0, sizeof ra);
+  void* eval_params[] = {path.rowpass ? static_cast<void*>(&ra) : static_cast<void*>(&a)};
   TableRing& ring = m->row_ring;
-  const hipStream_t ev = plan.upload_stream(m, s);
+  const bool one = plan.one_stream;
+  const hipStream_t ev = one ? s : m->side;
   const size_t batch = plan.batch, row_count = a.row_count;
   if (path.cpr > 0x7fffffffULL) return fail(INFLX_ERR_SHAPE, "grid rows too long for one launch");
   if (stores_only && batch < P)
     return fail(INFLX_ERR_ARG, "dominant_only timing needs the parameter rows to fit one table batch (%zu rows here, got %zu)", batch, P);
+  if (plan.inline_params && !p_host && m->n_par) return fail(INFLX_ERR_ARG, "internal: a sweep planned with in-line parameters got none");
   const bool store = d_out != nullptr;
+  unsigned slices = 1;
+  if (path.rowpass)
+    while (slices < 4 && slices < a.table_replicas && (size_t)path.eval_gx * std::min(batch, P) * slices * 2 <= 2048) slices *= 2;
   for (size_t p0 = 0; p0 < P; p0 += batch) {
     const size_t pb = std::min(batch, P - p0);
     const int b = (int)((ring.turn + (stores_only ? 1 : 0)) & 1);
@@ -677,18 +762,28 @@
       const int rc = ring.grow(b, pb * path.table_doubles);
       if (rc) return rc;
     }
-    a.params = d_params + p0 * m->n_par;
+    if (plan.inline_params) {
+      a.params = nullptr;
+      if (m->n_par) memcpy(ra.params_inline, p_host, pb * m->n_par * sizeof(double));
+    } else {
+      a.params = d_params + p0 * m->n_par;
+    }
     a.out = store ? d_out + p0 * row_count * a.N1 * kOpWidth[op] : nullptr;
     a.P = (uint32_t)pb;
     a.row_table = store ? ring.buf[b] : nullptr;
     if (!stores_only) {
       if (ring.used[b]) HIP_TRY(hipStreamWaitEvent(ev, ring.free[b], 0));
-      HIP_TRY(hipModuleLaunchKernel(path.eval, path.eval_gx, (unsigned)pb, 1, path.eval_block, 1, 1, 0, ev, params, nullptr));
-      if (ev != s) HIP_TRY(hipEventRecord(ring.ready[b], ev));
+      ring.used[b] = false;
+      const int rc = ring.order_behind_solo(b, ev);
+      if (rc) return rc;
+      if (one) ring.solo[b] = s;
+      ra.a = a;
+      HIP_TRY(hipModuleLaunchKernel(path.eval, path.eval_gx, (unsigned)pb, slices, path.eval_block, 1, 1, 0, ev, eval_params, nullptr));
+      if (!one) HIP_TRY(hipEventRecord(ring.ready[b], ev));
       ring.turn++;
     }
     if (store) {
-      if (ev != s) HIP_TRY(hipStreamWaitEvent(s, ring.ready[b], 0));
+      if (!one) HIP_TRY(hipStreamWaitEvent(s, ring.ready[b], 0));
       for (size_t r0 = 0; r0 < row_count; r0 += 65535) {
         a.stream_row0 = (uint32_t)r0;
         const size_t nr = std::min<size_t>(65535, row_count - r0);
@@ -696,8 +791,10 @@
         HIP_TRY(hipModuleLaunchKernel(path.store, (unsigned)path.cpr, (unsigned)nr, (unsigned)(pb * path.z_per_p), m->info.tile_cols, 1, 1, 0, s, params, nullptr));
         HIP_TRY(probe_end(m, s));
       }
-      HIP_TRY(hipEventRecord(ring.free[b], s));
-      ring.used[b] = true;
+      if (!one) {
+        HIP_TRY(hipEventRecord(ring.free[b], s));
+        ring.used[b] = true;
+      }
     }
   }
   return INFLX_OK;
@@ -776,7 +873,7 @@
   return INFLX_OK;
 }
 
-int launch_grid(inflx_model* m, const SweepPlan& plan, int op, const double* d_params, size_t P, double* d_out, const double* ss, size_t N0,
+int launch_grid(inflx_model* m, const SweepPlan& plan, int op, const double* p_host, const double* d_params, size_t P, double* d_out, const double* ss, size_t N0,
                 size_t N1, size_t row_begin, size_t row_count, int layout, hipStream_t s, bool stores_only = false, double accuracy = 0.0,
                 double* d_stats = nullptr) {
   if (row_count == 0 || N1 == 0) return INFLX_OK;
@@ -784,7 +881,7 @@
     for (size_t p0 = 0; p0 < P; p0 += 65535) {
       const size_t pb = std::min<size_t>(65535, P - p0);
       double* sub = d_out ? reinterpret_cast<double*>(reinterpret_cast<char*>(d_out) + p0 * row_count * N1 * kOpBytes[op]) : nullptr;
-      const int rc = launch_grid(m, plan, op, d_params + p0 * m->n_par, pb, sub, ss, N0, N1, row_begin, row_count, layout, s, stores_only, accuracy, d_stats);
+      const int rc = launch_grid(m, plan, op, p_host + p0 * m->n_par, d_params + p0 * m->n_par, pb, sub, ss, N0, N1, row_begin, row_count, layout, s, stores_only, accuracy, d_stats);
       if (rc) return rc;
     }
     return INFLX_OK;
@@ -811,17 +908,19 @@
       const bool aos6 = K == 6 && layout == INFLX_AOS;
       a.table_replicas = (uint32_t)plan.replicas;
       a.stream_planes = (uint32_t)K;
-      const BroadcastPath path = {d_stats ? m->rowvals_stats : m->rowvals[op], (unsigned)((row_count + 63) / 64), 64,
+      const bool rp = m->rowpass_module != nullptr;
+      const BroadcastPath path = {d_stats ? (rp ? m->rowpass_stats : m->rowvals_stats) : (rp ? m->rowpass[op] : m->rowvals[op]), (unsigned)((row_count + 63) / 64),
+                                  rp ? (unsigned)m->info.tile_cols : 64u, rp,
                                   aos6 ? m->rowstream6 : m->rowstream_planes, plan.cpr, aos6 ? 1 : K, row_count * plan.replicas * 8};
-      return launch_broadcast(m, plan, path, op, a, d_params, P, d_out, s, stores_only);
+      return launch_broadcast(m, plan, path, op, a, p_host, d_params, P, d_out, s, stores_only);
     }
     case INFLX_PATH_COL_STREAM: {
       const bool planes = layout == INFLX_SOA || K == 1;
       a.stream_units = (planes ? N1 : K * N1) / 2;
       const size_t tc = m->info.tile_cols;
-      const BroadcastPath path = {d_stats ? m->colvals_stats : m->colvals[op], (unsigned)((N1 + tc - 1) / tc), (unsigned)tc,
+      const BroadcastPath path = {d_stats ? m->colvals_stats : m->colvals[op], (unsigned)((N1 + tc - 1) / tc), (unsigned)tc, false,
                                   m->colstream, (a.stream_units + tc - 1) / tc, planes ? K : 1, K * N1};
-      return launch_broadcast(m, plan, path, op, a, d_params, P, d_out, s, stores_only);
+      return launch_broadcast(m, plan, path, op, a, p_host, d_params, P, d_out, s, stores_only);
     }
     case INFLX_PATH_ROWS:
       return launch_rows_fallback(m, op, a, P, N1, row_count, s);
@@ -996,6 +1095,7 @@
     if ((rc = resolve_group_kernels(m, m->module, present, artefact_path))) return bail(rc);
     m->groups = present;
   }
+  if ((m->info.out_mask & 2u) == 0 && (rc = load_rowpass(m))) return bail(rc);
   if (hipStreamCreateWithFlags(&m->stream, hipStreamNonBlocking) != hipSuccess ||
       hipStreamCreateWithFlags(&m->side, hipStreamNonBlocking) != hipSuccess ||
       hipStreamCreateWithFlags(&m->copy_stream, hipStreamNonBlocking) != hipSuccess) {
@@ -1051,6 +1151,7 @@
   if (m->copy_stream) (void)hipStreamDestroy(m->copy_stream);
   for (hipModule_t extra : m->attached) (void)hipModuleUnload(extra);
   if (m->bg_module) (void)hipModuleUnload(m->bg_module);
+  if (m->rowpass_module) (void)hipModuleUnload(m->rowpass_module);
   if (m->kin_module) (void)hipModuleUnload(m->kin_module);
   if (m->mass_module) (void)hipModuleUnload(m->mass_module);
   if (m->module) (void)hipModuleUnload(m->module);
@@ -1130,7 +1231,7 @@
     return fail(INFLX_ERR_SHAPE, "output buffer has %zu bytes, the sweep writes %zu", d_out_bytes, P * row_count * N1 * kOpBytes[op]);
   HIP_TRY(hipSetDevice(m->device));
   hipStream_t s = stream ? static_cast<hipStream_t>(stream) : m->stream;
-  const SweepPlan plan = plan_sweep(m->info, op, INFLX_AOS, P, N1, row_count, INFLX_SWEEP_DEFAULT, false);
+  const SweepPlan plan = plan_call(m, op, INFLX_AOS, P, N1, row_count, INFLX_SWEEP_DEFAULT, false);
   hipStream_t up = plan.upload_stream(m, s), eval = plan.reader_stream(m, s);
   if (!m->d_stats) HIP_TRY(hipMalloc(reinterpret_cast<void**>(&m->d_stats), 18 * sizeof(double)));
   inflx_summary init;
@@ -1142,11 +1243,11 @@
   static_assert(sizeof(inflx_summary) == 18 * 8, "inflx_summary must match the device layout");
   HIP_TRY(hipMemcpyAsync(m->d_stats, &init, sizeof init, hipMemcpyHostToDevice, up));
   const double* d_params = nullptr;
-  if ((rc = acquire_params(m, p, P * n_p, up, &d_params))) return rc;
+  if ((rc = acquire_params_for(m, plan, p, P * n_p, s, &d_params))) return rc;
   if (row_count && N1) {
-    rc = launch_grid(m, plan, op, d_params, P, static_cast<double*>(d_out), ss, N0, N1, row_begin, row_count, INFLX_AOS, s, false, 0.0, m->d_stats);
-  }
-  if ((rc = release_params_after(m, eval, rc))) return rc;
+    rc = launch_grid(m, plan, op, p, d_params, P, static_cast<double*>(d_out), ss, N0, N1, row_begin, row_count, INFLX_AOS, s, false, 0.0, m->d_stats);
+  }
+  if ((rc = release_params_for(m, plan, s, rc))) return rc;
   HIP_TRY(hipMemcpyAsync(summary, m->d_stats, sizeof *summary, hipMemcpyDeviceToHost, eval));
   HIP_TRY(hipStreamSynchronize(eval));
   if (eval != s) HIP_TRY(hipStreamSynchronize(s));
@@ -1177,6 +1278,8 @@
 }
 
 int inflx_uses_gsl(const inflx_model* m) { return m ? (int)m->use_gsl : 0; }
+
+int inflx_has_row_pass(const inflx_model* m) { return m && m->rowpass_module ? 1 : 0; }
 
 int inflx_sweep_device(inflx_model* m, int op, const double* p, size_t P, size_t n_p, void* d_out, size_t d_out_bytes,
                        const double* ss, size_t N0, size_t N1, size_t row_begin, size_t row_count, int layout, void* stream) {
@@ -1197,11 +1300,12 @@
   if (d_out_bytes < need) return fail(INFLX_ERR_SHAPE, "output buffer has %zu bytes, the sweep writes %zu", d_out_bytes, need);
   HIP_TRY(hipSetDevice(m->device));
   hipStream_t s = stream ? static_cast<hipStream_t>(stream) : m->stream;
-  const SweepPlan plan = plan_sweep(m->info, op, layout, P, N1, row_count, flags, handle_idle(m));
+  SweepPlan plan = plan_call(m, op, layout, P, N1, row_count, flags, true);
+  if (plan.path == INFLX_PATH_TILE && plan.one_stream && !handle_idle(m)) plan.one_stream = false;
   const double* d_params = nullptr;
-  if ((rc = acquire_params(m, p, P * n_p, plan.upload_stream(m, s), &d_params))) return rc;
-  rc = launch_grid(m, plan, op, d_params, P, static_cast<double*>(d_out), ss, N0, N1, row_begin, row_count, layout, s);
-  rc = release_params_after(m, plan.reader_stream(m, s), rc);
+  if ((rc = acquire_params_for(m, plan, p, P * n_p, s, &d_params))) return rc;
+  rc = launch_grid(m, plan, op, p, d_params, P, static_cast<double*>(d_out), ss, N0, N1, row_begin, row_count, layout, s);
+  rc = release_params_for(m, plan, s, rc);
   if (rc == INFLX_OK && !m->sf_words.empty() && s != m->stream) {
     if (!m->sf_done) HIP_TRY(hipEventCreateWithFlags(&m->sf_done, hipEventDisableTiming));
     HIP_TRY(hipEventRecord(m->sf_done, s));
@@ -1245,11 +1349,10 @@
     return INFLX_OK;
   }
   const int dominant_only = mode;
-  const double* d_params = m->pslot[m->pcur].dev;
   HIP_TRY(hipStreamSynchronize(s));
   HIP_TRY(hipStreamSynchronize(m->side));
-  const SweepPlan plan = plan_sweep(m->info, op, layout, P, N1, row_count, flags, false);
-  const hipStream_t reader = plan.reader_stream(m, s);
+  const SweepPlan plan = plan_call(m, op, layout, P, N1, row_count, flags, false);
+  const double* d_params = plan.inline_params ? nullptr : m->pslot[m->pcur].dev;
   std::vector<std::pair<hipEvent_t, hipEvent_t>> pairs;
   struct Disarm {
     inflx_model* m;
@@ -1274,12 +1377,12 @@
   }
   HIP_TRY(hipEventRecord(m->t0, s));
   for (int k = 0; k < repeats; ++k) {
-    rc = launch_grid(m, plan, op, d_params, P, static_cast<double*>(d_out), ss, N0, N1, row_begin, row_count, layout, s,
+    rc = launch_grid(m, plan, op, p, d_params, P, static_cast<double*>(d_out), ss, N0, N1, row_begin, row_count, layout, s,
                      dominant_only == 1);
-    if (rc) return release_params_after(m, reader, rc);
+    if (rc) return release_params_for(m, plan, s, rc);
   }
   HIP_TRY(hipEventRecord(m->t1, s));
-  if ((rc = release_params(m, reader))) return rc;
+  if ((rc = release_params_for(m, plan, s, INFLX_OK))) return rc;
   HIP_TRY(hipEventSynchronize(m->t1));
   float ms = 0.f;
   if (dominant_only == 2) {
@@ -1619,11 +1722,11 @@
       whole = false;
     }
   }
-  const SweepPlan plan = plan_sweep(m->info, op, layout, whole ? P : 1, N1, row_count, INFLX_SWEEP_DEFAULT, whole);
+  const SweepPlan plan = plan_call(m, op, layout, whole ? P : 1, N1, row_count, INFLX_SWEEP_DEFAULT, whole);
   const double* d_params = nullptr;
-  if ((rc = acquire_params(m, p, P * n_p, plan.upload_stream(m, m->stream), &d_params))) return rc;
+  if ((rc = acquire_params_for(m, plan, p, P * n_p, m->stream, &d_params))) return rc;
   if (whole) {
-    rc = launch_grid(m, plan, op, d_params, P, static_cast<double*>(m->d_whole), ss, N0, N1, row_begin, row_count, layout, m->stream, false, accuracy);
+    rc = launch_grid(m, plan, op, p, d_params, P, static_cast<double*>(m->d_whole), ss, N0, N1, row_begin, row_count, layout, m->stream, false, accuracy);
     if (rc) {
       (void)hipStreamSynchronize(m->side);
       (void)hipStreamSynchronize(m->stream);
@@ -1757,7 +1860,7 @@
       if (progress)
         for (; counted + 2 <= c; ++counted) progress->done += pieces[counted].nrows * piece_row_bytes;
     }
-    rc = launch_grid(m, plan, op, d_params + pc.pr * n_p, 1, static_cast<double*>(m->d_chunk[b]), ss, N0, N1, row_begin + pc.r, pc.nrows, layout,
+    rc = launch_grid(m, plan, op, p + pc.pr * n_p, d_params ? d_params + pc.pr * n_p : nullptr, 1, static_cast<double*>(m->d_chunk[b]), ss, N0, N1, row_begin + pc.r, pc.nrows, layout,
                      m->stream, false, accuracy);
     if (rc) { drain(); return rc; }
     if (ready.valid()) ready.wait();
diff --git a/inflatox_amd/csrc/inflx_rowpass_abi.h b/inflatox_amd/csrc/inflx_rowpass_abi.h
--- /dev/null
+++ b/inflatox_amd/csrc/inflx_rowpass_abi.h
@@ -0,0 +1,12 @@
+#pragma once
+#include <stdint.h>
+
+#include "inflx_kernel_abi.h"
+
+#define INFLX_ROWPASS_ABI_VERSION 1u
+#define INFLX_INLINE_PARAMS 16
+
+struct InflxRowPassArgs {
+  struct InflxSweepArgs a;
+  double params_inline[INFLX_INLINE_PARAMS];
+};
diff --git a/inflatox_amd/csrc/inflx_rowpass_kernels.hip b/inflatox_amd/csrc/inflx_rowpass_kernels.hip
--- /dev/null
+++ b/inflatox_amd/csrc/inflx_rowpass_kernels.hip
@@ -0,0 +1,84 @@
+#define INFLX_KERNEL_GROUPS 0u
+#include "inflx_sweep_kernels.hip"
+
+#include "inflx_rowpass_abi.h"
+
+INFLX_EXPORT uint32_t INFLX_ROWPASS_ABI = INFLX_ROWPASS_ABI_VERSION;
+
+template <int OP>
+__device__ __forceinline__ void rowpass_eval(const InflxSweepArgs& a, const double* A, uint64_t row, double* o) {
+  double U[kNU], R[kNR], C[kNC];
+  inflx_stage_uniform(A, U);
+  const double x0 = inflx_coord(a.row_begin + row, a.dx0, a.x0a);
+  inflx_stage_row(x0, A, U, R);
+  InflxModelValues mv;
+  inflx_stage_point(x0, a.x1a, A, U, R, C, mv);
+  fill_v01<OP>(mv, x0, a.x1a, A);
+  apply_op<OP>(mv, o, a.accuracy);
+}
+
+__device__ __forceinline__ void rowpass_params(const InflxRowPassArgs& ra, unsigned p, double* A) {
+  if (ra.a.params) return load_params(ra.a.params, p, A);
+  constexpr int kInlineRows = INFLX_INLINE_PARAMS / kNP;
+#pragma unroll
+  for (int k = 0; k < kNP; ++k) A[k] = 0.0;
+#pragma unroll
+  for (int q = 0; q < kInlineRows; ++q) {
+#pragma unroll
+    for (int k = 0; k < INFLX_N_PARAMETERS; ++k) A[k] = p == (unsigned)q ? ra.params_inline[q * INFLX_N_PARAMETERS + k] : A[k];
+  }
+}
+
+template <int OP, bool STATS = false>
+__device__ __forceinline__ void rowpass(const InflxRowPassArgs& ra) {
+  const InflxSweepArgs& a = ra.a;
+  __shared__ __attribute__((aligned(16))) double vals[kWave][8];
+  const unsigned tid = threadIdx.x;
+  const uint64_t row0 = (uint64_t)blockIdx.x * kWave;
+  const unsigned p = blockIdx.y;
+  if (tid < kWave) {
+    double o[8] = {0., 0., 0., 0., 0., 0., 0., 0.};
+    if (row0 + tid < a.row_count) {
+      double A[kNP];
+      rowpass_params(ra, p, A);
+      rowpass_eval<OP>(a, A, row0 + tid, o);
+    }
+    if constexpr (STATS) {
+      if (blockIdx.z == 0) {
+        StatAcc acc;
+        stat_init(acc);
+        if (row0 + tid < a.row_count) stat_add(acc, o, a.N1);
+        stat_flush(acc, a.stats);
+      }
+    }
+#pragma unroll
+    for (int k = 0; k < 8; ++k) vals[tid][k] = o[k];
+  }
+  if constexpr (STATS) {
+    if (a.row_table == nullptr) return;
+  }
+  __syncthreads();
+  const uint64_t left = a.row_count - row0;
+  const unsigned nrows = left < (uint64_t)kWave ? (unsigned)left : (unsigned)kWave;
+  const unsigned shift = 31 - __builtin_clz(a.table_replicas * 4);
+  const unsigned units = nrows << shift;
+  inflx_d2* dst = reinterpret_cast<inflx_d2*>(a.row_table + ((uint64_t)p * a.row_count + row0) * a.table_replicas * 8);
+  for (unsigned q = blockIdx.z * blockDim.x + tid; q < units; q += gridDim.z * blockDim.x) {
+    const unsigned r = q >> shift, part = q & 3;
+    dst[q] = *reinterpret_cast<const inflx_d2*>(&vals[r][2 * part]);
+  }
+}
+
+#define INFLX_DEFINE_ROWPASS(NAME, OP)                                                                      \
+  extern "C" __global__ __launch_bounds__(kThreads) void inflx_rowpass_##NAME(const InflxRowPassArgs ra) { \
+    if constexpr ((INFLX_OUT_MASK & 2) == 0) rowpass<OP>(ra);                                             \
+  }
+INFLX_DEFINE_ROWPASS(complete, INFLX_OP_COMPLETE)
+INFLX_DEFINE_ROWPASS(consistency, INFLX_OP_CONSISTENCY)
+INFLX_DEFINE_ROWPASS(rapidturn, INFLX_OP_RAPIDTURN)
+INFLX_DEFINE_ROWPASS(epsilon_v, INFLX_OP_EPSILON_V)
+INFLX_DEFINE_ROWPASS(raw, INFLX_OP_RAW)
+INFLX_DEFINE_ROWPASS(hesse, INFLX_OP_HESSE)
+extern "C" __global__ __launch_bounds__(kThreads) void inflx_rowpass_complete_stats(const InflxRowPassArgs ra) {
+  if constexpr ((INFLX_OUT_MASK & 2) == 0) rowpass<INFLX_OP_COMPLETE, true>(ra);
+}
```

After: 153.6 billion (median of 6 runs). +1.8%, better.
